# srogatch/ProbQA

Hardware: AMD Instinct MI355X
Metric: next_question_selections_per_sec (higher is better)
Workload: dtype f64; 1 GPU; 1000Qx5Ax1000T fp64 cube resident in HBM, single in-flight quiz; step = priority sweep + argmax + question id on host, synchronous call through the C ABI; questions_per_gpu=1000, parallelism=single GPU, eval_kernel=wg256_np2, selected_question=500

## Files before the change

probqa_amd/csrc/batch_kernels.hip:

```cpp
#include <algorithm>

#include "eval_device.h"
#include "pole_device.h"
#include "pqa_device.h"
#include "pqa_kernels.h"

namespace pqa {

static __device__ double gLog2TableB[kLog2TableDoubles];

hipError_t UploadLog2TableBatch(const double *hostTable) {
  return hipMemcpyToSymbol(HIP_SYMBOL(gLog2TableB), hostTable, kLog2TableDoubles * sizeof(double));
}

namespace {

constexpr int kTileThreads = 256;

template <typename R>
__global__ __launch_bounds__(kTileThreads) void batch_prep_kernel(const QuizSlot *__restrict__ slots, int nSlots, int Bp,
                                                                  const uint32_t *__restrict__ tgap, int64_t ldT, R *__restrict__ PT) {
  __shared__ double tile[64][65];
  const int64_t t0 = (int64_t)blockIdx.x * 64;
  const int b0 = blockIdx.y * 64;
// ... 458 lines not shown
      red[(wave * (K + 2) + K + 1) * QS + slot] = accL;
    }
    __syncthreads();
    if (head) {
      const bool skip = bit_test(a.qgap, q) || ((asked[q >> 5] >> (q & 31)) & 1u);
      double pri = 0.0;
      if (!skip) {
        double mW[K], mWV[K], sums[2];
#pragma unroll
        for (int r = 0; r < K + 2; r++) {
          double s2 = 0.0;
#pragma unroll
          for (int w2 = 0; w2 < NW; w2++) s2 += red[(w2 * (K + 2) + r) * QS + slot];
          if (r < K) { mW[r] = W[r]; mWV[r] = W[r] * sqrt(s2); }
          else sums[r - K] = s2;
        }
        pri = eval_epilogue(mW, -sums[0], mWV, kN, sums[1], a.vCompTail);
        uint32_t listRows = watchW[slot];
        if (watchW[QS + slot] != 0) {
#pragma unroll
          for (int r = 0; r < K; r++)
            if ((EXACT || r < kN) && ((watchW[QS + slot] >> r) & 1u) && mWV[r] * mWV[r] <= kSmallV * (mW[r] * mW[r])) listRows |= 1u << r;
        }
        if (live && listRows != 0) {
          const uint32_t at = pole_list_append(a.poleList, (uint32_t)q, listRows, (uint32_t)b);
          double *dst = a.poleSums + (size_t)at * (2 * kN + 2);
#pragma unroll
          for (int r = 0; r < K; r++)
            if (EXACT || r < kN) { dst[r] = mW[r]; dst[kN + r] = mWV[r]; }
          dst[2 * kN] = sums[0];
          dst[2 * kN + 1] = sums[1];
        }
      }
      watchW[slot] = 0;
      watchW[QS + slot] = 0;
      if (live) {
        if (a.priorityT) a.priorityT[q * Bp + b] = pri;
        if (!skip) {
          if (qs.hostPriority != nullptr) {
            typedef unsigned int u4 __attribute__((ext_vector_type(4)));
            const uint64_t w0 = d2u(pri), w1 = a.tag;
            const u4 x = {(unsigned)w0, (unsigned)(w0 >> 32), (unsigned)w1, (unsigned)(w1 >> 32)};
            asm volatile("global_store_dwordx4 %0, %1, off sc0 sc1" ::"v"(qs.hostPriority + q), "v"(x) : "memory");
          }
          const double cand = pri != pri ? -__builtin_huge_val() : pri;
          if (bestQ < 0 || cand > bestP) { bestP = cand; bestQ = q; }
        }
      }
    }
  }
  if (head && b < Bp) a.recs[(size_t)blockIdx.x * Bp + b] = BatchRecord{bestP, bestQ};
}

__global__ __launch_bounds__(64) void batch_pick_kernel(const BatchRecord *__restrict__ recs, int nRecs, int Bp,
                                                        const QuizSlot *__restrict__ slots, int nSlots, int64_t outBase,
                                                        uint64_t flagValue, uint32_t *dirty, const double *__restrict__ priorityT,
                                                        int64_t Q, const uint32_t *__restrict__ qgap) {
  const int b = blockIdx.x, lane = threadIdx.x;
  if (b >= nSlots) return;
  double bp = 0.0;
  int64_t bq = -1;
  if (dirty != nullptr && dirty[b] != 0) {
    const uint32_t *asked = slots[b].asked;
    for (int64_t q = lane; q < Q; q += 64) {
      if (bit_test(qgap, q) || bit_test(asked, q)) continue;
      double p = priorityT[(size_t)q * Bp + b];
      if (p != p) p = -__builtin_huge_val();
      if (bq < 0 || p > bp) { bp = p; bq = q; }
    }
    if (lane == 0) dirty[b] = 0;
  } else
  for (int g = lane; g < nRecs; g += 64) {
    const BatchRecord r = recs[(size_t)g * Bp + b];
    if (r.index >= 0 && (bq < 0 || r.priority > bp || (r.priority == bp && r.index < bq))) { bp = r.priority; bq = r.index; }
  }
#pragma unroll
  for (int m = 32; m >= 1; m >>= 1) {
    const double op = __shfl_xor(bp, m, 64);
    const int64_t oq = __shfl_xor(bq, m, 64);
    if (oq >= 0 && (bq < 0 || op > bp || (op == bp && oq < bq))) { bp = op; bq = oq; }
  }
  if (lane != 0) return;
  const QuizSlot s = slots[b];
  s.out->priority = bq < 0 ? 0.0 : bp;
  s.out->index = bq < 0 ? -1 : bq + outBase;
  if (s.seq != nullptr) {
    __builtin_amdgcn_fence(__ATOMIC_RELEASE, "");
    __hip_atomic_store(s.seq, flagValue, __ATOMIC_RELAXED, __HIP_MEMORY_SCOPE_SYSTEM);
  }
}

constexpr int kF32LdsTargets = 16384;
__device__ __forceinline__ float wave_sum_f(float v) { return wave_sum_f32(v); }
template <bool LDSROW, int NT>
__global__ __launch_bounds__(NT) void eval_questions_f32_stream(const float *__restrict__ cube, const double *__restrict__ prior,
                                                                 const uint32_t *__restrict__ tgap, const uint32_t *__restrict__ qgap,
                                                                 const uint32_t *__restrict__ asked, double *__restrict__ priority,
                                                                 int64_t K, int64_t Q, int64_t ldT, double vCompTail) {
  constexpr int NW = NT / kWave;
  extern __shared__ double smem[];
  double *wk = smem, *wv = smem + K;
  float *part = reinterpret_cast<float *>(smem + 2 * K);
  float4 *prL = reinterpret_cast<float4 *>(part + 64), *idL = prL + (ldT >> 2);
  const int tid = threadIdx.x, lane = tid % kWave, wave = tid / kWave;
  const int64_t nQuads = ldT >> 2;
  auto prior4 = [&](int64_t i) __attribute__((always_inline)) {
    const uint32_t g = tgap[i >> 3] >> ((4 * i) & 31);
    const double2 a = reinterpret_cast<const double2 *>(prior)[2 * i], b = reinterpret_cast<const double2 *>(prior)[2 * i + 1];
    return make_float4((g & 1) ? 0.f : (float)a.x, (g & 2) ? 0.f : (float)a.y, (g & 4) ? 0.f : (float)b.x, (g & 8) ? 0.f : (float)b.y);
  };
  auto invd4 = [&](const float4 *rowD, int64_t i) __attribute__((always_inline)) {
    const uint32_t g = tgap[i >> 3] >> ((4 * i) & 31);
    const float4 d = rowD[i];
    return make_float4((g & 1) ? 0.f : rcp_nr_f32(d.x), (g & 2) ? 0.f : rcp_nr_f32(d.y), (g & 4) ? 0.f : rcp_nr_f32(d.z),
                       (g & 8) ? 0.f : rcp_nr_f32(d.w));
  };
  if constexpr (LDSROW)
    for (int64_t i = tid; i < nQuads; i += NT) prL[i] = prior4(i);
  for (int64_t q = blockIdx.x; q < Q; q += gridDim.x) {
    if (bit_test(qgap, q) || bit_test(asked, q)) {
      if (tid == 0) priority[q] = 0.0;
      continue;
    }
    const float *qb = cube + q * (K + 1) * ldT;
    const float4 *rowD = reinterpret_cast<const float4 *>(qb + K * ldT);
    __syncthreads();
    if constexpr (LDSROW)
      for (int64_t i = tid; i < nQuads; i += NT) idL[i] = invd4(rowD, i);
    __syncthreads();
    double hWd = 0.0, accLd = 0.0;
    for (int64_t k = 0; k < K; k++) {
      const float4 *rowA = reinterpret_cast<const float4 *>(qb + k * ldT);
      float s = 0.f;
      for (int64_t i = tid; i < nQuads; i += NT) {
        const float4 a = rowA[i];
        float4 id, pr;
        if constexpr (LDSROW) { id = idL[i]; pr = prL[i]; } else { id = invd4(rowD, i); pr = prior4(i); }
        s += (a.x * id.x) * pr.x;
        s += (a.y * id.y) * pr.y;
        s += (a.z * id.z) * pr.z;
        s += (a.w * id.w) * pr.w;
      }
      s = wave_sum_f(s);
      __syncthreads();
      if (lane == 0) part[wave] = s;
      __syncthreads();
      float Wk = 0.f;
#pragma unroll
      for (int w = 0; w < NW; w++) Wk += part[w];
      const float invWk = 1.0f / Wk;
      float v = 0.f, hW = 0.f, accL = 0.f;
      auto element = [&](float a, float id, float pi) __attribute__((always_inline)) {
        const float lh = (a * id) * pi;
        const float p = lh * invWk;
        const float l2 = Num<float>::log2p(p, nullptr);
        hW = fmaf(lh, l2, hW);
        const float d = p - pi;
        v = fmaf(d, d, v);
        return l2;
      };
      for (int64_t i = tid; i < nQuads; i += NT) {
        const float4 a = rowA[i];
        float4 id, pr;
        if constexpr (LDSROW) { id = idL[i]; pr = prL[i]; } else { id = invd4(rowD, i); pr = prior4(i); }
        const float la = element(a.x, id.x, pr.x), lb = element(a.y, id.y, pr.y);
        accL = fmaf(fmaf(id.x * id.x, lb, (id.y * id.y) * la), Num<float>::rcp(la * lb), accL);
        const float lc = element(a.z, id.z, pr.z), ld = element(a.w, id.w, pr.w);
        accL = fmaf(fmaf(id.z * id.z, ld, (id.w * id.w) * lc), Num<float>::rcp(lc * ld), accL);
      }
      v = wave_sum_f(v);
      hW = wave_sum_f(hW);
      accL = wave_sum_f(accL);
// ... 264 lines not shown
```

probqa_amd/csrc/eval_kernels.hip:

```cpp
#include "pqa_device.h"
#include "eval_device.h"
#include "pqa_kernels.h"
#include "prior_device.h"
#include "pole_device.h"

namespace pqa {

static __device__ double gLog2Table[kLog2TableDoubles];
hipError_t UploadLog2Table(const double *hostTable) {
  return hipMemcpyToSymbol(HIP_SYMBOL(gLog2Table), hostTable, kLog2TableDoubles * sizeof(double));
}

struct EvalArgs {
  const double *cube;
  const double *prior;
  const uint32_t *tgap;
  const uint32_t *qgap;
  const uint32_t *asked;
  double *priority;
  double *poleScratch;
  PoleHeader *poleList;
  bool serverWatch;
  bool serverNoWatch;
  int64_t K, T, ldT, qFirst, qLimit;
  double vCompTail;
  FusedSelect fs;
  const QuizSlot *slots;
  int maxGrid;
  int poleNoFollow;
  int poleGate;
  const double *updRowA, *updRowD;
  int64_t updQuestion;
  int64_t updVects, updWorkers;
  int64_t updT;
  TopRequest updTop;
};

__device__ __forceinline__ void select_quiz(EvalArgs &a) {
  if (a.slots == nullptr) return;
  const QuizSlot s = a.slots[blockIdx.y];
  a.prior = s.prior;
  a.asked = s.asked;
  a.priority = s.priority;
  a.fs.out = s.out;
  a.fs.seq = s.seq;
  a.fs.hostPriority = s.hostPriority;
  a.fs.scratch += (size_t)blockIdx.y * (size_t)a.fs.scratchStride;
}

__device__ __forceinline__ void store_priority(double *p, double v) {
  __hip_atomic_store(p, v, __ATOMIC_RELAXED, __HIP_MEMORY_SCOPE_AGENT);
}

struct Best {
  double p;
  int64_t i;
};

__device__ __forceinline__ void best_merge(Best &b, double op, int64_t oi) {
  if (oi >= 0 && (b.i < 0 || op > b.p || (op == b.p && oi < b.i))) { b.p = op; b.i = oi; }
}
__device__ __forceinline__ void best_offer(Best &b, double p, int64_t i) {
  best_merge(b, p != p ? -__builtin_huge_val() : p, i);
}
__device__ __forceinline__ Best wave_best(Best b) {
#pragma unroll
  for (int m = kWave / 2; m >= 1; m >>= 1) {
    const double op = __shfl_xor(b.p, m, kWave);
    const int64_t oi = __shfl_xor(b.i, m, kWave);
    best_merge(b, op, oi);
  }
  return b;
}

template <bool UNI = false>
__device__ __forceinline__ void fused_select(const EvalArgs &a, Best mine, int lane, bool *allReported = nullptr, bool wgSuspect = false) {
  if (a.fs.scratch == nullptr) return;
  const bool sampled = a.fs.sampleSubtasks > 0;
  if (sampled && a.fs.hostPriority == nullptr) asm volatile("s_waitcnt vmcnt(0)" ::: "memory");
  const Best wg = wave_best(mine);
  uint64_t seqValue = a.fs.seqValue, flagValue = a.fs.flagValue;
  if (a.fs.tagCell != nullptr)
    seqValue = flagValue = __hip_atomic_load(a.fs.tagCell, __ATOMIC_RELAXED, __HIP_MEMORY_SCOPE_AGENT);
  const uint64_t tag = (uint64_t)(uint32_t)seqValue << 32;
  SelectResult *rec = a.fs.scratch;
  if (UNI || lane == 0) {
    typedef unsigned int u4 __attribute__((ext_vector_type(4)));
    const uint64_t w0 = d2u(wg.p), w1 = tag | (uint32_t)(wg.i < 0 ? 0x7FFFFFFFu : (uint32_t)wg.i) | (wgSuspect ? 0x80000000u : 0u);
    const u4 v = {(unsigned)w0, (unsigned)(w0 >> 32), (unsigned)w1, (unsigned)(w1 >> 32)};
    asm volatile("global_store_dwordx4 %0, %1, off sc1" ::"v"(rec + blockIdx.x), "v"(v) : "memory");
  }
  if (blockIdx.x != 0) return;
  const unsigned grid = gridDim.x;
  typedef unsigned int u4 __attribute__((ext_vector_type(4)));
  bool complete = true;
  uint32_t anySuspect = 0;
  Best b{0.0, -1};
  for (unsigned chunk = 0; chunk < grid && complete; chunk += 16 * kWave) {
    const SelectResult *p0 = rec + chunk + lane, *p1 = p0 + 4 * kWave, *p2 = p0 + 8 * kWave, *p3 = p0 + 12 * kWave;
    u4 r[16];
    bool all = false;
    for (unsigned spin = 0; spin < (1u << 24) && !all; spin++) {
      asm volatile(
          "global_load_dwordx4 %0, %16, off sc1\n\tglobal_load_dwordx4 %1, %16, off offset:1024 sc1\n\t"
          "global_load_dwordx4 %2, %16, off offset:2048 sc1\n\tglobal_load_dwordx4 %3, %16, off offset:3072 sc1\n\t"
          "global_load_dwordx4 %4, %17, off sc1\n\tglobal_load_dwordx4 %5, %17, off offset:1024 sc1\n\t"
          "global_load_dwordx4 %6, %17, off offset:2048 sc1\n\tglobal_load_dwordx4 %7, %17, off offset:3072 sc1\n\t"
          "global_load_dwordx4 %8, %18, off sc1\n\tglobal_load_dwordx4 %9, %18, off offset:1024 sc1\n\t"
          "global_load_dwordx4 %10, %18, off offset:2048 sc1\n\tglobal_load_dwordx4 %11, %18, off offset:3072 sc1\n\t"
          "global_load_dwordx4 %12, %19, off sc1\n\tglobal_load_dwordx4 %13, %19, off offset:1024 sc1\n\t"
          "global_load_dwordx4 %14, %19, off offset:2048 sc1\n\tglobal_load_dwordx4 %15, %19, off offset:3072 sc1\n\t"
          "s_waitcnt vmcnt(0)"
          : "=&v"(r[0]), "=&v"(r[1]), "=&v"(r[2]), "=&v"(r[3]), "=&v"(r[4]), "=&v"(r[5]), "=&v"(r[6]), "=&v"(r[7]),
            "=&v"(r[8]), "=&v"(r[9]), "=&v"(r[10]), "=&v"(r[11]), "=&v"(r[12]), "=&v"(r[13]), "=&v"(r[14]), "=&v"(r[15])
          : "v"(p0), "v"(p1), "v"(p2), "v"(p3)
          : "memory");
      bool mine = true;
#pragma unroll
      for (int u = 0; u < 16; u++)
        if (chunk + lane + u * kWave < grid) mine = mine && r[u][3] == (unsigned)(tag >> 32);
      all = __all(mine);
      if (!all) __builtin_amdgcn_s_sleep(2);
    }
    complete = all;
#pragma unroll
    for (int u = 0; u < 16; u++)
      if (chunk + lane + u * kWave < grid) {
        const uint64_t pw = (uint64_t)r[u][0] | ((uint64_t)r[u][1] << 32);
        anySuspect |= r[u][2] >> 31;
        best_merge(b, u2d(pw), (r[u][2] & 0x7FFFFFFFu) == 0x7FFFFFFFu ? -1 : (int64_t)(r[u][2] & 0x7FFFFFFFu));
      }
  }
  b = wave_best(b);
  const bool suspects = __any(anySuspect != 0);
  const bool listed = !UNI && suspects && complete && a.poleList != nullptr, lazy = a.fs.lazyFix != 0;
  const bool deferred = listed && !lazy, redo = (UNI && suspects && !a.serverNoWatch) || (listed && lazy);
  if (sampled) {
    if (allReported != nullptr && (UNI || lane == 0)) { allReported[0] = complete; allReported[1] = deferred; allReported[2] = redo; }
    return;
  }
  if (deferred) return;
  if (UNI || lane == 0) {
    a.fs.out->priority = b.i < 0 ? 0.0 : b.p;
    a.fs.out->index = !complete ? -3 : redo ? -4 : b.i < 0 ? -1 : b.i + a.fs.outBase;
    if (a.fs.seq != nullptr) {
      __builtin_amdgcn_fence(__ATOMIC_RELEASE, "");
      __hip_atomic_store(a.fs.seq, flagValue, __ATOMIC_RELAXED, __HIP_MEMORY_SCOPE_SYSTEM);
    }
    if (a.fs.tagCell != nullptr) {
      uint64_t next = seqValue + 1;
      if ((uint32_t)next == 0) next++;
      __hip_atomic_store(a.fs.tagCell, next, __ATOMIC_RELAXED, __HIP_MEMORY_SCOPE_AGENT);
    }
  }
}

__device__ __forceinline__ void pass2_pair(double2 lh, double2 id, double2 pr, double invWk, const double *tbl,
                                           double &hW, double &v, double &accL) {
  const double p0 = lh.x * invWk, p1 = lh.y * invWk;
  const double d0 = p0 - pr.x, d1 = p1 - pr.y;
  const double l20 = log2hot(p0, tbl), l21 = log2hot(p1, tbl);
  hW = fma(lh.x, l20, hW);
  hW = fma(lh.y, l21, hW);
  const double prod = l20 * l21;
  double r = __builtin_amdgcn_rcp(prod);
  r = fma(r, fma(-prod, r, 1.0), r);
  const double num = fma(id.y * l20, id.y, (id.x * l21) * id.x);
  accL = fma(num, r, accL);
  v = fma(d0, d0, v);
  v = fma(d1, d1, v);
}

constexpr double kNearOneShare = 1.0 - 0x1p-9;
constexpr double kQuarterShare = 0.2499;
constexpr int kSusDoubles = 4;

constexpr int kPend = 32;

__host__ __device__ constexpr size_t eval_lds_fixed_doubles(int wpq, int64_t K) {
  return kLog2TableDoubles + 2 * (size_t)wpq + 2 * (size_t)(K + 2) * wpq + (size_t)kPend * (2 * (size_t)K + 3) + 2 * kWave + kSusDoubles;
}
static_assert(kSusDoubles % 2 == 0 && kLog2TableDoubles % 2 == 0 && (kPend * 3) % 2 == 0,
              "the LDS priors behind the fixed part are read as 16-byte pairs: an odd count of doubles in front of them halves their rate (10000 x 5 x 10000: 906 -> 1250 us)");
__host__ __device__ constexpr size_t eval_md_row_offset_bytes(int wpq, int64_t K) {
  return (eval_lds_fixed_doubles(wpq, K) * sizeof(double) + 1023) / 1024 * 1024;
}
__host__ __device__ constexpr size_t eval_lds_doubles(int wpq, int64_t K, bool prLds, int64_t ldT) {
  return kLog2TableDoubles + 2 * (size_t)wpq + 2 * (size_t)(K + 2) * wpq + (size_t)kPend * (2 * (size_t)K + 3) + 2 * kWave + kSusDoubles +
         (prLds ? (size_t)ldT + 2 : 0);
}

__host__ __device__ constexpr bool eval_defers_sums(int wpq, int np, bool prLds) { return wpq <= 8 && !(wpq == 2 && np == 4); }
__host__ __device__ constexpr size_t eval_deferred_bytes(int wpq, int np, int64_t K, bool prLds) {
  return eval_defers_sums(wpq, np, prLds) ? (size_t)(K + 2) * wpq * kWave * sizeof(double) : 0;
}

__device__ __forceinline__ void flush_pending(const EvalArgs &a, const double *pend, int nPend, int lane, Best &best) {
  if (lane < nPend) {
    const int64_t K = a.K;
    const double *rec = pend + (size_t)lane * (2 * K + 3);
    const int64_t q = reinterpret_cast<const int64_t *>(rec)[2 * K + 2];
    const double pri = eval_epilogue(rec, -rec[2 * K], rec + K, K, rec[2 * K + 1], a.vCompTail);
    store_priority(a.priority + (q - a.qFirst), pri);
    if (a.fs.hostPriority != nullptr && a.fs.sampleSubtasks > 0) {
      typedef unsigned int u4 __attribute__((ext_vector_type(4)));
      const uint64_t w0 = d2u(pri), w1 = a.fs.seqValue;
      const u4 x = {(unsigned)w0, (unsigned)(w0 >> 32), (unsigned)w1, (unsigned)(w1 >> 32)};
      asm volatile("global_store_dwordx4 %0, %1, off sc0 sc1" ::"v"(a.fs.hostPriority + (q - a.qFirst)), "v"(x) : "memory");
    }
    best_offer(best, pri, q - a.qFirst);
  }
}

__device__ __forceinline__ double uniform_double(double x) {
  const uint64_t u = d2u(x);
  const uint32_t lo = __builtin_amdgcn_readfirstlane((uint32_t)u), hi = __builtin_amdgcn_readfirstlane((uint32_t)(u >> 32));
  return u2d(((uint64_t)hi << 32) | lo);
}
template <bool COH>
__device__ __forceinline__ uint32_t load_word(const uint32_t *p) {
  if constexpr (COH) return __hip_atomic_load(p, __ATOMIC_RELAXED, __HIP_MEMORY_SCOPE_AGENT);
  else return *p;
}
template <bool COH>
__device__ __forceinline__ double2 load_pair(const double2 *p) {
  if constexpr (COH) {
    const double *d = reinterpret_cast<const double *>(p);
    return make_double2(__hip_atomic_load(d, __ATOMIC_RELAXED, __HIP_MEMORY_SCOPE_AGENT),
                        __hip_atomic_load(d + 1, __ATOMIC_RELAXED, __HIP_MEMORY_SCOPE_AGENT));
  } else {
    return *p;
// ... 317 lines not shown
      }
      wgSuspect = wgSuspect || suspect;
      if (!SERVER && suspect) {
        __syncthreads();
        const int64_t at = a.slots != nullptr ? (int64_t)susWords[4] : q - a.qFirst;
        for (int i = tid; i < 2 * (int)K + 2; i += kThreads) a.poleScratch[at * (2 * K + 2) + i] = rec[i];
      }
      if (nPend + 1 == kPend) {
        __syncthreads();
        if (wave == 0) flush_pending(a, pend, kPend, lane, bestLds[lane]);
      }
    } else {
      hW = wave_sum(hW);
      accL = wave_sum(accL);
      if (lane == 0) {
        part[K * WPQ + wave] = hW;
        part[(K + 1) * WPQ + wave] = accL;
      }
      if constexpr (kListWatch) {
        if (watchRows != 0) atomicOr(&susWords[qpar], watchRows);
      }
      if constexpr (WPQ > 1) __syncthreads();
      uint32_t wideRows = 0;
      if constexpr (kListWatch) {
        const uint32_t w = watchOn ? susWords[qpar] : 0u;
        suspect = (w & 0xFFFFu) != 0;
        wideRows = w >> 16;
      }
      if (wave == 0) {
        for (int r = lane; r < nPart; r += kWave) {
          double acc = part[r * WPQ];
          for (int w2 = 1; w2 < WPQ; w2++) acc += part[r * WPQ + w2];
          if constexpr (kListWatch) {
            if (r < K && acc <= kSmallV && ((wideRows >> (r < 15 ? r : 15)) & 1u)) atomicOr(&susWords[qpar], 1u << (r < 15 ? r : 15));
          }
          if (r < K) acc = rec[r] * sqrt(acc);
          rec[K + r] = acc;
        }
        if constexpr (kListWatch) { if (wideRows != 0) suspect = (susWords[qpar] & 0xFFFFu) != 0; }
        if constexpr (kListWatch && !SERVER) { if (a.poleNoFollow) suspect = false; }
        if (lane == 0) {
          reinterpret_cast<int64_t *>(rec)[2 * K + 2] = q;
          if constexpr (kListWatch) { susWords[qpar ^ 1] = 0; susWords[2 + (qpar ^ 1)] = kGapNoneBits; }
          if constexpr (!SERVER) {
            if (suspect) susWords[4] = pole_list_append(a.poleList, (uint32_t)(q - a.qFirst), K <= 15 ? susWords[qpar] & 0xFFFFu : 0u, a.slots != nullptr ? blockIdx.y : 0u,
                                                        a.poleGate ? susWords[2 + qpar] : 0u);
          }
        }
        wgSuspect = wgSuspect || suspect;
        if (!SERVER && suspect) {
          const int64_t at = a.slots != nullptr ? (int64_t)susWords[4] : q - a.qFirst;
          for (int i = lane; i < 2 * (int)K + 2; i += kWave) a.poleScratch[at * (2 * K + 2) + i] = rec[i];
        }
        if (nPend + 1 == kPend) flush_pending(a, pend, kPend, lane, bestLds[lane]);
      }
    }
    nPend = nPend + 1 == kPend ? 0 : nPend + 1;
    qpar ^= 1;
    q = qn;
  }
  if constexpr (kWatch && SERVER) { if (stepNear >= -0x00001000 || stepSmall >= -0x00201000) susWords[0] = 1u; }
  if constexpr (kDefer || (kWatch && SERVER)) __syncthreads();
  if constexpr (kWatch && SERVER) {
    if (wave == 0) { wgSuspect = watchOn && susWords[0] != 0u; if (lane == 0) susWords[0] = 0u; }
  }
  bool *allReported = reinterpret_cast<bool *>(redW);
  if (wave == 0) flush_pending(a, pend, nPend, lane, bestLds[lane]);
  if (wave == 0) fused_select<SERVER>(a, bestLds[lane], lane, allReported, wgSuspect);
  if constexpr (FUSE) {
    if (blockIdx.x == 0) {
      __syncthreads();
#pragma unroll
      for (int j = 0; j < NP; j++) {
        const int p = tid + j * kThreads;
        if (p < nPairs) reinterpret_cast<double2 *>(const_cast<double *>(a.prior))[p] = pr[j];
      }
    }
  }
  if (a.fs.scratch != nullptr && a.fs.sampleSubtasks > 0 && a.fs.hostPriority != nullptr) {
    if (blockIdx.x == 0) {
      __syncthreads();
      const bool complete = allReported[0], deferred = allReported[1], redo = allReported[2];
      if (!deferred && (SERVER ? wave == 0 : tid == 0)) {
        a.fs.out->priority = 0.0;
        a.fs.out->index = !complete ? -3 : redo ? -4 : 0;
        if (a.fs.seq != nullptr) {
          __builtin_amdgcn_fence(__ATOMIC_RELEASE, "");
          __hip_atomic_store(a.fs.seq, a.fs.flagValue, __ATOMIC_RELAXED, __HIP_MEMORY_SCOPE_SYSTEM);
        }
      }
    }
    return;
  }
  if constexpr (!SERVER) {
    if (a.fs.scratch != nullptr && a.fs.sampleSubtasks > 0 && blockIdx.x == 0) {
      __syncthreads();
      const bool complete = allReported[0];
      if (allReported[1]) return;
      const SampledPick r = select_sampled_wg_lds<true>(a.priority, a.qgap, a.asked, a.qFirst, a.qLimit - a.qFirst,
                                                        a.fs.sampleSubtasks, a.fs.sampleRnd, tbl);
      if (tid == 0) {
        a.fs.out->priority = r.priority;
        a.fs.out->index = complete ? r.index + a.fs.outBase : -3;
        if (a.fs.seq != nullptr) {
          __builtin_amdgcn_fence(__ATOMIC_RELEASE, "");
          __hip_atomic_store(a.fs.seq, a.fs.flagValue, __ATOMIC_RELAXED, __HIP_MEMORY_SCOPE_SYSTEM);
        }
      }
    }
  }
}

template <int WPQ, int NP, bool PRLDS, bool DEFER, bool POLE = false, int KC = 0>
__global__ __launch_bounds__(WPQ * 64) void eval_questions_f64(EvalArgs a) {
  select_quiz(a);
  sweep_body<WPQ, NP, PRLDS, false, DEFER, false, POLE, KC>(a, true);
}
template <int WPQ, int NP, bool PRLDS, bool DEFER, bool POLE = false>
__global__ __launch_bounds__(WPQ * 64) __attribute__((amdgpu_waves_per_eu(3, 3))) void eval_questions_f64_occ3(EvalArgs a) {
  select_quiz(a);
  sweep_body<WPQ, NP, PRLDS, false, DEFER, false, POLE>(a, true);
}

template <int WPQ, int NP, bool DEFER, bool POLE = false, int KC = 0>
__global__ __launch_bounds__(WPQ * 64) void eval_questions_f64_upd(EvalArgs a) {
  sweep_body<WPQ, NP, false, false, DEFER, true, POLE, KC>(a, true);
}

__device__ __forceinline__ uint64_t uniform64(uint64_t x) {
  const uint32_t lo = __builtin_amdgcn_readfirstlane((uint32_t)x), hi = __builtin_amdgcn_readfirstlane((uint32_t)(x >> 32));
  return ((uint64_t)hi << 32) | lo;
}
static_assert(offsetof(ServerMailbox, stop) == 56 && offsetof(ServerMailbox, state) == 64 && sizeof(ServerCtl) == 64, "request line");
__device__ __forceinline__ uint64_t line_u64(uint32_t v, int i) {
  return (uint64_t)(uint32_t)__builtin_amdgcn_readlane((int)v, 2 * i) |
         ((uint64_t)(uint32_t)__builtin_amdgcn_readlane((int)v, 2 * i + 1) << 32);
}

template <int WPQ, int NP, bool DEFER, int KC>
__global__ __launch_bounds__(WPQ * 64) __attribute__((amdgpu_waves_per_eu(3, 3)))
void eval_server_f64(EvalArgs a, ServerMailbox *mb, uint32_t *requestLine, int everyonePolls, ServerCtl *ctl, uint64_t lastSeq,
                     uint64_t idleTicks, unsigned stepOffsetBytes) {
  extern __shared__ double smem[];
  uint32_t *step = reinterpret_cast<uint32_t *>(reinterpret_cast<char *>(smem) + stepOffsetBytes);
  const int wave = (int)__builtin_amdgcn_readfirstlane(threadIdx.x / kWave);
  const unsigned word = threadIdx.x & 15;
  const bool first = blockIdx.x == 0;
  uint32_t *mbWord = requestLine + word, *ctlWord = reinterpret_cast<uint32_t *>(ctl) + word;
  uint64_t last = lastSeq;
  bool copyTable = true;
  for (;;) {
    if (wave == 0) {
      uint32_t v = 0;
      uint64_t go = last;
      const uint64_t t0 = wall_clock64();
      if (first) {
        for (;;) {
          v = __hip_atomic_load(mbWord, __ATOMIC_RELAXED, __HIP_MEMORY_SCOPE_SYSTEM);
          go = line_u64(v, 0);
          if (go != last) break;
          const bool stop = line_u64(v, 7) != 0;
          if (stop || wall_clock64() - t0 > idleTicks) {
            __hip_atomic_store(&mb->state, kServerExiting, __ATOMIC_RELEASE, __HIP_MEMORY_SCOPE_SYSTEM);
            __builtin_amdgcn_fence(__ATOMIC_SEQ_CST, "");
            v = __hip_atomic_load(mbWord, __ATOMIC_RELAXED, __HIP_MEMORY_SCOPE_SYSTEM);
            go = line_u64(v, 0);
            if (go != last && !stop) {
              __hip_atomic_store(&mb->state, kServerRunning, __ATOMIC_RELEASE, __HIP_MEMORY_SCOPE_SYSTEM);
            } else {
              go = ~0ull;
              v = 0xFFFFFFFFu;
            }
            break;
          }
        }
        if (go != ~0ull) __hip_atomic_store(&mb->taken, go, __ATOMIC_RELAXED, __HIP_MEMORY_SCOPE_SYSTEM);
        if (!everyonePolls || go == ~0ull)
          __hip_atomic_store(ctlWord, v, __ATOMIC_RELAXED, __HIP_MEMORY_SCOPE_AGENT);
      } else if (everyonePolls) {
        for (unsigned it = 0;; it++) {
          v = __hip_atomic_load(mbWord, __ATOMIC_RELAXED, __HIP_MEMORY_SCOPE_SYSTEM);
          go = line_u64(v, 0);
          if (go != last && go != 0) break;
          if ((it & 15) == 15) {
            const uint32_t v2 = __hip_atomic_load(ctlWord, __ATOMIC_RELAXED, __HIP_MEMORY_SCOPE_AGENT);
            if (line_u64(v2, 0) == ~0ull) { v = v2; break; }
            if (wall_clock64() - t0 > 8 * idleTicks + 100000000ull) { v = 0xFFFFFFFFu; break; }
          }
          __builtin_amdgcn_s_sleep(1);
        }
      } else {
        for (;;) {
          v = __hip_atomic_load(ctlWord, __ATOMIC_RELAXED, __HIP_MEMORY_SCOPE_AGENT);
          go = line_u64(v, 0);
          if (go != last && go != 0) break;
          if (wall_clock64() - t0 > 8 * idleTicks + 100000000ull) { v = 0xFFFFFFFFu; break; }
          __builtin_amdgcn_s_sleep(1);
        }
      }
      step[word] = v;
    }
    __syncthreads();
    const uint64_t go = uniform64(reinterpret_cast<const uint64_t *>(step)[0]);
    if (go == ~0ull) break;
    EvalArgs b = a;
    b.prior = reinterpret_cast<const double *>(uniform64(reinterpret_cast<const uint64_t *>(step)[1]));
    b.asked = reinterpret_cast<const uint32_t *>(uniform64(reinterpret_cast<const uint64_t *>(step)[2]));
    b.fs.out = reinterpret_cast<SelectResult *>(uniform64(reinterpret_cast<const uint64_t *>(step)[3]));
    b.fs.seq = reinterpret_cast<uint64_t *>(uniform64(reinterpret_cast<const uint64_t *>(step)[4]));
    b.fs.flagValue = uniform64(reinterpret_cast<const uint64_t *>(step)[5]);
    const uint64_t ob = uniform64(reinterpret_cast<const uint64_t *>(step)[6]);
    b.fs.outBase = (int64_t)(ob & ~(kServerHandOver | kServerNoWatch));
    b.serverNoWatch = (ob & kServerNoWatch) != 0;
    b.fs.sampleSubtasks = (ob & kServerHandOver) ? 1 : 0;
    b.fs.seqValue = go;
    asm volatile("" : "+s"(b.cube), "+s"(b.tgap), "+s"(b.qgap), "+s"(b.priority), "+s"(b.fs.scratch), "+s"(b.K), "+s"(b.ldT),
                 "+s"(b.qFirst), "+s"(b.qLimit));
    __syncthreads();
    const uint64_t tA = wall_clock64();
    sweep_body<WPQ, NP, false, true, DEFER, false, true, KC>(b, copyTable);
    copyTable = false;
    last = go;
    if (first && wave == 0) {
      __hip_atomic_store(&mb->pad[0], wall_clock64() - tA, __ATOMIC_RELAXED, __HIP_MEMORY_SCOPE_SYSTEM);
      __hip_atomic_store(&mb->pad[1], go, __ATOMIC_RELEASE, __HIP_MEMORY_SCOPE_SYSTEM);
      __hip_atomic_store(&mb->done, go, __ATOMIC_RELEASE, __HIP_MEMORY_SCOPE_SYSTEM);
    }
    __syncthreads();
  }
  if (first && wave == 0) __hip_atomic_store(&mb->state, kServerExited, __ATOMIC_RELEASE, __HIP_MEMORY_SCOPE_SYSTEM);
}

__global__ __launch_bounds__(256) void eval_questions_f64_stream(EvalArgs a) {
  select_quiz(a);
  constexpr int WPQ = 4, kThreads = 256;
  extern __shared__ double smem[];
  const int64_t ldT = a.ldT, K = a.K;
  double *tbl = smem;
  if (!lds_table_at_zero(tbl)) __builtin_trap();
  double *redW = tbl + kLog2TableDoubles;
  double *wkAll = redW + 2 * WPQ;
  double *partAll = wkAll + 2 * K;
  const int nPart = (int)(K + 2);
  uint32_t *watchWords = reinterpret_cast<uint32_t *>(partAll + 2 * nPart * WPQ);
  const int tid = threadIdx.x, lane = tid % kWave, wave = tid / kWave;
  for (int i = tid; i < kLog2TableDoubles; i += kThreads) tbl[i] = gLog2Table[i];
  if (tid < 4) watchWords[tid] = 0;
  __syncthreads();
  const int64_t qStride = (K + 1) * ldT;
  const int64_t nPairs = ldT >> 1;
  int phase = 0, qpar = 0;
  const bool watch = a.poleList != nullptr;
  bool wgSuspect = false;
  Best best{0.0, -1};
  for (int64_t q = a.qFirst + blockIdx.x; q < a.qLimit; q += gridDim.x) {
    if (bit_test(a.qgap, q) || bit_test(a.asked, q)) {
      if (tid == 0) store_priority(a.priority + (q - a.qFirst), 0.0);
      continue;
    }
    const double *qBase = a.cube + q * qStride;
    const double2 *rowD = reinterpret_cast<const double2 *>(qBase + K * ldT);
    const double2 *prior2 = reinterpret_cast<const double2 *>(a.prior);
    double *wk = wkAll + qpar * K;
    double *part = partAll + qpar * (nPart * WPQ);
    double accL = 0, hW = 0;
    uint32_t poleRows = 0, quarterRows = 0;
    for (int64_t k = 0; k < K; k++) {
      const double2 *rowA = reinterpret_cast<const double2 *>(qBase + k * ldT);
      double s0 = 0, c0 = 0, s1 = 0, c1 = 0;
      for (int64_t p = tid; p < nPairs; p += kThreads) {
        const bool g0 = bit_test(a.tgap, 2 * p), g1 = bit_test(a.tgap, 2 * p + 1);
        const double2 d = rowD[p], av = rowA[p], pv = prior2[p];
        const double x0 = g0 ? 0.0 : (av.x * div_nr(1.0, d.x)) * pv.x;
        const double x1 = g1 ? 0.0 : (av.y * div_nr(1.0, d.y)) * pv.y;
        {
          const double y = x0 - c0;
          const double t = s0 + y;
          c0 = (t - s0) - y;
          s0 = t;
        }
        {
          const double y = x1 - c1;
          const double t = s1 + y;
          c1 = (t - s1) - y;
          s1 = t;
        }
      }
      const double sLane = (s0 - c0) + (s1 - c1);
      double Wk = wave_sum(sLane);
      {
        double *buf = redW + phase * WPQ;
        if (lane == 0) buf[wave] = Wk;
        __syncthreads();
        Wk = row_sum<WPQ>(buf[lane % WPQ]);
        phase ^= 1;
// ... 108 lines not shown
  const int tid = threadIdx.x, lane = tid % kWave, wave = tid / kWave;
  const int b = blockIdx.y;
  const int64_t q = cand[(size_t)b * kRerank + blockIdx.x];
  if (q < 0) {
    if (tid == 0) candPri[(size_t)b * kRerank + blockIdx.x] = 0.0;
    return;
  }
  for (int i = tid; i < kLog2TableDoubles; i += kThreads) tbl[i] = gLog2Table[i];
  __syncthreads();
  const double *prior = slots[b].prior;
  const E *qBase = cube + q * (K + 1) * ldT;
  const E *rowD = qBase + K * ldT;
  const int64_t nPairs = ldT >> 1;
  int phase = 0;
  double accL = 0, hW = 0;
  for (int64_t k = 0; k < K; k++) {
    const E *rowA = qBase + k * ldT;
    double s0 = 0, c0 = 0, s1 = 0, c1 = 0;
    for (int64_t p = tid; p < nPairs; p += kThreads) {
      const bool g0 = bit_test(tgap, 2 * p), g1 = bit_test(tgap, 2 * p + 1);
      const double x0 = g0 ? 0.0 : ((double)rowA[2 * p] * div_nr(1.0, (double)rowD[2 * p])) * prior[2 * p];
      const double x1 = g1 ? 0.0 : ((double)rowA[2 * p + 1] * div_nr(1.0, (double)rowD[2 * p + 1])) * prior[2 * p + 1];
      { const double y = x0 - c0; const double t = s0 + y; c0 = (t - s0) - y; s0 = t; }
      { const double y = x1 - c1; const double t = s1 + y; c1 = (t - s1) - y; s1 = t; }
    }
    double Wk = wave_sum((s0 - c0) + (s1 - c1));
    {
      double *buf = redW + phase * WPQ;
      if (lane == 0) buf[wave] = Wk;
      __syncthreads();
      Wk = row_sum<WPQ>(buf[lane % WPQ]);
      phase ^= 1;
    }
    const double invWk = div_nr(1.0, Wk);
    double v = 0;
    for (int64_t p = tid; p < nPairs; p += kThreads) {
      const bool g0 = bit_test(tgap, 2 * p), g1 = bit_test(tgap, 2 * p + 1);
      double2 pv, id, lh;
      id.x = g0 ? 0.0 : div_nr(1.0, (double)rowD[2 * p]);
      id.y = g1 ? 0.0 : div_nr(1.0, (double)rowD[2 * p + 1]);
      pv.x = g0 ? 0.0 : prior[2 * p];
      pv.y = g1 ? 0.0 : prior[2 * p + 1];
      lh.x = ((double)rowA[2 * p] * id.x) * pv.x;
      lh.y = ((double)rowA[2 * p + 1] * id.y) * pv.y;
      pass2_pair(lh, id, pv, invWk, tbl, hW, v, accL);
    }
    v = wave_sum(v);
    if (lane == 0) {
      if (wave == 0) wk[k] = Wk;
      part[k * WPQ + wave] = v;
    }
  }
  hW = wave_sum(hW);
  accL = wave_sum(accL);
  if (lane == 0) {
    part[K * WPQ + wave] = hW;
    part[(K + 1) * WPQ + wave] = accL;
  }
  __syncthreads();
  if (tid == 0) {
    for (int r = 0; r < nPart; r++) {
      double acc = part[r * WPQ];
      for (int w2 = 1; w2 < WPQ; w2++) acc += part[r * WPQ + w2];
      part[r] = r < K ? wk[r] * sqrt(acc) : acc;
    }
    candPri[(size_t)b * kRerank + blockIdx.x] = eval_epilogue(wk, -part[K], part, K, part[K + 1], vCompTail);
  }
}

__global__ __launch_bounds__(256) void batch_repick_kernel(const int64_t *__restrict__ cand, const double *__restrict__ candPri,
                                                           const QuizSlot *__restrict__ slots, int nSlots, int64_t outBase, uint64_t flagValue) {
  const int b = blockIdx.x * blockDim.x + threadIdx.x;
  if (b >= nSlots) return;
  double bp = 0.0;
  int64_t bq = -1;
  for (int r = 0; r < kRerank; r++) {
    const int64_t q = cand[(size_t)b * kRerank + r];
    if (q < 0) continue;
    double p = candPri[(size_t)b * kRerank + r];
    if (p != p) p = -__builtin_huge_val();
    if (bq < 0 || p > bp || (p == bp && q < bq)) { bp = p; bq = q; }
  }
  const QuizSlot s = slots[b];
  s.out->priority = bq < 0 ? 0.0 : bp;
  s.out->index = bq < 0 ? -1 : bq + outBase;
  if (s.seq != nullptr) {
    __builtin_amdgcn_fence(__ATOMIC_RELEASE, "");
    __hip_atomic_store(s.seq, flagValue, __ATOMIC_RELAXED, __HIP_MEMORY_SCOPE_SYSTEM);
  }
}

size_t BatchRerankScratchBytes() { return (size_t)256 * kRerank * (sizeof(int64_t) + sizeof(double)); }

hipError_t LaunchBatchRerank(const KbView &kb, const QuizSlot *slots, int nSlots, int Bp, const double *priorityT, void *scratch,
                             int64_t outBase, uint64_t flagValue, hipStream_t stream) {
  if (kb.elem != 4 || nSlots <= 0 || nSlots > 256 || scratch == nullptr || priorityT == nullptr) return hipErrorInvalidValue;
  int64_t *cand = static_cast<int64_t *>(scratch);
  double *candPri = reinterpret_cast<double *>(cand + 256 * kRerank);
  const double vCompTail = VCompTail(kb);
  hipLaunchKernelGGL(batch_topk_kernel, dim3((unsigned)nSlots), dim3(256), 0, stream, priorityT, kb.Q, Bp, kb.qgap, slots, cand);
  const size_t shmem = (size_t)(kLog2TableDoubles + 2 * 4 + kb.K + (kb.K + 2) * 4) * sizeof(double);
  hipLaunchKernelGGL(batch_rerank_kernel<float>, dim3(kRerank, (unsigned)nSlots), dim3(256), shmem, stream, static_cast<const float *>(kb.cube),
                     kb.tgap, slots, cand, candPri, kb.K, kb.ldT, vCompTail);
  hipLaunchKernelGGL(batch_repick_kernel, dim3((unsigned)((nSlots + 255) / 256)), dim3(256), 0, stream, cand, candPri, slots, nSlots, outBase, flagValue);
  return hipGetLastError();
}

__global__ __launch_bounds__(256) void log2hot_array_kernel(const double *x, double *out, int64_t n) {
  extern __shared__ double smem[];
  double *tbl = smem;
  if (!lds_table_at_zero(tbl)) __builtin_trap();
  for (int i = threadIdx.x; i < kLog2TableDoubles; i += 256) tbl[i] = gLog2Table[i];
  __syncthreads();
  for (int64_t i = (int64_t)blockIdx.x * 256 + threadIdx.x; i < n; i += (int64_t)gridDim.x * 256) out[i] = log2hot(x[i], tbl);
}

hipError_t LaunchLog2HotArray(const double *x, double *out, int64_t n, hipStream_t stream) {
  if (n <= 0) return hipSuccess;
  const int64_t blocks = (n + 255) / 256;
  hipLaunchKernelGGL(log2hot_array_kernel, dim3((unsigned)(blocks < 2048 ? blocks : 2048)), dim3(256),
                     kLog2TableDoubles * sizeof(double), stream, x, out, n);
  return hipGetLastError();
}

namespace {

struct Variant {
  int id, wpq, np;
  bool prLds;
  const char *name;
};
#define PQA_REG_SHAPES(X)                    \
  X(1, 1, 8, false, "wave_per_question_np8") \
  X(2, 4, 2, false, "wg256_np2")             \
  X(3, 4, 4, false, "wg256_np4")             \
  X(4, 4, 8, false, "wg256_np8")             \
  X(5, 8, 8, true, "wg512_np8_prlds")        \
  X(6, 16, 5, true, "wg1024_np5_prlds")      \
  X(7, 16, 8, true, "wg1024_np8_prlds")      \
  X(8, 2, 4, false, "wg128_np4")             \
  X(9, 8, 5, false, "wg512_np5")             \
  X(10, 8, 10, true, "wg512_np10_prlds")     \
  X(11, 16, 5, false, "wg1024_np5")          \
  X(12, 8, 10, false, "wg512_np10")          \
  X(13, 4, 3, false, "wg256_np3")            \
  X(14, 4, 5, false, "wg256_np5")            \
  X(15, 4, 6, false, "wg256_np6")            \
  X(16, 8, 6, false, "wg512_np6")            \
  X(17, 8, 7, false, "wg512_np7")            \
  X(18, 8, 8, false, "wg512_np8")            \
  X(19, 8, 9, false, "wg512_np9")            \
  X(20, 4, 10, true, "wg256_np10_prlds")     \
  X(21, 4, 10, false, "wg256_np10")          \
  X(22, 4, 6, true, "wg256_np6_prlds")       \
  X(23, 4, 8, true, "wg256_np8_prlds")       \
  X(24, 4, 9, true, "wg256_np9_prlds")
const Variant kVariants[] = {
#define PQA_SHAPE_ROW(id, wpq, np, prLds, name) {id, wpq, np, prLds, name},
    PQA_REG_SHAPES(PQA_SHAPE_ROW)
#undef PQA_SHAPE_ROW
    {99, 4, 0, false, "stream256"},
};

int pick_variant(int64_t ldT, int variant) {
  if (variant != 0) return variant;
  if (ldT <= 1024) return 2;
  if (ldT <= 1536) return 13;
  if (ldT <= 2048) return 3;
  if (ldT <= 2560) return 14;
  if (ldT <= 3072) return 15;
  if (ldT <= 4096) return 4;
  if (ldT <= 4608) return 24;
// ... 292 lines not shown
```

probqa_amd/csrc/hip_engine.h:

```cpp
#pragma once

#include <hip/hip_runtime.h>

#include <atomic>
#include <chrono>
#include <condition_variable>
#include <functional>
#include <cstdint>
#include <memory>
#include <mutex>
#include <cstdio>
#include <ctime>
#include <string>
#include <thread>
#include <unordered_map>
#include <vector>

#include "../../include/PqaHipExt.h"
#include "engine_interface.h"
#include "pqa_kernels.h"
#include "combining.h"
#include "kb_plan.h"
#include "engine_options.h"

// ... 269 lines not shown
  Error RecordAnswerLocked(int64_t iQuiz, int64_t iAnswer, bool remote, bool flushNow);
  struct ResumeEntry { int64_t nAnswered = 0; const AQ *pAQs = nullptr; const void *const *rows = nullptr; Error err; int64_t id = -1; Quiz *quiz = nullptr; };
  Error ResumeEntriesLocked(std::vector<ResumeEntry> &e, bool allOrNone);
  Error ResumeBatchEntriesLocked(int64_t n, const int64_t *pCounts, const AQ *pAQs, const void *const *rows, int64_t *pQuizzes);
  Error PackageRowsLocked(int64_t total, const AQ *pAQs, const void *pRows, std::vector<const void *> &rows);
  Error EnsurePackList(int64_t words);
  int64_t *_hPack = nullptr;
  int64_t _hPackWords = 0;
  hipEvent_t _evPack = nullptr;
  char *_dRowStage = nullptr;
  size_t _rowStageBytes = 0;
  uint64_t _packCalls = 0, _packBytes = 0, _rowsStaged = 0;
  hipError_t TakeQuizBuffers(Quiz *q);
  char *_dResume = nullptr, *_hResume = nullptr;
  size_t _dResumeBytes = 0, _hResumeBytes = 0;
  uint64_t _resumeBatches = 0, _resumesBatched = 0;
  StartBatchInline *_startBatch = nullptr;
  void AppendTrainSteps(int64_t n, const AQ *pAQs, bool fromQuiz, std::vector<TrainStep> &out, std::vector<int64_t> &scratch) const;
  void BuildTrainSteps(int64_t n, const AQ *pAQs, bool fromQuiz, std::vector<TrainStep> &steps, std::vector<int64_t> &chainStart) const;
  struct TrainRecord { const AQ *pAQs; int64_t n, iTarget; double amount; };
  struct TrainBulk;
  TrainBulk *_tb = nullptr;
  void FreeTrainBulk();
  Error ValidateTrainBatchLocked(int64_t n, const int64_t *pCounts, const AQ *pAQs, const int64_t *pTargets, const int64_t *pQuizzes);
  Error TrainRecordsLocked(const std::vector<TrainRecord> &recs, bool fromQuiz);
  uint64_t _trainBulkCalls = 0, _trainBulkRecords = 0, _trainBulkLaunches = 0, _trainBulkHostNs = 0, _trainBulkDeviceNs = 0;
  Error TrainLocked(int64_t nQuestions, const AQ *pAQs, int64_t iTarget, double amount, bool fromQuiz);
  Error ValidateTrainLocked(int64_t nQuestions, const AQ *pAQs, int64_t iTarget) const;
  Error UploadGaps();
  Error RemoveIds(int64_t n, const int64_t *ids, int64_t limit, std::vector<uint32_t> &gapBits, std::vector<int64_t> &gapList, IdLedger &ledger,
                  const char *absentMsg);
  Error ReallocKB(int64_t newQ, int64_t newT, int64_t newQTotal);
  Error CompactLocked(bool fromBlocks, const void *pBlocks, int64_t slotBytes, int64_t emptiedRank, int64_t *pnQuestions,
                      const int64_t **ppOldQuestions, int64_t *pnTargets, const int64_t **ppOldTargets);
  bool IsShard() const { return _qTotal != _Q; }
  int64_t AssignQuiz(Quiz *q);
  void UnassignQuiz(int64_t iQuiz);

  enum class Mode { Regular, Maintenance, Shutdown };

  int64_t _K = 0, _Q = 0, _T = 0, _ldT = 0, _qFirst = 0, _qTotal = 0;
  double _initAmount = 1;
  int _device = 0;
  hipStream_t _stream = nullptr, _ownStream = nullptr;
  char *_dCube = nullptr;
  int _elem = 8;
  uint8_t _precType = 3;
  char *CubeAt(int64_t q, int64_t row = 0) const { return _dCube + ((size_t)(q * (_K + 1) + row) * (size_t)_ldT) * (size_t)_elem; }
  static int64_t RoundLdT(int64_t T, int elem) { const int64_t m = 128 / elem; return ((T + m - 1) / m) * m; }
  double *_dVB = nullptr, *_dPriority = nullptr, *_dRunLength = nullptr, *_dPoleScratch = nullptr;
  size_t PoleScratchBytes(int64_t capQ) const { return (size_t)capQ * (size_t)(2 * _K + 2) * sizeof(double) + PoleListBytes(capQ); }
  uint32_t *_dTGap = nullptr, *_dQGap = nullptr;
  int64_t *_dExps = nullptr, *_dAqs = nullptr, *_dStatus = nullptr, *_dNOut = nullptr;
  int64_t _aqCapacity = 0;
  RatedTargetDev *_dTopScratch[2] = {nullptr, nullptr};
  int64_t _topScratchRecords = 0;
  RatedTargetDev *_hTopBatch = nullptr;
  int64_t _hTopBatchRecords = 0;
  Error EnsureTopScratch(int64_t nQuizzes, int64_t want);
  Error EnsureTopScratchRecords(int64_t need);
  struct TopQFlight { int64_t n = 0, want = 0; uint64_t op = 0; bool onHost = false; std::vector<double> pri; std::vector<std::vector<uint32_t>> asked; };
  TopQFlight _topQ, _topQBatch;
  RatedTargetDev *_hTopQ = nullptr;
  int64_t _hTopQRecords = 0;
  Error EnqueueTopQuestionsLocked(Quiz *q, int64_t maxCount);
  int64_t CollectTopQuestionsLocked(Error &err, CiRatedQuestion *pDest);
  Error EnqueueTopQuestionsBatchLocked(int64_t n, const int64_t *pQuizzes, int64_t maxCount);
  Error CollectTopQuestionsBatchLocked(int64_t n, int64_t stride, CiRatedQuestion *pDest, int64_t *pCounts);
  int64_t TopQuestionsOfVector(const double *pri, const std::vector<uint32_t> &asked, int64_t want, CiRatedQuestion *pDest) const;
  int64_t ListTopTargetsOnHost(Error &err, Quiz *q, int64_t want, CiRatedTarget *pDest, bool referenceOrder = false);
  int64_t ListTopTargetsFast(Error &err, int64_t iQuiz, int64_t maxCount, CiRatedTarget *pDest);
  int64_t ListTopTargetsExact(Error &err, int64_t iQuiz, int64_t maxCount, CiRatedTarget *pDest);
  Error EnsureTopExactScratch(int64_t nQuizzes, int64_t want);
  void *_dTopExact = nullptr;
  size_t _topExactBytes = 0;
  uint64_t _topExactListings = 0;
  struct QuizBuffers { double *dPrior; uint32_t *dAsked; int64_t ldT; size_t askedWords; };
  std::vector<QuizBuffers> _quizBufferPool;
  struct GraphEntry { hipGraphExec_t exec; int64_t variant; hipStream_t stream; uint64_t kbVersion; };
  uint64_t _kbVersion = 0;
  std::unordered_map<Quiz *, GraphEntry> _graphs;
  SelectResult *_dGraphScratch = nullptr;
  uint64_t *_dTagCell = nullptr;
  static constexpr uint64_t kGraphFlagBase = 1ull << 40, kServerFlagBase = 2ull << 40;
  uint64_t _graphTag = kGraphFlagBase + 1;
  void DropQuizBufferPool();
  SelectResult *_dSel = nullptr;
  struct Pinned {
    SelectResult sel; uint64_t seq; int64_t status[2]; int64_t nOut;
    uint64_t opFlag;
    uint64_t topFlag;
    RatedTargetDev top[256];
    int64_t nOutQ;
    uint64_t topQFlag;
    RatedTargetDev topQ[256];
  };
  uint64_t _opSeq = 0;
  std::vector<QuizPinned *> _pinSlabs, _pinFree;
  static constexpr int kPinSlab = 256;
  QuizPinned *TakePin();
  struct BatchCtx;
  struct PendingUpdate { Quiz *q; int64_t qLocal, iAnswer; const void *rowA = nullptr, *rowD = nullptr; bool list = true; };
  std::vector<PendingUpdate> _pendingUpdates;
  Error FlushUpdates();
  void MarkStreamBusy();
  uint64_t _flushes = 0, _flushedUpdates = 0, _maxFlush = 0;
  std::atomic<int> _activeCallers{0};
  const std::atomic<int> *_extCallers = nullptr;
  int Callers() const {
    const int own = _activeCallers.load(std::memory_order_relaxed);
    return _extCallers ? std::max(own, _extCallers->load(std::memory_order_relaxed)) : own;
  }
  bool Concurrent() const { return _opt.combine && Callers() > 1; }
  static int AllowedCpus();
  bool ClientsFitCpus() const { return _opt.combineSpin && Callers() + 2 <= AllowedCpus(); }
  struct SelRequest {
    int64_t iQuiz = -1;
    int kind = 0;
    uint64_t rnd = 0;
    int64_t result = -1;
    Error err;
    std::atomic<int> state{0};
    const double *pri = nullptr;
    int64_t priStride = 0;
    uint64_t priTag = 0;
    BatchCtx *ctx = nullptr;
    uint64_t serial = 0;
    Quiz *quiz = nullptr;
    std::vector<uint32_t> unavailable;
    int64_t nQ = 0, nSub = 0;
  };
  int64_t SelectFromPriorities(SelRequest *r);
  std::atomic<size_t> _pendingCount{0};
  std::atomic<int64_t> _flushedSinceSweep{0};
  std::atomic<int64_t> _sweepNsEwma{0};
  std::atomic<int64_t> _lastCombined{0};
  int64_t Combine(Error &err, int64_t iQuiz, int kind, uint64_t rnd);
  struct Flight;
  struct PostedOp {
    int kind = 0;
    const AQ *aqs = nullptr;
    double amount = 0;
    int64_t iQuiz = -1, arg = 0;
    bool remote = false;
    Error err;
    int64_t result = 0;
    QuizPinned *pin = nullptr;
    uint64_t flagOp = 0;
    Quiz *quiz = nullptr;
    uint64_t serial = 0;
    BatchCtx *ctx = nullptr;
    std::vector<SelRequest *> *batch = nullptr;
    Flight *flight = nullptr;
    std::atomic<int> state{0};
    PostedOp *next = nullptr;
  };
  uint64_t _postedOps = 0, _postedDrains = 0;
  void DrainPosted(PostedOp *ordered);
  void TrainPosted(PostedOp *ordered);
  uint64_t _trainBatches = 0, _trainBatchCalls = 0;
  Error ReleaseQuizLocked(int64_t iQuiz, bool mayWait);
  Error RecordQuizTargetLocked(int64_t iQuiz, int64_t iTarget, double amount);
  int64_t PreferredCombinedBatch(int64_t m) const;
  struct Flight {
    std::vector<SelRequest *> live;
    uint64_t tag = 0;
    bool anySampled = false, quizMinor = false, tagged = false;
    int64_t Bp = 0, nQ = 0;
    hipError_t he = hipSuccess;
    std::chrono::steady_clock::time_point tA, tB, tC;
  };
  void LaunchBatch(BatchCtx &c, std::vector<SelRequest *> &batch, Flight &f);
  void LaunchBatchLocked(BatchCtx &c, std::vector<SelRequest *> &batch, Flight &f);
  bool CollectBatch(BatchCtx &c, std::vector<SelRequest *> &batch, Flight &f, SelRequest *own);
  int64_t NextQuestionArgmaxLocked(Error &err, int64_t iQuiz);
  int64_t NextQuestionSampledLocked(Error &err, int64_t iQuiz, uint64_t rnd);
  std::mutex _rngMu;
  uint64_t _quizSerial = 0;
  uint64_t _combBatches = 0, _combRequests = 0, _combMaxBatch = 0;
  std::atomic<uint64_t> _combNs[7] = {{0}, {0}, {0}, {0}, {0}, {0}, {0}};
  volatile uint64_t *_pendingRecordFlag = nullptr;
  Error WaitFlag(volatile uint64_t *flag, uint64_t value, const char *what);
  Error WaitFlagNapping(volatile uint64_t *flag, uint64_t value, const char *what);
  SelectResult *_dSelScratch = nullptr;
  double *_dPriorScratch = nullptr;
  hipEvent_t _evSweep[2] = {nullptr, nullptr};
  mutable bool _sweepTimed = false;
  static constexpr int64_t kMaxBatch = 256, kBatchGrid = 1024;
  struct BatchPinned {
    QuizSlot slots[kMaxBatch]; SelectResult out[kMaxBatch]; uint64_t seq[kMaxBatch];
    SelectResult sweepOut[kMaxBatch]; uint64_t sweepSeq[kMaxBatch]; uint64_t rnd[kMaxBatch];
  };
  struct BatchCtx : CombineCtx {
    BatchPinned *h = nullptr;
    QuizSlot *dSlots = nullptr;
    SelectResult *dScratch = nullptr;
    double *dPriority = nullptr;
    int64_t priorityQ = -1;
    void *dPT = nullptr; double *dAcc = nullptr; BatchRecord *dRecs = nullptr; double *dPriT = nullptr;
    size_t ptBytes = 0, accBytes = 0, recBytes = 0, priTBytes = 0, rerankBytes = 0;
    void *dRerank = nullptr;
    void *dPole = nullptr;
    size_t poleBytes = 0;
    double *dSelGrand = nullptr, *dSelRun = nullptr;
    size_t selGrandBytes = 0, selRunBytes = 0;
    hipEvent_t evSel[2] = {nullptr, nullptr};
    int lastBp = 0;
    double *hPri = nullptr;
    size_t hPriDoubles = 0;
    bool hPriCoherent = false;
    hipEvent_t event = nullptr;
  };
  BatchCtx _ctx[2];
  Combiner<SelRequest, BatchCtx> _comb{_ctx};
  Error BatchSweep(BatchCtx &c, int64_t n, const int64_t *pQuizzes, std::vector<Quiz *> &quizzes, bool wantPriorities, uint64_t tag,
                   bool hostPriorities = false, bool *pQuizMinor = nullptr, bool *pTagged = nullptr, bool devicePriorities = false);
  Error ValidateBatchLocked(int64_t n, const int64_t *pQuizzes);
  Error NextQuestionSampledBatchLocked(int64_t n, const int64_t *pQuizzes, const uint64_t *pRnd, int64_t *pOut);
  Error LaunchSampledBatch(BatchCtx &c, int64_t n, const uint64_t *pRnd, uint64_t tag);
  struct PartsPack {
    uint64_t seq = 0;
    std::vector<int64_t> quizzes;
    std::vector<uint64_t> serials, versions;
    int64_t nSub = 0, qFirst = 0, nLocal = 0, qTotal = 0, runQuiz = 0, runStride = 0;
    uint64_t kbVersion = 0;
  } _parts;
  int64_t SampledSubtasks() const { return _opt.evalSubtasks ? _opt.evalSubtasks : 8 * _opt.workers; }
  uint64_t *_dPartsWords = nullptr;
  double *_dPartsRun = nullptr, *_dPartsGrand = nullptr, *_dPartsPickRun = nullptr;
  size_t _partsRunBytes = 0, _partsGrandBytes = 0, _partsPickRunBytes = 0;
  uint64_t _sampledBatches = 0, _sampledBatchDeviceNs = 0;
  uint64_t _priorityHostBytes = 0;
  Error WaitBatchFlags(BatchCtx &c, int64_t n, uint64_t tag);
  Error EnqueueBatchLocked(int64_t n, const int64_t *pQuizzes, bool wantPriorities, uint64_t *pTag);
  Error CollectBatchSelectionsLocked(int64_t n, uint64_t tag, CiHipSelection *pOut);
  Error CollectBatchPrioritiesLocked(int64_t n, double *pOut);
  std::vector<Quiz *> _batchQuizzes;
  void *_dClusterScratch = nullptr;
  size_t _clusterScratchBytes = 0;
  bool UseClusterSweep() const;
  Error LaunchSingleSweep(Quiz *q, const FusedSelect *fused);
  bool LazyFix() const;
  Error RunLazyFix(Quiz *q, const FusedSelect &swept, const char *what);
  uint64_t _selSeq = 0;
  uint64_t NextLaunchTag() {
    if ((uint32_t)++_selSeq == 0) ++_selSeq;
    return _selSeq;
  }
  Pinned *_hPinned = nullptr;
  std::vector<uint32_t> _hTGap, _hQGap;
  int64_t _nTargetGaps = 0;
  int64_t _capQ = 0;
  std::vector<int64_t> _questionGapList, _targetGapList;
  IdLedger _questionIds, _targetIds, _quizIds;
  std::vector<int64_t> _globalQuestionGaps;
  IdLedger _globalQuestionIds;
  uint32_t _precMantissa = 0;
  uint16_t _precExponent = 0;
  std::vector<Quiz *> _quizzes;
  std::vector<int64_t> _quizGaps;
  friend struct KbIo;
  struct EngineMutex : PostingLock<PostedOp, HipEngine> {
    using PostingLock::PostingLock;
    bool busy = false, wasBusy = false;
    std::atomic<bool> spinFirst{false};
    bool try_lock() {
      if (!PostingLock::try_lock()) return false;
      wasBusy = busy; busy = true;
      return true;
    }
    void lock() {
      if (spinFirst.load(std::memory_order_relaxed))
        for (int i = 0; i < 400; i++) {
          if (PostingLock::try_lock()) { wasBusy = busy; busy = true; return; }
          for (int j = 0; j < 4; j++) __builtin_ia32_pause();
        }
      PostingLock::lock(); wasBusy = busy; busy = true;
    }
    void lock_urgent() { lock(); }
  };
  struct UrgentLock {
    EngineMutex &mu;
    bool held = false;
    explicit UrgentLock(EngineMutex &m) : mu(m) { lock(); }
    ~UrgentLock() { if (held) unlock(); }
    void lock() { mu.lock_urgent(); held = true; }
    void unlock() { mu.unlock(); held = false; }
  };
  mutable EngineMutex _mu{this, &HipEngine::DrainPosted};
  std::atomic<uint64_t> _nQuestionsAsked{0};
  Mode _mode = Mode::Regular;
  EngineOptions _opt;
  void ApplyEnvironment();
  TaggedPriority *_hHostPriority = nullptr;
  std::vector<double> _hostRun;
  Error CollectHostPriority(uint64_t tag, const Quiz *q);
  int64_t _hostPriorityCap = 0;
  hipError_t EnsureHostPriority();
  int64_t ClusterFrom() const { return _elem == 8 ? _opt.clusterFrom : 16384; }
  struct Speculation {
    Quiz *quiz = nullptr;
    uint64_t priorVersion = 0, tag = 0;
    int kind = 0;
    int64_t variant = 0;
    hipStream_t stream = nullptr;
    FusedSelect fs{};
  } _spec;
  bool _poleListPending = false;
  Error SettlePoleList();
  int _specScore = 0;
  uint64_t _specProbe = 0, _specHits = 0, _specDropped = 0;
  bool Speculate(Quiz *q, int64_t updQuestion = -1, int64_t updAnswer = -1);
  uint64_t _fusedUpdates = 0;
  int64_t SpeculateFor(int64_t iQuiz);
  int TakeSpeculation(Quiz *q, int kindMask, uint64_t *pTag);
  void DropSpeculation() {
    if (_spec.quiz != nullptr) { _spec.quiz = nullptr; _specDropped++; if (_specScore > -8) _specScore--; }
  }
  int64_t _topWantRecent = 10;
  hipStream_t _serverStream = nullptr;
  ServerMailbox *_hMailbox = nullptr;
  ServerCtl *_dServerCtl = nullptr;
  volatile uint64_t *_serverRequest = nullptr;
  bool _serverRequestInVram = false;
  uint64_t _serverReqSeq = 0;
  bool _serverLaunched = false;
  uint64_t _serverKb = 0, _serverPosted = 0;
  int64_t _serverVariant = 0;
  uint64_t _pendingRecordOp = 0;
  bool ServerUsable() const;
  Error ServerPost(Quiz *q, SelectResult *out, uint64_t *flag, uint64_t flagValue, int64_t outBase);
  Error ServerWait(volatile uint64_t *flag, uint64_t value, const char *what);
  void StopServer();
  void ServerQuiesce();
  SelectorRng _rng;
};

void LogAnomaly(DefaultLogger::Severity sev, const char *what, double value);
void CheckPriority(double priority, int64_t index);
int64_t SelectSampledHost(double *run, int64_t n, int64_t nWorkers, uint64_t rnd, const std::function<bool(int64_t)> &skipped);
int64_t SelectSampledHostBits(double *run, int64_t n, int64_t nWorkers, uint64_t rnd, const uint32_t *a, const uint32_t *b);
int64_t FindNearestInPacks(int64_t iMiddle, int64_t nQuestions, const std::function<uint64_t(int64_t)> &avail);
IEngine *CreateShardedEngine(Error &err, const CiEngineDefinition &def, const std::vector<int> &devices);
IEngine *LoadShardedEngine(Error &err, const char *filePath, const std::vector<int> &devices, uint8_t precType = 0);

}
```

probqa_amd/csrc/hip_engine_select.cpp:

```cpp
#include "hip_engine_internal.h"

namespace pqa {
bool HipEngine::QuestionUnavailable(const Quiz *q, int64_t qLocal) const {
  return BitTest(_hQGap, qLocal) || BitTest(q->hAsked, qLocal);
}

int64_t FindNearestInPacks(int64_t iMiddle, int64_t nQuestions, const std::function<uint64_t(int64_t)> &avail) {
  const uint32_t dInf = 200;
  const int64_t iPack64 = iMiddle >> 6;
  const uint32_t iWithin = (uint32_t)(iMiddle & 63);
  const uint64_t available = avail(iPack64);
  if (available != 0) {
    const uint64_t baseMask = (1ULL << iWithin) - 1;
    const uint64_t higher = available & ~baseMask, lower = baseMask & available;
    const uint32_t dHigher = higher ? ((uint32_t)__builtin_ctzll(higher) - iWithin) : dInf;
    const uint32_t dLower = lower ? (iWithin - (uint32_t)(63 - __builtin_clzll(lower))) : dInf;
    return (dHigher < dLower) ? iMiddle + dHigher : iMiddle - dLower;
  }
  const int64_t limPack64 = (nQuestions + 63) >> 6;
  int64_t i = 1;
  while ((iPack64 >= i) && (iPack64 + i < limPack64)) {
    const uint64_t availLeft = avail(iPack64 - i), availRight = avail(iPack64 + i);
    if ((availLeft | availRight) == 0) { i++; continue; }
    const uint32_t dHigher = availRight ? ((uint32_t)__builtin_ctzll(availRight) + 64 - iWithin) : dInf;
// ... 37 lines not shown
    double get() const { return sum - corr; }
  };
  const int64_t quot = n / nWorkers, rem = n % nWorkers, nSubtasks = quot == 0 ? rem : nWorkers;
  auto bound = [&](int64_t i) { return (i + 1) * quot + std::min<int64_t>(i + 1, rem); };
  std::vector<double> grand((size_t)nSubtasks);
  for (int64_t s = 0; s < nSubtasks; s++) {
    Kahan acc;
    for (int64_t i = s == 0 ? 0 : bound(s - 1); i < bound(s); i++) {
      if (!skipped(i)) acc.add(run[i]);
      run[i] = acc.get();
    }
    grand[(size_t)s] = acc.get();
  }
  Kahan tot;
  for (int64_t s = 0; s < nSubtasks; s++) {
    tot.add(grand[(size_t)s]);
    grand[(size_t)s] = tot.get();
    if (!std::isfinite(grand[(size_t)s]))
      LogAnomaly(DefaultLogger::Severity::Error, "Overflow or underflow has happened in the question evaluation subtasks: ", grand[(size_t)s]);
  }
  const double totG = grand[(size_t)nSubtasks - 1];
  if (totG <= 0) LogAnomaly(DefaultLogger::Severity::Warning, "Grand-grand total is ", totG);
  const double selRunLen = totG * (double)rnd / 18446744073709551615.0;
  const int64_t iWorker = std::upper_bound(grand.begin(), grand.end(), selRunLen) - grand.begin();
  if (iWorker >= nSubtasks) return n - 1;
  const double inWorker = selRunLen - (iWorker == 0 ? 0.0 : grand[(size_t)iWorker - 1]);
  const int64_t first = iWorker == 0 ? 0 : bound(iWorker - 1), limit = bound(iWorker);
  int64_t sel = std::upper_bound(run + first, run + limit, inWorker) - run;
  if (sel >= limit) sel = limit - 1;
  return sel;
}
}
int64_t SelectSampledHost(double *run, int64_t n, int64_t nWorkers, uint64_t rnd, const std::function<bool(int64_t)> &skipped) {
  return SelectSampledHostT(run, n, nWorkers, rnd, skipped);
}
int64_t SelectSampledHostBits(double *run, int64_t n, int64_t nWorkers, uint64_t rnd, const uint32_t *a, const uint32_t *b) {
  if (b == nullptr) return SelectSampledHostT(run, n, nWorkers, rnd, [a](int64_t i) { return ((a[i >> 5] >> (i & 31)) & 1u) != 0; });
  return SelectSampledHostT(run, n, nWorkers, rnd, [a, b](int64_t i) { return (((a[i >> 5] | b[i >> 5]) >> (i & 31)) & 1u) != 0; });
}

int64_t HipEngine::FindNearestQuestion(int64_t iMiddle, const Quiz *q) const {
  return FindNearestInPacks(iMiddle, _Q, [&](int64_t p) { return ~(Pack64(_hQGap, p) | Pack64(q->hAsked, p)); });
}

int64_t HipEngine::FinishSelection(Error &err, Quiz *q, int64_t selLocal) {
  if (selLocal >= 0 && QuestionUnavailable(q, selLocal)) selLocal = FindNearestQuestion(selLocal, q);
  if (selLocal < 0) {
    err = Error::Make(ErrCode::QuestionsExhausted, "Found no unasked question that is not in a gap.");
    return -1;
  }
  q->activeQuestion = _qFirst + selLocal;
  _nQuestionsAsked.fetch_add(1, std::memory_order_relaxed);
  return q->activeQuestion;
}

Error HipEngine::EnqueueEval(int64_t iQuiz) {
  std::lock_guard<EngineMutex> lk(_mu);
  Error err = CheckRegular("compute next question");
  if (!err.ok()) return err;
  Quiz *q = UseQuiz(err, iQuiz);
  if (!q) return err;
  hipSetDevice(_device);
  StopServer();
  return LaunchSingleSweep(q, nullptr);
}

bool HipEngine::UseClusterSweep() const { return _opt.evalVariant == 0 && _ldT > ClusterFrom() && EvalClusterSupported(View()); }

Error HipEngine::LaunchSingleSweep(Quiz *q, const FusedSelect *fused) {
  { Error se = SettlePoleList(); if (!se.ok()) return se; }
  if (UseClusterSweep()) {
    const size_t need = EvalClusterScratchBytes(View());
    if (need > _clusterScratchBytes) {
      HIP_TRY(hipStreamSynchronize(_stream));
      hipFree(_dClusterScratch);
      _dClusterScratch = nullptr;
      _clusterScratchBytes = 0;
      HIP_TRY(hipMalloc(&_dClusterScratch, need));
      HIP_TRY(hipMemsetAsync(_dClusterScratch, 0, need, _stream));
      _clusterScratchBytes = need;
    }
    HIP_TRY(LaunchEvalCluster(View(), q->dPrior, q->dAsked, _dPriority, _dClusterScratch, _stream));
    if (fused != nullptr)
      HIP_TRY(LaunchSelectArgmax(_dPriority, _dQGap, q->dAsked, 0, _Q, fused->outBase, fused->out, fused->seq, fused->flagValue, _stream));
    return Error();
  }
  if (_elem == 8) {
    if (_opt.timeSweeps) {
      if (!_evSweep[0]) { HIP_TRY(hipEventCreate(&_evSweep[0])); HIP_TRY(hipEventCreate(&_evSweep[1])); }
      HIP_TRY(hipEventRecord(_evSweep[0], _stream));
    }
    HIP_TRY(LaunchEvalQuestions(View(), q->dPrior, q->dAsked, 0, _Q, _dPriority, (int)_opt.evalVariant, fused, _stream));
    if (_opt.timeSweeps) { HIP_TRY(hipEventRecord(_evSweep[1], _stream)); _sweepTimed = true; }
    return Error();
  }
  if (_opt.evalVariant != 99 && EvalF32RegisterShape(View(), (int)_opt.evalVariant))
    HIP_TRY(LaunchEvalQuestionsF32Reg(View(), q->dPrior, q->dAsked, _dPriority, (int)_opt.evalVariant, _stream));
  else
    HIP_TRY(LaunchEvalQuestionsF32(View(), q->dPrior, q->dAsked, _dPriority, _stream));
  if (fused != nullptr)
    HIP_TRY(LaunchSelectArgmax(_dPriority, _dQGap, q->dAsked, 0, _Q, fused->outBase, fused->out, fused->seq, fused->flagValue, _stream));
  return Error();
}

Error HipEngine::EnqueueSelectArgmax(int64_t iQuiz, void *pOut) {
  std::lock_guard<EngineMutex> lk(_mu);
  Error err = CheckRegular("compute next question");
  if (!err.ok()) return err;
  Quiz *q = UseQuiz(err, iQuiz);
  if (!q) return err;
  const FusedSelect fs{_dSelScratch, pOut ? (SelectResult *)pOut : _dSel, nullptr, NextLaunchTag(), _qFirst, 0, 0, nullptr, 0, 0, nullptr, nullptr};
  hipSetDevice(_device);
  StopServer();
  return LaunchSingleSweep(q, &fs);
}

Error HipEngine::EnqueueSelectArgmaxFlag(int64_t iQuiz, void *pOut, void *pFlag, uint64_t flagValue) {
  std::lock_guard<EngineMutex> lk(_mu);
  Error err = CheckRegular("compute next question");
  if (!err.ok()) return err;
  Quiz *q = UseQuiz(err, iQuiz);
  if (!q) return err;
  if (!pOut || !pFlag) return Error::Make(ErrCode::NullArgument, "Nullptr is passed in place of the record or the flag.");
  hipSetDevice(_device);
  if (_opt.server && !_opt.poleFix && ServerUsable()) return ServerPost(q, (SelectResult *)pOut, (uint64_t *)pFlag, flagValue, _qFirst | (int64_t)kServerNoWatch);
  const FusedSelect fs{_dSelScratch, (SelectResult *)pOut, (uint64_t *)pFlag, NextLaunchTag(), _qFirst, 0, flagValue, nullptr, 0, 0, nullptr, nullptr};
  StopServer();
  return LaunchSingleSweep(q, &fs);
}

hipError_t HipEngine::EnsureHostPriority() {
  if (_hostPriorityCap >= _capQ && _hHostPriority != nullptr) return hipSuccess;
  StopServer();
  if (_hHostPriority) hipHostFree(_hHostPriority);
  _hHostPriority = nullptr;
  _hostPriorityCap = 0;
  const hipError_t e = hipHostMalloc((void **)&_hHostPriority, (size_t)_capQ * sizeof(TaggedPriority), hipHostMallocMapped | hipHostMallocCoherent);
  if (e == hipSuccess) {
    std::memset(_hHostPriority, 0, (size_t)_capQ * sizeof(TaggedPriority));
    _hostPriorityCap = _capQ;
  }
  return e;
}

Error HipEngine::CollectHostPriority(uint64_t tag, const Quiz *q) {
  _hostRun.resize((size_t)_Q);
  const volatile TaggedPriority *rec = _hHostPriority;
  SpinWait w;
  for (int64_t i = 0; i < _Q; i++) {
    if (BitTest(_hQGap, i) || BitTest(q->hAsked, i)) { _hostRun[(size_t)i] = 0.0; continue; }
    while (rec[i].tag != tag)
      if (!w.Tick(std::chrono::seconds(30))) return HipErr(hipErrorNotReady, "priority vector hand-over");
    std::atomic_thread_fence(std::memory_order_acquire);
    _hostRun[(size_t)i] = rec[i].priority;
  }
  return Error();
}

Error HipEngine::WaitFlagNapping(volatile uint64_t *flag, uint64_t value, const char *what) {
  for (int spins = 0; spins < 2000; spins++) {
    if (*flag == value) { std::atomic_thread_fence(std::memory_order_acquire); return Error(); }
    _mm_pause();
  }
  static thread_local bool slackSet = false;
  if (!slackSet) { prctl(PR_SET_TIMERSLACK, 2000UL, 0, 0, 0); slackSet = true; }
  const auto t0 = std::chrono::steady_clock::now();
  uint64_t naps = 0;
  while (*flag != value) {
    struct timespec ts{0, 20000};
    nanosleep(&ts, nullptr);
    if ((++naps & 0x3FF) == 0) {
      if (hipStreamQuery(_stream) == hipSuccess && *flag != value) {
        const hipError_t he = hipStreamSynchronize(_stream);
        if (he != hipSuccess || *flag != value) return HipErr(he == hipSuccess ? hipErrorUnknown : he, what);
      }
      if (std::chrono::steady_clock::now() - t0 > std::chrono::seconds(30)) return HipErr(hipErrorNotReady, what);
    }
  }
  std::atomic_thread_fence(std::memory_order_acquire);
  return Error();
}

Error HipEngine::WaitFlag(volatile uint64_t *flag, uint64_t value, const char *what) {
  SpinWait w;
  while (*flag != value) {
    if (!w.Tick(std::chrono::seconds(30))) return HipErr(hipErrorNotReady, what);
    if (w.Due() && hipStreamQuery(_stream) == hipSuccess && *flag != value) {
      const hipError_t he = hipStreamSynchronize(_stream);
      if (he != hipSuccess || *flag != value) return HipErr(he == hipSuccess ? hipErrorUnknown : he, what);
    }
  }
  std::atomic_thread_fence(std::memory_order_acquire);
  return Error();
}

int64_t HipEngine::NextQuestionArgmax(Error &err, int64_t iQuiz) { return Combine(err, iQuiz, 0, 0); }

bool HipEngine::LazyFix() const {
  return _opt.poleFix && _opt.poleLazy && _opt.poleFollow && _elem == 8 && !UseClusterSweep() && EvalVariantHasFinisherWorkgroup(View(), (int)_opt.evalVariant);
}
Error HipEngine::SettlePoleList() {
  if (!_poleListPending) return Error();
  _poleListPending = false;
  DropSpeculation();
  const KbView kb = View();
  if (kb.poleList != nullptr) HIP_TRY(hipMemsetAsync(kb.poleList, 0, sizeof(PoleHeader), _stream));
  return Error();
}
Error HipEngine::RunLazyFix(Quiz *q, const FusedSelect &swept, const char *what) {
  FusedSelect fs = swept;
  fs.lazyFix = 0;
  fs.flagValue = NextLaunchTag();
  HIP_TRY(LaunchEvalPoleFixup(View(), q->dPrior, q->dAsked, _dPriority, fs, _stream));
  Error err = WaitFlag(fs.seq, fs.flagValue, what);
  std::atomic_thread_fence(std::memory_order_acquire);
  if (err.ok()) _poleListPending = false;
  return err;
}

int64_t HipEngine::NextQuestionArgmaxLocked(Error &err, int64_t iQuiz) {
  err = CheckRegular("compute next question");
  if (!err.ok()) return -1;
  Quiz *q = UseQuiz(err, iQuiz);
  if (!q) return -1;
  hipSetDevice(_device);
  err = FlushUpdates();
  if (!err.ok()) return -1;
  if (_opt.useGraph && _elem == 8) return NextQuestionArgmaxGraph(err, q);
  if (_opt.server && !q->noServer && ServerUsable()) {
    const uint64_t value = kServerFlagBase | ++_opSeq;
    err = ServerPost(q, &_hPinned->sel, &_hPinned->seq, value, 0);
    if (err.ok()) err = ServerWait(&_hPinned->seq, value, "NextQuestionArgmax");
    if (!err.ok()) return -1;
    if (_hPinned->sel.index == -3) {
      err = HipErr(hipErrorLaunchFailure, "NextQuestionArgmax (incomplete sweep)");
      return -1;
    }
    if (_hPinned->sel.index != -4) {
      CheckPriority(_hPinned->sel.priority, _hPinned->sel.index);
      return FinishSelection(err, q, _hPinned->sel.index);
    }
    q->noServer = true;
  }
  uint64_t seq;
  FusedSelect fs{};
  if (TakeSpeculation(q, 1 << 1, &seq) != 0) fs = _spec.fs;
  else {
    seq = NextLaunchTag();
    fs = FusedSelect{_dSelScratch, &_hPinned->sel, &_hPinned->seq, seq, 0, 0, seq, nullptr, 0, 0, nullptr, nullptr, LazyFix() && q->lateStreak < _opt.lateEager ? 1 : 0};
    StopServer();
    err = LaunchSingleSweep(q, &fs);
    if (!err.ok()) return -1;
    if (fs.lazyFix) _poleListPending = true;
  }
  err = WaitFlag(&_hPinned->seq, seq, "NextQuestionArgmax");
  if (!err.ok()) return -1;
  std::atomic_thread_fence(std::memory_order_acquire);
  if (fs.lazyFix) {
    if (_hPinned->sel.index == -4) {
      err = RunLazyFix(q, fs, "NextQuestionArgmax");
      if (!err.ok()) return -1;
      q->lateStreak++;
    } else {
      q->lateStreak = 0;
      if (_hPinned->sel.index != -3) _poleListPending = false;
    }
  }
  if (_hPinned->sel.index == -3) {
    err = HipErr(hipErrorLaunchFailure, "NextQuestionArgmax (incomplete sweep)");
    return -1;
  }
  CheckPriority(_hPinned->sel.priority, _hPinned->sel.index);
  return FinishSelection(err, q, _hPinned->sel.index);
}


Error HipEngine::BatchSweep(BatchCtx &c, int64_t n, const int64_t *pQuizzes, std::vector<Quiz *> &quizzes, bool wantPriorities, uint64_t tag,
                            bool hostPriorities, bool *pQuizMinor, bool *pTagged, bool devicePriorities) {
  if (!c.h) {
    HIP_TRY(hipHostMalloc(&c.h, sizeof(BatchPinned), hipHostMallocMapped | hipHostMallocCoherent));
    std::memset(c.h, 0, sizeof(BatchPinned));
    HIP_TRY(hipMalloc(&c.dSlots, kMaxBatch * sizeof(QuizSlot)));
    HIP_TRY(hipMalloc(&c.dScratch, (size_t)kMaxBatch * kBatchGrid * sizeof(SelectResult)));
    HIP_TRY(hipMemset(c.dScratch, 0, (size_t)kMaxBatch * kBatchGrid * sizeof(SelectResult)));
  }
  const int64_t qb = _opt.batchQb > 0 ? _opt.batchQb : (_elem == 4 ? 4 : 2), wavesRowSharing = ((n + 63) / 64) * ((_Q + qb - 1) / qb);
  bool rowSharing = _elem == 4 || wantPriorities ||
                    (_opt.batchMin > 0 ? n >= _opt.batchMin : (n >= 32 && (wavesRowSharing >= 1536 || (n > 32 && _ldT > 1024 && wavesRowSharing >= 1000))));
  bool mid = EvalMidBatchSupported(View()) && ((_opt.batchForm == 0 && !rowSharing && n >= 7) || _opt.batchForm == 3);
  if (_opt.batchForm == 1 && _elem == 8) { rowSharing = false; mid = false; }
  if (_opt.batchForm == 2) { rowSharing = true; mid = false; }
  if (mid) rowSharing = false;
  if (hostPriorities) {
    wantPriorities = rowSharing;
    if (pQuizMinor) *pQuizMinor = rowSharing;
    if (!c.event) HIP_TRY(hipEventCreateWithFlags(&c.event, hipEventDisableTiming));
  }
  auto copyToHost = [&](const double *src, size_t doubles) -> Error {
    if (c.readers.load(std::memory_order_acquire) != 0)
      return Error::Make(ErrCode::Internal, "A priority buffer is still being read.");
    if (doubles > c.hPriDoubles) {
      HIP_TRY(hipStreamSynchronize(_stream));
      if (c.hPri) hipHostFree(c.hPri);
      c.hPri = nullptr;
      c.hPriDoubles = 0;
      HIP_TRY(hipHostMalloc((void **)&c.hPri, doubles * sizeof(double), hipHostMallocDefault));
      c.hPriDoubles = doubles;
      c.hPriCoherent = false;
    }
    HIP_TRY(hipMemcpyAsync(c.hPri, src, doubles * sizeof(double), hipMemcpyDeviceToHost, _stream));
    _priorityHostBytes += doubles * sizeof(double);
    return Error();
  };
  if (!rowSharing && c.priorityQ != _Q) {
    if (c.dPriority) hipFree(c.dPriority);
    c.dPriority = nullptr;
    c.priorityQ = -1;
    HIP_TRY(hipMalloc(&c.dPriority, (size_t)kMaxBatch * (size_t)_Q * sizeof(double)));
    c.priorityQ = _Q;
  }
  Error err;
  quizzes.assign((size_t)n, nullptr);
  for (int64_t i = 0; i < n; i++) {
    quizzes[i] = UseQuiz(err, pQuizzes[i]);
    if (!quizzes[i]) return err;
    for (int64_t j = 0; j < i; j++)
      if (pQuizzes[j] == pQuizzes[i])
        return Error::MakeP(ErrCode::IndexOutOfRange, "quizId=" + std::to_string(pQuizzes[i]), "A quiz appears twice in one batch.");
    c.h->slots[i] = QuizSlot{quizzes[i]->dPrior, quizzes[i]->dAsked, rowSharing ? nullptr : c.dPriority + (size_t)i * (size_t)_Q,
                                 devicePriorities ? &c.h->sweepOut[i] : &c.h->out[i], devicePriorities ? &c.h->sweepSeq[i] : &c.h->seq[i], nullptr};
  }
  const bool tagged = hostPriorities && !rowSharing && (mid || EvalVariantHasFinisherWorkgroup(View(), (int)_opt.evalVariant));
  if (pTagged) *pTagged = tagged;
  if (tagged) {
    const size_t doubles = 2 * (size_t)n * (size_t)_Q;
    if (c.readers.load(std::memory_order_acquire) != 0) return Error::Make(ErrCode::Internal, "A priority buffer is still being read.");
    if (doubles > c.hPriDoubles || !c.hPriCoherent) {
      HIP_TRY(hipStreamSynchronize(_stream));
      if (c.hPri) hipHostFree(c.hPri);
      c.hPri = nullptr;
// ... 271 lines not shown
    _hostRun.resize((size_t)_Q);
    for (int64_t i = 0; i < n; i++) {
      if (c.h->out[i].index == -3) return HipErr(hipErrorLaunchFailure, "sampled batch (incomplete sweep)");
      const Quiz *q = _batchQuizzes[(size_t)i];
      if (tagged) {
        const volatile TaggedPriority *rec = reinterpret_cast<const TaggedPriority *>(c.hPri) + (size_t)i * (size_t)_Q;
        SpinWait w;
        for (int64_t k = 0; k < _Q; k++) {
          if (BitTest(_hQGap, k) || BitTest(q->hAsked, k)) { _hostRun[(size_t)k] = 0.0; continue; }
          while (rec[k].tag != tag)
            if (!w.Tick(std::chrono::seconds(30))) return HipErr(hipErrorNotReady, "priority vector hand-over (sampled batch)");
          std::atomic_thread_fence(std::memory_order_acquire);
          _hostRun[(size_t)k] = rec[k].priority;
        }
      } else {
        const double *pri = quizMinor ? c.hPri + i : c.hPri + (size_t)i * (size_t)_Q;
        const size_t stride = quizMinor ? (size_t)c.lastBp : 1;
        for (int64_t k = 0; k < _Q; k++) _hostRun[(size_t)k] = BitTest(_hQGap, k) || BitTest(q->hAsked, k) ? 0.0 : pri[(size_t)k * stride];
      }
      picks[(size_t)i] = SelectSampledHostBits(_hostRun.data(), _Q, nSub, pRnd[i], _hQGap.data(), q->hAsked.data());
    }
  } else {
    err = BatchSweep(c, n, pQuizzes, _batchQuizzes, false, tag, false, nullptr, nullptr, true);
    if (!err.ok()) return err;
    err = LaunchSampledBatch(c, n, pRnd, tag);
    if (!err.ok()) return err;
    err = WaitBatchFlags(c, n, tag);
    if (!err.ok()) return err;
    for (int64_t i = 0; i < n; i++) {
      if (c.h->sweepSeq[i] == tag && c.h->sweepOut[i].index == -3) return HipErr(hipErrorLaunchFailure, "sampled batch (incomplete sweep)");
      CheckPriority(c.h->out[i].priority, c.h->out[i].index);
      picks[(size_t)i] = c.h->out[i].index;
    }
    if (_opt.timeSweeps && c.evSel[1]) {
      float ms = 0;
      if (hipEventSynchronize(c.evSel[1]) == hipSuccess && hipEventElapsedTime(&ms, c.evSel[0], c.evSel[1]) == hipSuccess) _sampledBatchDeviceNs += (uint64_t)(ms * 1e6);
      else (void)hipGetLastError();
    }
  }
  _sampledBatches++;
  for (int64_t i = 0; i < n; i++) {
    Error e;
    pOut[i] = FinishSelection(e, _batchQuizzes[(size_t)i], picks[(size_t)i]);
  }
  return Error();
}

Error HipEngine::NextQuestionSampledBatch(int64_t n, const int64_t *pQuizzes, const uint64_t *pRnd, int64_t *pOut) {
  std::lock_guard<std::mutex> selLk(_ctx[0].mu);
  std::lock_guard<EngineMutex> lk(_mu);
  return NextQuestionSampledBatchLocked(n, pQuizzes, pRnd, pOut);
}

Error HipEngine::NextQuestionBatch(int64_t n, const int64_t *pQuizzes, int64_t *pOut) {
  if (_opt.select == 1) return NextQuestionArgmaxBatch(n, pQuizzes, pOut);
  std::lock_guard<std::mutex> selLk(_ctx[0].mu);
  std::lock_guard<EngineMutex> lk(_mu);
  Error err = ValidateBatchLocked(n, pQuizzes);
  if (!err.ok() || n == 0) return err;
  if (!pOut) return Error::Make(ErrCode::NullArgument, "Nullptr is passed in place of a batch buffer.");
  std::vector<uint64_t> rnd((size_t)n);
  {
    std::lock_guard<std::mutex> rk(_rngMu);
    for (int64_t i = 0; i < n; i++) rnd[(size_t)i] = _rng.Next();
  }
  return NextQuestionSampledBatchLocked(n, pQuizzes, rnd.data(), pOut);
}

int64_t HipEngine::NextQuestionArgmaxGraph(Error &err, Quiz *q) {
  if (!_dGraphScratch) {
    hipError_t he = hipMalloc(&_dGraphScratch, kFusedMaxGrid * sizeof(SelectResult));
    if (he == hipSuccess) he = hipMemsetAsync(_dGraphScratch, 0, kFusedMaxGrid * sizeof(SelectResult), _stream);
    if (he == hipSuccess) he = hipMalloc(&_dTagCell, sizeof(uint64_t));
    const uint64_t one = kGraphFlagBase + 1;
    if (he == hipSuccess) he = hipMemcpyAsync(_dTagCell, &one, sizeof(one), hipMemcpyHostToDevice, _stream);
    if (he == hipSuccess) he = hipStreamSynchronize(_stream);
    if (he != hipSuccess) { err = HipErr(he, "graph selection buffers"); return -1; }
    _graphTag = one;
  }
  auto it = _graphs.find(q);
  if (it == _graphs.end() || it->second.variant != _opt.evalVariant || it->second.stream != _stream ||
      it->second.kbVersion != _kbVersion) {
    if (it != _graphs.end()) { hipGraphExecDestroy(it->second.exec); _graphs.erase(it); }
    const FusedSelect fs{_dGraphScratch, &_hPinned->sel, &_hPinned->seq, 0, 0, 0, 0, _dTagCell, 0, 0, nullptr, nullptr};
    hipGraph_t graph = nullptr;
    hipGraphExec_t exec = nullptr;
    hipError_t he = hipStreamBeginCapture(_stream, hipStreamCaptureModeThreadLocal);
    if (he == hipSuccess) {
      const hipError_t le = LaunchEvalQuestions(View(), q->dPrior, q->dAsked, 0, _Q, _dPriority, (int)_opt.evalVariant, &fs, _stream);
      he = hipStreamEndCapture(_stream, &graph);
      if (he == hipSuccess) he = le;
    }
    if (he == hipSuccess) he = hipGraphInstantiate(&exec, graph, nullptr, nullptr, 0);
    if (graph) hipGraphDestroy(graph);
    if (he != hipSuccess) { err = HipErr(he, "graph capture of the selection"); return -1; }
    it = _graphs.emplace(q, GraphEntry{exec, _opt.evalVariant, _stream, _kbVersion}).first;
  }
  const uint64_t expect = _graphTag;
  StopServer();
  err = SettlePoleList();
  if (!err.ok()) return -1;
  const hipError_t he = hipGraphLaunch(it->second.exec, _stream);
  if (he != hipSuccess) { err = HipErr(he, "hipGraphLaunch"); return -1; }
  uint64_t next = _graphTag + 1;
  if ((uint32_t)next == 0) next++;
  _graphTag = next;
  err = WaitFlag(&_hPinned->seq, expect, "NextQuestionArgmax (graph)");
  if (!err.ok()) return -1;
  if (_hPinned->sel.index == -3) { err = HipErr(hipErrorLaunchFailure, "NextQuestionArgmax (incomplete sweep)"); return -1; }
  CheckPriority(_hPinned->sel.priority, _hPinned->sel.index);
  return FinishSelection(err, q, _hPinned->sel.index);
}

int64_t HipEngine::NextQuestionSampled(Error &err, int64_t iQuiz, uint64_t rnd) { return Combine(err, iQuiz, 1, rnd); }

int64_t HipEngine::NextQuestionSampledLocked(Error &err, int64_t iQuiz, uint64_t rnd) {
  err = CheckRegular("compute next question");
  if (!err.ok()) return -1;
  Quiz *q = UseQuiz(err, iQuiz);
  if (!q) return -1;
  hipSetDevice(_device);
  err = FlushUpdates();
  if (!err.ok()) return -1;
  const KbView kb = View();
  const int64_t nSub = _opt.evalSubtasks ? _opt.evalSubtasks : 8 * _opt.workers;
  if (_opt.server && !q->noServer && _opt.hostSampled && !_opt.fusedSampled && ServerUsable()) {
    const uint64_t value = kServerFlagBase | ++_opSeq;
    err = ServerPost(q, &_hPinned->sel, &_hPinned->seq, value, (int64_t)kServerHandOver);
    if (err.ok()) err = ServerWait(&_hPinned->seq, value, "NextQuestionSampled");
    if (!err.ok()) return -1;
    if (_hPinned->sel.index == -3) { err = HipErr(hipErrorLaunchFailure, "NextQuestionSampled (incomplete sweep)"); return -1; }
    if (_hPinned->sel.index != -4) {
      err = CollectHostPriority(_serverPosted, q);
      if (!err.ok()) return -1;
      const int64_t sel = SelectSampledHostBits(_hostRun.data(), _Q, nSub, rnd, _hQGap.data(), q->hAsked.data());
      return FinishSelection(err, q, sel);
    }
    q->noServer = true;
  }
  uint64_t specTag = 0;
  const int took = TakeSpeculation(q, (1 << 2) | (1 << 3), &specTag);
  const bool speculated = took == 2;
  if (took == 0) StopServer();
  if (took != 3 && _opt.hostSampled && !_opt.fusedSampled && _elem == 8 && EvalVariantHasFinisherWorkgroup(kb, (int)_opt.evalVariant)) {
    const hipError_t ae = EnsureHostPriority();
    if (ae != hipSuccess) { err = HipErr(ae, "host priority buffer"); return -1; }
    uint64_t seq = specTag;
    FusedSelect fs{};
    if (speculated) fs = _spec.fs;
    else {
      { Error se = SettlePoleList(); if (!se.ok()) { err = se; return -1; } }
      seq = NextLaunchTag();
      fs = FusedSelect{_dSelScratch, &_hPinned->sel, &_hPinned->seq, seq, 0, 0, seq, nullptr, 1, 0, nullptr, _hHostPriority, LazyFix() && q->lateStreak < _opt.lateEager ? 1 : 0};
      const hipError_t he = LaunchEvalQuestions(kb, q->dPrior, q->dAsked, 0, _Q, _dPriority, (int)_opt.evalVariant, &fs, _stream);
      if (he != hipSuccess) { err = HipErr(he, "NextQuestionSampled"); return -1; }
      if (fs.lazyFix) _poleListPending = true;
    }
    err = WaitFlag(&_hPinned->seq, seq, "NextQuestionSampled");
    if (!err.ok()) return -1;
    if (fs.lazyFix) {
      if (_hPinned->sel.index == -4) {
        err = RunLazyFix(q, fs, "NextQuestionSampled");
        if (!err.ok()) return -1;
        q->lateStreak++;
      } else {
        q->lateStreak = 0;
        if (_hPinned->sel.index != -3) _poleListPending = false;
      }
    }
    if (_hPinned->sel.index == -3) { err = HipErr(hipErrorLaunchFailure, "NextQuestionSampled (incomplete sweep)"); return -1; }
    err = CollectHostPriority(seq, q);
    if (!err.ok()) return -1;
    const int64_t sel = SelectSampledHostBits(_hostRun.data(), _Q, nSub, rnd, _hQGap.data(), q->hAsked.data());
    return FinishSelection(err, q, sel);
  }
  if (took != 3 && _opt.fusedSampled && _elem == 8 && EvalVariantFusesSampled(kb, (int)_opt.evalVariant, nSub)) {
    { Error se = SettlePoleList(); if (!se.ok()) { err = se; return -1; } }
    const uint64_t seq = NextLaunchTag();
    const FusedSelect fs{_dSelScratch, &_hPinned->sel, &_hPinned->seq, seq, 0, 0, seq, nullptr, nSub, rnd, _dRunLength, nullptr};
    const hipError_t he = LaunchEvalQuestions(kb, q->dPrior, q->dAsked, 0, _Q, _dPriority, (int)_opt.evalVariant, &fs, _stream);
    if (he != hipSuccess) { err = HipErr(he, "NextQuestionSampled"); return -1; }
    err = WaitFlag(&_hPinned->seq, seq, "NextQuestionSampled");
    if (!err.ok()) return -1;
    if (_hPinned->sel.index == -3) { err = HipErr(hipErrorLaunchFailure, "NextQuestionSampled (incomplete sweep)"); return -1; }
    CheckPriority(_hPinned->sel.priority, _hPinned->sel.index);
  return FinishSelection(err, q, _hPinned->sel.index);
  }
  if (took != 3) {
    err = LaunchSingleSweep(q, nullptr);
    if (!err.ok()) return -1;
  }
  hipError_t he = hipSuccess;
  const uint64_t op = ++_opSeq;
  if (he == hipSuccess)
    he = LaunchSelectSampled(_dPriority, _dQGap, q->dAsked, 0, _Q, nSub, rnd, _dRunLength, &_hPinned->sel, &_hPinned->opFlag,
                             op, _stream);
  if (he != hipSuccess) { err = HipErr(he, "NextQuestionSampled"); return -1; }
  err = WaitFlag(&_hPinned->opFlag, op, "NextQuestionSampled");
  if (!err.ok()) return -1;
  CheckPriority(_hPinned->sel.priority, _hPinned->sel.index);
  return FinishSelection(err, q, _hPinned->sel.index);
}

int64_t HipEngine::NextQuestion(Error &err, int64_t iQuiz) {
  if (_opt.select == 1) return Combine(err, iQuiz, 0, 0);
  uint64_t rnd;
  { std::lock_guard<std::mutex> lk(_rngMu); rnd = _rng.Next(); }
  return Combine(err, iQuiz, 1, rnd);
}

}
```

probqa_amd/csrc/hip_engine_server.cpp:

```cpp
#include "hip_engine_internal.h"

namespace pqa {
bool HipEngine::ServerUsable() const { return _elem == 8 && EvalServerSupported(View(), (int)_opt.evalVariant) && _Q > 0; }

void HipEngine::StopServer() {
  (void)FlushUpdates();
  DropSpeculation();
  if (!_serverLaunched) return;
  hipSetDevice(_device);
  _serverRequest[7] = 1;
  std::atomic_thread_fence(std::memory_order_seq_cst);
  hipStreamSynchronize(_serverStream);
  _serverRequest[7] = 0;
  std::atomic_thread_fence(std::memory_order_seq_cst);
  _serverLaunched = false;
}

void HipEngine::ServerQuiesce() {
  if (!_serverLaunched || _serverPosted == 0) return;
  volatile ServerMailbox *mb = _hMailbox;
  SpinWait w;
  while (mb->done != _serverPosted && mb->state != kServerExited)
    if (!w.Tick(std::chrono::seconds(30))) return;
}

Error HipEngine::ServerWait(volatile uint64_t *flag, uint64_t value, const char *what) {
  SpinWait w;
  volatile ServerMailbox *mb = _hMailbox;
  while (*flag != value) {
    if (!w.Tick(std::chrono::seconds(30))) return HipErr(hipErrorNotReady, what);
    if (w.Due() && mb->state == kServerExited && mb->taken != _serverPosted && *flag != value) return HipErr(hipErrorUnknown, what);
  }
  std::atomic_thread_fence(std::memory_order_acquire);
  return Error();
}

Error HipEngine::ServerPost(Quiz *q, SelectResult *out, uint64_t *flag, uint64_t flagValue, int64_t outBase) {
  { Error fe = FlushUpdates(); if (!fe.ok()) return fe; }
  if (_pendingRecordOp != 0 && _pendingRecordFlag != nullptr && !_mu.wasBusy) {
    Error e = WaitFlag(_pendingRecordFlag, _pendingRecordOp, "ServerPost");
    if (!e.ok()) return e;
  } else if (_mu.wasBusy) {
    HIP_TRY(hipStreamSynchronize(_stream));
  }
  _pendingRecordOp = 0;
  _mu.busy = false;
  if (!_serverStream) {
    int prLeast = 0, prGreatest = 0;
    HIP_TRY(hipDeviceGetStreamPriorityRange(&prLeast, &prGreatest));
    HIP_TRY(hipStreamCreateWithPriority(&_serverStream, hipStreamNonBlocking, prLeast));
    HIP_TRY(hipHostMalloc((void **)&_hMailbox, sizeof(ServerMailbox), hipHostMallocDefault));
    std::memset(_hMailbox, 0, sizeof(ServerMailbox));
    HIP_TRY(hipMalloc((void **)&_dServerCtl, sizeof(ServerCtl)));
    void *vram = nullptr;
    int largeBar = 0;
    if (_opt.serverVramMailbox && hipDeviceGetAttribute(&largeBar, hipDeviceAttributeIsLargeBar, _device) == hipSuccess && largeBar &&
        hipExtMallocWithFlags(&vram, 64, hipDeviceMallocFinegrained) == hipSuccess && vram != nullptr) {
      _serverRequest = (volatile uint64_t *)vram;
      _serverRequestInVram = true;
      for (int i = 0; i < 8; i++) _serverRequest[i] = 0;
      std::atomic_thread_fence(std::memory_order_seq_cst);
    } else {
      (void)hipGetLastError();
    }
    if (!_serverRequestInVram) _serverRequest = &_hMailbox->req;
  }
  if (_serverLaunched && (_serverKb != _kbVersion || _serverVariant != _opt.evalVariant)) StopServer();
  volatile ServerMailbox *mb = _hMailbox;
  if (_serverLaunched && _serverPosted != 0) {
    SpinWait w;
    while ((_serverRequestInVram ? mb->done : mb->taken) != _serverPosted && mb->state != kServerExited)
      if (!w.Tick(std::chrono::seconds(30))) return HipErr(hipErrorNotReady, "ServerPost (previous request never taken)");
  }
  const uint64_t prev = _serverReqSeq;
  const uint64_t seq = NextLaunchTag();
  volatile uint64_t *rq = _serverRequest;
  rq[1] = (uint64_t)(uintptr_t)q->dPrior;
  rq[2] = (uint64_t)(uintptr_t)q->dAsked;
  rq[3] = (uint64_t)(uintptr_t)out;
  rq[4] = (uint64_t)(uintptr_t)flag;
  rq[5] = flagValue;
  rq[6] = (uint64_t)outBase;
  std::atomic_thread_fence(std::memory_order_seq_cst);
  rq[0] = seq;
  std::atomic_thread_fence(std::memory_order_seq_cst);
  _serverReqSeq = seq;
  _serverPosted = seq;
  if (_serverLaunched) {
    SpinWait w;
    for (;;) {
      if (mb->taken == seq) return Error();
      if (mb->state == kServerExited) {
        std::atomic_thread_fence(std::memory_order_acquire);
        if (mb->taken == seq) return Error();
        break;
      }
      if (!w.Tick(std::chrono::seconds(30))) return HipErr(hipErrorNotReady, "ServerPost (request neither taken nor refused)");
    }
    _serverLaunched = false;
  }
  HIP_TRY(hipStreamSynchronize(_serverStream));
  HIP_TRY(hipMemsetAsync(_dServerCtl, 0, sizeof(ServerCtl), _serverStream));
  mb->state = kServerRunning;
  std::atomic_thread_fence(std::memory_order_seq_cst);
  HIP_TRY(EnsureHostPriority());
  HIP_TRY(LaunchEvalServer(View(), 0, _Q, _dPriority, (int)_opt.evalVariant, _dSelScratch, _hMailbox, (void *)_serverRequest, _serverRequestInVram, _dServerCtl, prev,
                           (uint64_t)_opt.serverIdleUs * 100, _hHostPriority, _serverStream,
                           _opt.poleFix != 0));
  _serverLaunched = true;
  _serverKb = _kbVersion;
  _serverVariant = _opt.evalVariant;
  return Error();
}

}
```

probqa_amd/csrc/hip_engine_update.cpp:

```cpp
#include "hip_engine_internal.h"

namespace pqa {
Error HipEngine::RecordAnswerImpl(int64_t iQuiz, int64_t iAnswer, bool remote) {
  CallScope scope(_activeCallers);
  if (_opt.combine && (_opt.postAlways || !_mu.try_lock())) {
    PostedOp op;
    op.kind = 1; op.iQuiz = iQuiz; op.arg = iAnswer; op.remote = remote;
    PostAndWait(_mu, op);
    return op.err;
  }
  std::unique_lock<EngineMutex> lk(_mu, std::defer_lock);
  if (_opt.combine) lk = std::unique_lock<EngineMutex>(_mu, std::adopt_lock);
  else lk.lock();
  return RecordAnswerLocked(iQuiz, iAnswer, remote, !Concurrent());
}

Error HipEngine::RecordAnswerBatch(int64_t n, const int64_t *pQuizzes, const int64_t *pAnswers) {
  if (n < 0) return Error::MakeP(ErrCode::NegativeCount, "count=" + std::to_string(n), "|nQuizzes| must be non-negative.");
  if (n > 0 && (!pQuizzes || !pAnswers)) return Error::Make(ErrCode::NullArgument, "Nullptr is passed in place of a batch buffer.");
  CallScope scope(_activeCallers);
  std::lock_guard<EngineMutex> lk(_mu);
  Error first;
  for (int64_t i = 0; i < n && first.ok(); i++) first = RecordAnswerLocked(pQuizzes[i], pAnswers[i], false, false);
  Error fe = FlushUpdates();
// ... 89 lines not shown
  if (_pendingUpdates.empty()) return Error();
  std::vector<PendingUpdate> ups;
  ups.swap(_pendingUpdates);
  _pendingCount.store(0, std::memory_order_relaxed);
  for (PendingUpdate &u : ups) u.q->updatePending = false;
  auto requeue = [&](size_t from, hipError_t he, const char *what) {
    (void)hipGetLastError();
    for (size_t i = from; i < ups.size(); i++) ups[i].q->updatePending = true;
    _pendingUpdates.insert(_pendingUpdates.begin(), ups.begin() + (std::ptrdiff_t)from, ups.end());
    _pendingCount.store(_pendingUpdates.size(), std::memory_order_relaxed);
    MarkStreamBusy();
    return HipErr(he, what);
  };
  hipSetDevice(_device);
  ServerQuiesce();
  const int64_t nLoose = std::max<int64_t>(1, _opt.workers - 1);
  const int64_t topCount = _T <= 16384 ? std::min<int64_t>(std::min<int64_t>(std::min<int64_t>(_opt.topCache, _topWantRecent), kQuizTop), _T) : 0;
  auto listed = [&](Quiz *q, uint64_t op) { q->topOp = op; q->topVersion = q->priorVersion; q->topCount = topCount; };
  auto counted = [&](size_t n) {
    _flushes++;
    _flushedUpdates += n;
    _flushedSinceSweep.fetch_add((int64_t)n, std::memory_order_relaxed);
    if (n > _maxFlush) _maxFlush = n;
  };
  if (ups.size() == 1) {
    const PendingUpdate &u = ups[0];
    const uint64_t op = _opSeq + 1;
    const hipError_t he = LaunchRecordAnswer(View(), u.q->dPrior, u.q->dAsked, u.qLocal, u.iAnswer, nLoose, u.list ? u.q->pin->top : nullptr, &u.q->pin->nOut,
                                             &u.q->pin->topFlag, op, topCount, _stream, u.rowA, u.rowD);
    if (he != hipSuccess) return requeue(0, he, "LaunchRecordAnswer");
    _opSeq = op;
    counted(1);
    if (u.list) listed(u.q, op);
    if (topCount > 0 && u.list) {
      _pendingRecordOp = op;
      _pendingRecordFlag = &u.q->pin->topFlag;
      _mu.busy = _mu.wasBusy;
    } else {
      MarkStreamBusy();
    }
    return Error();
  }
  static_assert(kQuizTopDev == kQuizTop && offsetof(QuizPinned, nOut) == kQuizTop * sizeof(RatedTargetDev) &&
                offsetof(QuizPinned, topFlag) == offsetof(QuizPinned, nOut) + 8, "the batched kernel addresses the quiz's lines by layout");
  const KbView kb = View();
  static thread_local RecordBatchInline b;
  for (size_t first = 0; first < ups.size(); first += kRecordInline) {
    b.n = (int32_t)std::min<size_t>(kRecordInline, ups.size() - first);
    b.topCount = (int32_t)topCount;
    for (int32_t i = 0; i < b.n; i++) {
      const PendingUpdate &u = ups[first + (size_t)i];
      b.s[i] = RecordSlot{u.q->dPrior, u.q->dAsked, u.list ? (void *)u.q->pin : nullptr, (int32_t)u.qLocal, (int32_t)u.iAnswer, _opSeq + 1 + (uint64_t)i, u.rowA, u.rowD};
    }
    const hipError_t he = LaunchRecordAnswerBatch(kb, b, nLoose, _stream);
    if (he != hipSuccess) return requeue(first, he, "LaunchRecordAnswerBatch");
    for (int32_t i = 0; i < b.n; i++) if (ups[first + (size_t)i].list) listed(ups[first + (size_t)i].q, _opSeq + 1 + (uint64_t)i);
    _opSeq += (uint64_t)b.n;
    counted((size_t)b.n);
  }
  MarkStreamBusy();
  return Error();
}

bool HipEngine::Speculate(Quiz *q, int64_t updQuestion, int64_t updAnswer) {
  const bool withUpdate = updQuestion >= 0;
  if (!withUpdate) DropSpeculation();
  if (!_opt.speculate || (_opt.server && !q->noServer) || _opt.useGraph || _qTotal != _Q || _Q <= 0) return false;
  if (_opt.server && _serverLaunched) return false;
  if (Concurrent()) return false;
  if (withUpdate && (!_opt.fuseUpdate || _specScore < -4)) return false;
  if (_specScore < -4 && (++_specProbe & 31) != 0) return false;
  const KbView kb = View();
  int kind = 0;
  if (_opt.select == 1) kind = 1;
  else if (_opt.hostSampled && !_opt.fusedSampled && _elem == 8 && EvalVariantHasFinisherWorkgroup(kb, (int)_opt.evalVariant)) kind = 2;
  else if (!(_opt.fusedSampled && _elem == 8)) kind = 3;
  if (kind == 0) return false;
  const int64_t nLoose = std::max<int64_t>(1, _opt.workers - 1);
  if (withUpdate && (kind == 3 || UseClusterSweep() || !EvalFusesUpdate(kb, (int)_opt.evalVariant, nLoose))) return false;
  if (kind == 2 && EnsureHostPriority() != hipSuccess) return false;
  if (withUpdate) DropSpeculation();
  const uint64_t seq = NextLaunchTag();
  if (!SettlePoleList().ok()) return false;
  const FusedSelect fs{_dSelScratch, &_hPinned->sel, &_hPinned->seq, seq, 0, 0, seq, nullptr, kind == 2 ? 1 : 0, 0, nullptr,
                       kind == 2 ? _hHostPriority : nullptr, (kind == 1 || kind == 2) && LazyFix() && q->lateStreak < _opt.lateEager ? 1 : 0};
  if (withUpdate) {
    const int64_t topCount = std::min<int64_t>(std::min<int64_t>(std::min<int64_t>(_opt.topCache, _topWantRecent), kQuizTop), _T);
    const uint64_t op = _opSeq + 1;
    if (LaunchEvalQuestionsWithUpdate(kb, q->dPrior, q->dAsked, _dPriority, (int)_opt.evalVariant, fs, updQuestion, updAnswer, nLoose, q->pin->top,
                                      &q->pin->nOut, &q->pin->topFlag, op, topCount, _stream) != hipSuccess) {
      (void)hipGetLastError();
      return false;
    }
    _opSeq = op;
    q->topOp = op; q->topVersion = q->priorVersion; q->topCount = topCount;
    _flushes++; _flushedUpdates++; _fusedUpdates++;
    if (_maxFlush < 1) _maxFlush = 1;
  } else if (kind == 1   ? !LaunchSingleSweep(q, &fs).ok()
             : kind == 3 ? !LaunchSingleSweep(q, nullptr).ok()
                         : LaunchEvalQuestions(kb, q->dPrior, q->dAsked, 0, _Q, _dPriority, (int)_opt.evalVariant, &fs, _stream) != hipSuccess) {
    (void)hipGetLastError();
    return false;
  }
  _spec.quiz = q; _spec.priorVersion = q->priorVersion; _spec.tag = seq; _spec.kind = kind; _spec.fs = fs;
  if (fs.lazyFix) _poleListPending = true;
  _spec.variant = _opt.evalVariant; _spec.stream = _stream;
  _pendingRecordOp = 0;
  _pendingRecordFlag = nullptr;
  _mu.busy = true;
  return withUpdate;
}

int HipEngine::TakeSpeculation(Quiz *q, int kindMask, uint64_t *pTag) {
  if (_spec.quiz == nullptr) return 0;
  const bool match = _spec.quiz == q && ((kindMask >> _spec.kind) & 1) && _spec.priorVersion == q->priorVersion && _spec.tag == _selSeq &&
                     _spec.variant == _opt.evalVariant && _spec.stream == _stream && (!_opt.server || q->noServer) && !_opt.useGraph;
  if (!match) { DropSpeculation(); return 0; }
  _spec.quiz = nullptr;
  _specHits++;
  if (_specScore < 8) _specScore++;
  *pTag = _spec.tag;
  return _spec.kind;
}

Error HipEngine::RecordAnswer(int64_t iQuiz, int64_t iAnswer) { return RecordAnswerImpl(iQuiz, iAnswer, false); }
Error HipEngine::RecordAnswerRemote(int64_t iQuiz, int64_t iAnswer) { return RecordAnswerImpl(iQuiz, iAnswer, true); }

int64_t HipEngine::GetActiveQuestionId(Error &err, int64_t iQuiz) {
  std::lock_guard<EngineMutex> lk(_mu);
  err = CheckRegular("get active question ID for a quiz");
  if (!err.ok()) return -1;
  Quiz *q = UseQuiz(err, iQuiz);
  if (!q) return -1;
  return q->activeQuestion;
}

Error HipEngine::SetActiveQuestion(int64_t iQuiz, int64_t iQuestion) {
  std::lock_guard<EngineMutex> lk(_mu);
  Error err = CheckRegular("set active question ID for a quiz");
  if (!err.ok()) return err;
  Quiz *q = UseQuiz(err, iQuiz);
  if (!q) return err;
  q->activeQuestion = iQuestion;
  return Error();
}

Error HipEngine::GetPriors(int64_t iQuiz, double *pOut, int64_t n) {
  std::lock_guard<EngineMutex> lk(_mu);
  Error err;
  Quiz *q = UseQuiz(err, iQuiz);
  if (!q) return err;
  if (!pOut) return Error::Make(ErrCode::NullArgument, "Nullptr is passed in place of the prior buffer.");
  if (n != _T) return Error::MakeP(ErrCode::IndexOutOfRange, RangeParams(n, _T, _T), "Prior buffer length must equal nTargets.");
  hipSetDevice(_device);
  { Error fe = FlushUpdates(); if (!fe.ok()) return fe; }
  HIP_TRY(hipMemcpyAsync(pOut, q->dPrior, (size_t)_T * sizeof(double), hipMemcpyDeviceToHost, _stream));
  HIP_TRY(hipStreamSynchronize(_stream));
  return Error();
}

Error HipEngine::Log2HotArray(const double *pIn, double *pOut, int64_t n) {
  std::lock_guard<EngineMutex> lk(_mu);
  if (n < 0 || (n > 0 && (!pIn || !pOut))) return Error::Make(ErrCode::NullArgument, "Nullptr is passed in place of a Log2Hot buffer.");
  if (n == 0) return Error();
  hipSetDevice(_device);
  double *dIn = nullptr, *dOut = nullptr;
  HIP_TRY(hipMalloc(&dIn, (size_t)n * sizeof(double)));
  hipError_t he = hipMalloc(&dOut, (size_t)n * sizeof(double));
// ... 491 lines not shown
```

probqa_amd/csrc/pole_kernels.hip:

```cpp
#include <cmath>

#include "eval_device.h"
#include "pole_device.h"
#include "pqa_device.h"
#include "pqa_kernels.h"

namespace pqa {

static __device__ double gLog2TableP[kLog2TableDoubles];
static __device__ double gLog2Entry0RefP;

hipError_t UploadLog2TablePole(const double *hostTable) {
  const double entry0 = std::log2(1.0 + 0x1p-11) * 9.9999999999999927e-01;
  const hipError_t e = hipMemcpyToSymbol(HIP_SYMBOL(gLog2Entry0RefP), &entry0, sizeof(double));
  if (e != hipSuccess) return e;
  return hipMemcpyToSymbol(HIP_SYMBOL(gLog2TableP), hostTable, kLog2TableDoubles * sizeof(double));
}

namespace {

#ifndef PQA_FIX_WAVES
#define PQA_FIX_WAVES 4
#endif
#ifndef PQA_FIX_DEPTH
// ... 239 lines not shown
            double vNew = (vOld - dF * dF) + dR * dR;
            if (!(vNew > 0.0)) vNew = dR * dR;
            recV[kk] = a.secondIsWV ? Wx * sqrt(vNew) : vNew;
            recW[kk] = Wx;
          }
          rr[10] = dH;
          rr[11] = dL;
        }
        __builtin_amdgcn_wave_barrier();
        if (lane == 0)
          for (int r = 0; r < nb; r++) { dHsum += red[(size_t)r * kFixRed + 10]; dLsum += red[(size_t)r * kFixRed + 11]; }
        __builtin_amdgcn_wave_barrier();
      }
    }
    if (lane == 0) {
      if (a.priority != nullptr || a.priorityT != nullptr || a.slots != nullptr) {
        const double pri = eval_epilogue(recW, -(rec[2 * K] + dHsum), recV, K, rec[2 * K + 1] + dLsum, a.vCompTail);
        double *dst = a.priorityT != nullptr ? a.priorityT + (size_t)qLocal * a.Bp + en.b
                      : a.slots != nullptr ? a.slots[en.b].priority + qLocal : a.priority + qLocal;
        __hip_atomic_store(dst, pri, __ATOMIC_RELAXED, __HIP_MEMORY_SCOPE_AGENT);
        TaggedPriority *hp = a.slots != nullptr ? a.slots[en.b].hostPriority : a.hostPriority;
        if (hp != nullptr) {
          typedef unsigned int u4 __attribute__((ext_vector_type(4)));
          const uint64_t w0 = d2u(pri), w1 = a.hostTag;
          const u4 x = {(unsigned)w0, (unsigned)(w0 >> 32), (unsigned)w1, (unsigned)(w1 >> 32)};
          asm volatile("global_store_dwordx4 %0, %1, off sc0 sc1" ::"v"(hp + qLocal), "v"(x) : "memory");
        }
      } else {
        for (int k = 0; k < K; k++) { recG[a.wOff + k] = recW[k]; recG[a.vOff + k] = recV[k]; }
        recG[a.hOff] = rec[2 * K] + dHsum;
        recG[a.lOff] = rec[2 * K + 1] + dLsum;
      }
      if (a.maskDense != nullptr) a.maskDense[qLocal] = 0;
      if (a.dirty != nullptr) a.dirty[en.b] = 1u;
    }
    __builtin_amdgcn_wave_barrier();
  }
  double *misc = smem, *pub = smem + 8;
  if (a.hostPriority != nullptr || a.slots != nullptr) __threadfence_system();
  else __threadfence();
  __syncthreads();
  if (tid == 0) {
    const uint32_t arrived = atomicAdd(&a.list->arrived, 1u);
    misc[2] = arrived == gridDim.x - 1 ? 1.0 : 0.0;
  }
  __syncthreads();
  if (misc[2] == 0.0) return;
  __threadfence();
  if (a.fs.scratch != nullptr && a.slots == nullptr) {
    const int64_t nQ = a.nQ;
    const bool sampled = a.fs.sampleSubtasks > 0;
    uint64_t seqValue = a.fs.seqValue, flagValue = a.fs.flagValue;
    if (a.fs.tagCell != nullptr) seqValue = flagValue = __hip_atomic_load(a.fs.tagCell, __ATOMIC_RELAXED, __HIP_MEMORY_SCOPE_AGENT);
    double outP = 0.0;
    int64_t outI = 0;
    if (!sampled) {
      Best b{0.0, -1};
      for (int64_t j = tid; j < nQ; j += blockDim.x) {
        const int64_t q = a.qFirst + j;
        if (bit_test(a.qgap, q) || bit_test(a.asked, q)) continue;
        double p = __hip_atomic_load(a.priority + j, __ATOMIC_RELAXED, __HIP_MEMORY_SCOPE_AGENT);
        if (p != p) p = -__builtin_huge_val();
        best_merge(b, p, j);
      }
      for (int m = kWave / 2; m >= 1; m >>= 1) {
        const double op = __shfl_xor(b.p, m, kWave);
        const int64_t oi = __shfl_xor(b.i, m, kWave);
        best_merge(b, op, oi);
      }
      Best *wb = reinterpret_cast<Best *>(pub);
      if (lane == 0) wb[wave] = b;
      __syncthreads();
      if (tid == 0) {
        for (int w = 1; w < wgWaves; w++) best_merge(b, wb[w].p, wb[w].i);
        outP = b.i < 0 ? 0.0 : b.p;
        outI = b.i < 0 ? -1 : b.i + a.fs.outBase;
      }
    } else if (a.fs.hostPriority == nullptr) {
      const SampledPick r = select_sampled_wg_lds<true>(a.priority, a.qgap, a.asked, a.qFirst, nQ, a.fs.sampleSubtasks, a.fs.sampleRnd, pub);
      outP = r.priority;
      outI = r.index + a.fs.outBase;
    }
    if (tid == 0) {
      a.fs.out->priority = outP;
      a.fs.out->index = outI;
      if (a.fs.seq != nullptr) {
        __builtin_amdgcn_fence(__ATOMIC_RELEASE, "");
        __hip_atomic_store(a.fs.seq, flagValue, __ATOMIC_RELAXED, __HIP_MEMORY_SCOPE_SYSTEM);
      }
      if (a.fs.tagCell != nullptr) {
        uint64_t next = seqValue + 1;
        if ((uint32_t)next == 0) next++;
        __hip_atomic_store(a.fs.tagCell, next, __ATOMIC_RELAXED, __HIP_MEMORY_SCOPE_AGENT);
      }
    }
  }
  if (a.fs.scratch != nullptr && a.slots != nullptr && a.nSlots > 0) {
    const bool handOver = a.fs.sampleSubtasks > 0;
    for (int b = wave; b < a.nSlots; b += wgWaves) {
      const QuizSlot qs = a.slots[b];
      Best best{0.0, -1};
      if (!handOver) {
        for (int64_t j = lane; j < a.nQ; j += kWave) {
          const int64_t q = a.qFirst + j;
          if (bit_test(a.qgap, q) || bit_test(qs.asked, q)) continue;
          double p = __hip_atomic_load(qs.priority + j, __ATOMIC_RELAXED, __HIP_MEMORY_SCOPE_AGENT);
          if (p != p) p = -__builtin_huge_val();
          best_merge(best, p, j);
        }
        for (int m = kWave / 2; m >= 1; m >>= 1) {
          const double op = __shfl_xor(best.p, m, kWave);
          const int64_t oi = __shfl_xor(best.i, m, kWave);
          best_merge(best, op, oi);
        }
      }
      if (lane == 0) {
        qs.out->priority = handOver || best.i < 0 ? 0.0 : best.p;
        qs.out->index = handOver ? 0 : best.i < 0 ? -1 : best.i + a.fs.outBase;
        if (qs.seq != nullptr) {
          __builtin_amdgcn_fence(__ATOMIC_RELEASE, "");
          __hip_atomic_store(qs.seq, a.fs.flagValue, __ATOMIC_RELAXED, __HIP_MEMORY_SCOPE_SYSTEM);
        }
      }
    }
  }
  if (tid == 0) {
    a.list->arrived = 0;
    a.list->floorBits = 0ull;
    __hip_atomic_store(&a.list->count, 0u, __ATOMIC_RELAXED, __HIP_MEMORY_SCOPE_AGENT);
  }
}

}

size_t PoleListBytes(int64_t capacity) { return sizeof(PoleHeader) + (size_t)capacity * sizeof(PoleEntry); }

hipError_t LaunchPoleFixup(const PoleFix &fix, hipStream_t stream) {
  if (fix.list == nullptr || fix.sums == nullptr) return hipErrorInvalidValue;
  PoleFix a = fix;
  a.rows = a.K <= 2 ? 2 : a.K <= 5 ? 5 : a.K <= 8 ? 8 : 16;
  void (*kern)(PoleFix) = a.rows == 2 ? pole_fixup_kernel<2> : a.rows == 5 ? pole_fixup_kernel<5> : a.rows == 8 ? pole_fixup_kernel<8> : pole_fixup_kernel<16>;
  a.waveLds = (int)(((size_t)kFixDepth * (((size_t)a.rows + 2) * 1024 + 16) / 8 + (size_t)a.rows * kFixRowStride + (size_t)a.rows * kFixRed + 2 * (size_t)a.K + 2 + 1) / 2 * 2);
  int wgWaves = kFixThreads / kWave;
  while (wgWaves > 1 && (size_t)wgWaves * a.waveLds * sizeof(double) > 150 * 1024) wgWaves--;
  size_t shmem = (size_t)wgWaves * a.waveLds * sizeof(double);
  if (shmem < 512) shmem = 512;
  if (a.fs.scratch != nullptr && a.fs.sampleSubtasks > 0 && a.fs.hostPriority == nullptr) {
    const size_t need = ((size_t)select_sampled_lds_doubles(a.nQ, a.fs.sampleSubtasks) + 8) * sizeof(double);
    if (need > shmem) shmem = need;
  }
  if (shmem > kLdsPerCU) return hipErrorInvalidValue;
  static LaunchCache caches[4];
  const int dev = DeviceSlot();
  int perCU = 0;
  const hipError_t e = caches[a.rows == 2 ? 0 : a.rows == 5 ? 1 : a.rows == 8 ? 2 : 3].Residency(dev, kern, wgWaves * kWave, shmem, &perCU);
  if (e != hipSuccess) return e;
  int64_t grid = (int64_t)DeviceCUs(dev) * perCU;
  const int64_t wgs = (fix.capacity + wgWaves - 1) / wgWaves;
  if (fix.capacity > 0 && grid > wgs) grid = wgs;
  if (grid < 1) grid = 1;
  if (a.gate) {
    if (a.priority == nullptr || a.slots != nullptr || a.bySlot || !a.secondIsWV) a.gate = 0;
    else hipLaunchKernelGGL(pole_bounds_kernel, dim3((unsigned)((fix.capacity + 255) / 256 < 1 ? 1 : (fix.capacity + 255) / 256 > 64 ? 64 : (fix.capacity + 255) / 256)),
                            dim3(256), 0, stream, a);
  }
  hipLaunchKernelGGL(kern, dim3((unsigned)grid), dim3((unsigned)(wgWaves * kWave)), shmem, stream, a);
  return hipGetLastError();
}

}
```

probqa_amd/csrc/pqa_device.h:

```cpp
#pragma once

#include <hip/hip_runtime.h>
#include <stdint.h>

#include <type_traits>
#include <utility>

namespace pqa {

constexpr int kWave = 64;

template <typename F, int... I>
__device__ __forceinline__ void static_for_impl(F &&f, std::integer_sequence<int, I...>) {
  (f(std::integral_constant<int, I>{}), ...);
}
template <int N, typename F>
__device__ __forceinline__ void static_for(F &&f) {
  static_for_impl(static_cast<F &&>(f), std::make_integer_sequence<int, N>{});
}
constexpr uint64_t kExpMaskUp = 0x7FF0000000000000ULL;
constexpr uint64_t kExp0Up = 0x3FF0000000000000ULL;

__device__ __forceinline__ uint64_t d2u(double d) { return (uint64_t)__double_as_longlong(d); }
__device__ __forceinline__ double u2d(uint64_t u) { return __longlong_as_double((long long)u); }

__device__ __forceinline__ bool bit_test(const uint32_t *__restrict__ bits, int64_t i) {
  return (bits[i >> 5] >> (i & 31)) & 1u;
}

__device__ __forceinline__ double cube_ld(const void *cube, int elem, int64_t i) {
  return elem == 8 ? static_cast<const double *>(cube)[i] : (double)static_cast<const float *>(cube)[i];
}
__device__ __forceinline__ void cube_st(void *cube, int elem, int64_t i, double v) {
  if (elem == 8) static_cast<double *>(cube)[i] = v; else static_cast<float *>(cube)[i] = (float)v;
}

__device__ __forceinline__ double div_nr(double n, double d) {
  double r = __builtin_amdgcn_rcp(d);
  const double e = fma(-d, r, 1.0);
  r = fma(r, e, r);
  const double q0 = n * r;
  const double rem = fma(-d, q0, n);
  return fma(rem, r, q0);
}

typedef unsigned int u32x4_t __attribute__((ext_vector_type(4)));
using RowRsrc = __amdgpu_buffer_rsrc_t;

__device__ __forceinline__ RowRsrc row_rsrc(const void *row, int64_t bytes) {
  const uint64_t p = (uint64_t)(uintptr_t)row;
  const uint64_t pu = ((uint64_t)(uint32_t)__builtin_amdgcn_readfirstlane((int)(uint32_t)(p >> 32)) << 32) |
                      (uint32_t)__builtin_amdgcn_readfirstlane((int)(uint32_t)p);
  return __builtin_amdgcn_make_buffer_rsrc(reinterpret_cast<void *>((uintptr_t)pu), (short)0,
                                           __builtin_amdgcn_readfirstlane((int)bytes), 0x00020000);
}
template <bool NT = false>
__device__ __forceinline__ double2 row_load(RowRsrc rs, uint32_t byteOffset) {
  return __builtin_bit_cast(double2, __builtin_amdgcn_raw_buffer_load_b128(rs, byteOffset, 0, NT ? 2 : 0));
}

typedef unsigned int dma_rsrc_t __attribute__((ext_vector_type(4)));
template <bool PLAIN_BYTES = false>
__device__ __forceinline__ dma_rsrc_t dma_rsrc(const void *row, int64_t bytes) {
  const uint64_t base = (uint64_t)(uintptr_t)row;
  return dma_rsrc_t{(unsigned)__builtin_amdgcn_readfirstlane((unsigned)base),
                    (unsigned)__builtin_amdgcn_readfirstlane((unsigned)(base >> 32)) & 0xFFFFu,
                    PLAIN_BYTES ? (unsigned)bytes : (unsigned)__builtin_amdgcn_readfirstlane((unsigned)bytes), 0x00020000u};
}
__device__ __forceinline__ void dma16(dma_rsrc_t rsrc, unsigned byteOffset, unsigned ldsDst) {
  unsigned keep;
  asm volatile("s_mov_b32 %0, m0\n\ts_mov_b32 m0, %3\n\ts_nop 0\n\tbuffer_load_dwordx4 %1, %2, 0 offen lds\n\ts_mov_b32 m0, %0"
               : "=&s"(keep) : "v"(byteOffset), "s"(rsrc), "s"(__builtin_amdgcn_readfirstlane(ldsDst)) : "memory");
}
__device__ __forceinline__ void dma4(dma_rsrc_t rsrc, unsigned byteOffset, unsigned ldsDst) {
  unsigned keep;
  asm volatile("s_mov_b32 %0, m0\n\ts_mov_b32 m0, %3\n\ts_nop 0\n\tbuffer_load_dword %1, %2, 0 offen lds\n\ts_mov_b32 m0, %0"
               : "=&s"(keep) : "v"(byteOffset), "s"(rsrc), "s"(__builtin_amdgcn_readfirstlane(ldsDst)) : "memory");
}
__device__ __forceinline__ void wait_vmcnt(int n) {
#define PQA_VM(k) case k: asm volatile("s_waitcnt vmcnt(" #k ")" ::: "memory"); break;
  switch (n) {
    PQA_VM(0) PQA_VM(1) PQA_VM(2) PQA_VM(3) PQA_VM(4) PQA_VM(5) PQA_VM(6) PQA_VM(7) PQA_VM(8) PQA_VM(9) PQA_VM(10) PQA_VM(11) PQA_VM(12)
    PQA_VM(13) PQA_VM(14) PQA_VM(15) PQA_VM(16) PQA_VM(17) PQA_VM(18) PQA_VM(19) PQA_VM(20) PQA_VM(21) PQA_VM(22) PQA_VM(23) PQA_VM(24)
    PQA_VM(25) PQA_VM(26) PQA_VM(27) PQA_VM(28) PQA_VM(29) PQA_VM(30) PQA_VM(31) PQA_VM(32) PQA_VM(33) PQA_VM(34) PQA_VM(35) PQA_VM(36)
    PQA_VM(37) PQA_VM(38) PQA_VM(39) PQA_VM(40) PQA_VM(41) PQA_VM(42) PQA_VM(43) PQA_VM(44) PQA_VM(45) PQA_VM(46) PQA_VM(47) PQA_VM(48)
    default: asm volatile("s_waitcnt vmcnt(48)" ::: "memory"); break;
  }
#undef PQA_VM
}
// ... 21 lines not shown
  return k;
}

__device__ __forceinline__ double log2hot(double x, const double *__restrict__ tbl) {
  const Log2Bits k = log2_bits();
  const uint32_t lo = (uint32_t)d2u(x);
  const uint32_t hi = (uint32_t)(d2u(x) >> 32);
  const double de = u2d(0x4330000000000000ULL | (uint64_t)(hi >> 20)) - 4503599627371519.0;
#ifdef PQA_ABLATE_TABLE_CONFLICTS
  const uint32_t tblByte = (((hi >> 6) & 0x0u) | ((uint32_t)__lane_id() << 4)) & 0x3FF0u;
#else
  const uint32_t tblByte = (hi >> 6) & 0x3FF0u;
#endif
  (void)tbl;
  typedef double f64x2_t __attribute__((ext_vector_type(2)));
  const f64x2_t yc = *reinterpret_cast<const __attribute__((address_space(3))) f64x2_t *>((uintptr_t)tblByte);
  const uint32_t mhi = (hi & k.keepM) | (k.fill & ~k.keepM);
  const uint32_t zhi = (hi & k.keepZ) | (k.fill & ~k.keepZ);
  const double m = u2d((uint64_t)mhi << 32);
  const double z = u2d(((uint64_t)zhi << 32) | lo);
  const double w = (z - m) * yc.y;
  double c = fma(w, -0x1.55046a143789p-4, 0x1.47fd3ffac83b4p-3);
  c = fma(w, c, -0x1.62e42fefa39efp-2);
  c = fma(w, c, 1.0);
  const double log2z = fma(w, c, yc.x);
  return log2z + de;
}

__device__ __forceinline__ void two_sum(double a, double b, double &s, double &e) {
  s = a + b;
  const double bb = s - a;
  e = (a - (s - bb)) + (b - bb);
}

struct Comp {
  double s, c;
};

__device__ __forceinline__ Comp comp_merge(Comp a, Comp b) {
  Comp r;
  double e;
  two_sum(a.s, b.s, r.s, e);
  r.c = (a.c + b.c) + e;
  return r;
}

constexpr int kDppXor1 = 0xB1, kDppXor2 = 0x4E, kDppHalfMirror = 0x141, kDppMirror = 0x140;

template <int CTRL>
__device__ __forceinline__ double mov_dpp(double v) {
  const uint64_t b = d2u(v);
  int lo = (int)(uint32_t)b, hi = (int)(uint32_t)(b >> 32);
  lo = __builtin_amdgcn_update_dpp(0, lo, CTRL, 0xF, 0xF, true);
  hi = __builtin_amdgcn_update_dpp(0, hi, CTRL, 0xF, 0xF, true);
  return u2d(((uint64_t)(uint32_t)hi << 32) | (uint32_t)lo);
}

struct Pair { double a, b; };
__device__ __forceinline__ Pair swap16(double v) {
  const uint64_t b = d2u(v);
  const auto r0 = __builtin_amdgcn_permlane16_swap((uint32_t)b, (uint32_t)b, false, false);
  const auto r1 = __builtin_amdgcn_permlane16_swap((uint32_t)(b >> 32), (uint32_t)(b >> 32), false, false);
  return Pair{u2d(((uint64_t)r1[0] << 32) | r0[0]), u2d(((uint64_t)r1[1] << 32) | r0[1])};
}
__device__ __forceinline__ Pair swap32(double v) {
  const uint64_t b = d2u(v);
  const auto r0 = __builtin_amdgcn_permlane32_swap((uint32_t)b, (uint32_t)b, false, false);
  const auto r1 = __builtin_amdgcn_permlane32_swap((uint32_t)(b >> 32), (uint32_t)(b >> 32), false, false);
  return Pair{u2d(((uint64_t)r1[0] << 32) | r0[0]), u2d(((uint64_t)r1[1] << 32) | r0[1])};
}

__device__ __forceinline__ double wave_sum(double v) {
  v += mov_dpp<kDppXor1>(v);
  v += mov_dpp<kDppXor2>(v);
  v += mov_dpp<kDppHalfMirror>(v);
  v += mov_dpp<kDppMirror>(v);
  Pair p = swap16(v);
  v = p.a + p.b;
  p = swap32(v);
  return p.a + p.b;
}

template <int CTRL>
__device__ __forceinline__ float mov_dpp_f32(float v) {
  return __builtin_bit_cast(float, __builtin_amdgcn_update_dpp(0, __builtin_bit_cast(int, v), CTRL, 0xF, 0xF, true));
}
__device__ __forceinline__ float wave_sum_f32(float v) {
  v += mov_dpp_f32<kDppXor1>(v);
  v += mov_dpp_f32<kDppXor2>(v);
  v += mov_dpp_f32<kDppHalfMirror>(v);
  v += mov_dpp_f32<kDppMirror>(v);
  const uint32_t b = __builtin_bit_cast(uint32_t, v);
  const auto r = __builtin_amdgcn_permlane16_swap(b, b, false, false);
  v = __builtin_bit_cast(float, (uint32_t)r[0]) + __builtin_bit_cast(float, (uint32_t)r[1]);
  const uint32_t c = __builtin_bit_cast(uint32_t, v);
  const auto r2 = __builtin_amdgcn_permlane32_swap(c, c, false, false);
  return __builtin_bit_cast(float, (uint32_t)r2[0]) + __builtin_bit_cast(float, (uint32_t)r2[1]);
}

__device__ __forceinline__ Comp wave_sum_comp(Comp v) {
  v = comp_merge(v, Comp{mov_dpp<kDppXor1>(v.s), mov_dpp<kDppXor1>(v.c)});
  v = comp_merge(v, Comp{mov_dpp<kDppXor2>(v.s), mov_dpp<kDppXor2>(v.c)});
  v = comp_merge(v, Comp{mov_dpp<kDppHalfMirror>(v.s), mov_dpp<kDppHalfMirror>(v.c)});
  v = comp_merge(v, Comp{mov_dpp<kDppMirror>(v.s), mov_dpp<kDppMirror>(v.c)});
  Pair ps = swap16(v.s), pc = swap16(v.c);
  v = comp_merge(Comp{ps.a, pc.a}, Comp{ps.b, pc.b});
  ps = swap32(v.s);
  pc = swap32(v.c);
  return comp_merge(Comp{ps.a, pc.a}, Comp{ps.b, pc.b});
}

template <int W>
__device__ __forceinline__ Comp row_sum_comp(Comp v) {
  if constexpr (W >= 2) v = comp_merge(v, Comp{mov_dpp<kDppXor1>(v.s), mov_dpp<kDppXor1>(v.c)});
  if constexpr (W >= 4) v = comp_merge(v, Comp{mov_dpp<kDppXor2>(v.s), mov_dpp<kDppXor2>(v.c)});
  if constexpr (W >= 8) v = comp_merge(v, Comp{mov_dpp<kDppHalfMirror>(v.s), mov_dpp<kDppHalfMirror>(v.c)});
  if constexpr (W >= 16) v = comp_merge(v, Comp{mov_dpp<kDppMirror>(v.s), mov_dpp<kDppMirror>(v.c)});
  return v;
}

template <int W>
__device__ __forceinline__ double row_sum(double v) {
  if constexpr (W >= 2) v += mov_dpp<kDppXor1>(v);
  if constexpr (W >= 4) v += mov_dpp<kDppXor2>(v);
  if constexpr (W >= 8) v += mov_dpp<kDppHalfMirror>(v);
  if constexpr (W >= 16) v += mov_dpp<kDppMirror>(v);
  return v;
}

__device__ __forceinline__ double shfl_xor_d(double v, int mask) { return __shfl_xor(v, mask, kWave); }

struct Kahan1 {
  double sum, corr;
  __device__ __forceinline__ void init(double v) { sum = v; corr = 0; }
  __device__ __forceinline__ void add(double v) {
    const double y = v - corr;
    const double t = sum + y;
    corr = (t - sum) - y;
    sum = t;
  }
  __device__ __forceinline__ double get() const { return sum - corr; }
};

__device__ __forceinline__ double precise_sum4(const double *sum, const double *corr) {
  Kahan1 a;
  a.init(corr[3]);
  for (int i = 2; i >= 0; i--) a.add(corr[i]);
  a.sum = -a.sum;
  a.corr = -a.corr;
  for (int i = 3; i >= 0; i--) a.add(sum[i]);
  return a.get();
}

__device__ __forceinline__ int64_t upper_bound_d(const double *a, int64_t n, double v) {
  int64_t lo = 0, hi = n;
  while (lo < hi) {
    const int64_t mid = lo + ((hi - lo) >> 1);
    if (!(v < a[mid])) lo = mid + 1; else hi = mid;
  }
  return lo;
}
__device__ __forceinline__ int64_t upper_bound_strided(const double *a, int64_t n, int64_t stride, double v) {
  int64_t lo = 0, hi = n;
  while (lo < hi) {
    const int64_t mid = lo + ((hi - lo) >> 1);
    if (!(v < a[mid * stride])) lo = mid + 1; else hi = mid;
// ... 309 lines not shown
```

probqa_amd/csrc/pqa_kernels.h:

```cpp
#pragma once

#include <hip/hip_runtime.h>
#include <stdint.h>

#include <atomic>

namespace pqa {

constexpr size_t kLdsPerCU = 160 * 1024;
constexpr size_t kLdsNoOptIn = 64 * 1024;
constexpr double kLnSqrt2 = 0.34657359027997265470861606072909;

constexpr int kMaxDevices = 64;
inline int DeviceSlot() { int d = 0; return hipGetDevice(&d) == hipSuccess ? (d & (kMaxDevices - 1)) : 0; }
inline int DeviceCUs(int dev) {
  static std::atomic<int> numCUs[kMaxDevices];
  int n = numCUs[dev].load(std::memory_order_relaxed);
  if (n == 0) {
    int d = 0;
    n = (hipGetDevice(&d) == hipSuccess && hipDeviceGetAttribute(&n, hipDeviceAttributeMultiprocessorCount, d) == hipSuccess && n > 0) ? n : 256;
    numCUs[dev].store(n, std::memory_order_relaxed);
  }
  return n;
}
inline int DeviceCUs() { return DeviceCUs(DeviceSlot()); }

struct LaunchCache {
  std::atomic<uint64_t> slot[kMaxDevices];
  bool Get(int dev, size_t key, int *perCU) const {
    const uint64_t v = slot[dev].load(std::memory_order_acquire);
    if (v == 0 || (v >> 16) != (uint64_t)key) return false;
    *perCU = (int)(v & 0xFFFF) - 1;
    return true;
  }
  void Put(int dev, size_t key, int perCU) { slot[dev].store(((uint64_t)key << 16) | (uint64_t)(perCU + 1), std::memory_order_release); }
  static hipError_t Ask(const void *kern, int threads, size_t shmem, int *perCU) {
    *perCU = 0;
    if (shmem > kLdsNoOptIn) {
      const hipError_t e = hipFuncSetAttribute(kern, hipFuncAttributeMaxDynamicSharedMemorySize, (int)shmem);
      if (e != hipSuccess) return e;
    }
    if (hipOccupancyMaxActiveBlocksPerMultiprocessor(perCU, kern, threads, shmem) != hipSuccess) *perCU = 0;
    return hipSuccess;
  }
  template <typename Kern>
  hipError_t Residency(int dev, Kern *kern, int threads, size_t shmem, size_t key, int *perCU) {
    if (Get(dev, key, perCU)) return hipSuccess;
    const hipError_t e = Ask(reinterpret_cast<const void *>(kern), threads, shmem, perCU);
    if (e != hipSuccess) return e;
    if (*perCU < 1) *perCU = 1;
    Put(dev, key, *perCU);
    return hipSuccess;
  }
  template <typename Kern>
  hipError_t Residency(int dev, Kern *kern, int threads, size_t shmem, int *perCU) { return Residency(dev, kern, threads, shmem, shmem, perCU); }
  template <typename Kern>
  hipError_t OptIn(int dev, Kern *kern, size_t maxShmem, size_t key = 1) {
    int done = 0;
    if (Get(dev, key, &done)) return hipSuccess;
    const hipError_t e = hipFuncSetAttribute(reinterpret_cast<const void *>(kern), hipFuncAttributeMaxDynamicSharedMemorySize, (int)maxShmem);
    if (e == hipSuccess) Put(dev, key, 1);
    return e;
  }
};

struct KbView {
  const void *cube;
  int elem;
  const double *vB;
  const uint32_t *tgap;
  const uint32_t *qgap;
  int64_t K, Q, T, ldT;
  int64_t nValidTargets;
  int smallLaunches;
  double *priorScratch;
  int maxGrid;
  int clusterForm;
  int clusterShape;
  int64_t clusterFrom;
  double *poleScratch;
  struct PoleHeader *poleList;
  int poleNoFollow;
  int poleGate;
};

inline double VCompTail(const KbView &kb) {
  const double nT = (double)(kb.nValidTargets + 1);
  return kLnSqrt2 / (nT * nT);
}

struct PoleHeader { uint32_t count, arrived; unsigned long long floorBits; };
struct PoleEntry {
  uint32_t q;
  uint32_t rowMask;
  uint32_t b;
  uint32_t gap;
};
static_assert(sizeof(PoleHeader) == 16, "header and entries are 16 bytes each");
size_t PoleListBytes(int64_t capacity);
hipError_t UploadLog2TablePole(const double *hostTable);

struct SelectResult {
  double priority;
  int64_t index;
};

hipError_t UploadLog2Table(const double *hostTable);
hipError_t LaunchLog2HotArray(const double *x, double *out, int64_t n, hipStream_t stream);

constexpr int kFusedMaxGrid = 4096;
struct alignas(16) TaggedPriority { double priority; uint64_t tag; };

struct FusedSelect {
  SelectResult *scratch;
  SelectResult *out;
  uint64_t *seq;
  uint64_t seqValue;
  int64_t outBase;
  int64_t scratchStride;
  uint64_t flagValue;
  uint64_t *tagCell;
  int64_t sampleSubtasks;
  uint64_t sampleRnd;
  double *runLength;
  TaggedPriority *hostPriority;
  int64_t lazyFix;
};
struct QuizSlot {
  const double *prior;
  const uint32_t *asked;
  double *priority;
  SelectResult *out;
  uint64_t *seq;
  TaggedPriority *hostPriority;
};
hipError_t LaunchEvalQuestions(const KbView &kb, const double *prior, const uint32_t *asked, int64_t qFirst,
                               int64_t qLimit, double *priority, int variant, const FusedSelect *fused,
                               hipStream_t stream);
hipError_t LaunchEvalPoleFixup(const KbView &kb, const double *prior, const uint32_t *asked, double *priority, const FusedSelect &fused,
                               hipStream_t stream);
struct PoleFix {
  const double *cube;
  const uint32_t *tgap, *qgap, *asked;
  const double *prior;
  const QuizSlot *slots;
  int nSlots;
  PoleHeader *list;
  uint32_t *maskDense;
  uint32_t *dirty;
  double *sums;
  int64_t sumsStride;
  int bySlot, wOff, vOff, hOff, lOff, secondIsWV;
  double *priority, *priorityT;
  int Bp;
  TaggedPriority *hostPriority;
  uint64_t hostTag;
  int64_t K, T, ldT, qFirst, nQ, capacity;
  double vCompTail;
  FusedSelect fs;
  int rows, waveLds;
  int gate;
};
hipError_t LaunchPoleFixup(const PoleFix &fix, hipStream_t stream);
inline PoleFix PoleFixWV(const double *cube, const uint32_t *tgap, const uint32_t *qgap, int64_t K, int64_t T, int64_t ldT) {
  PoleFix f{};
  f.cube = cube; f.tgap = tgap; f.qgap = qgap;
  f.K = K; f.T = T; f.ldT = ldT;
  f.sumsStride = 2 * K + 2;
  f.wOff = 0; f.vOff = (int)K; f.hOff = (int)(2 * K); f.lOff = (int)(2 * K + 1); f.secondIsWV = 1;
  return f;
}
size_t EvalBatchPoleBytes(const KbView &kb, int nSlots);
hipError_t LaunchEvalQuestionsBatch(const KbView &kb, const QuizSlot *slots, int nSlots, int64_t qFirst, int64_t qLimit,
                                    int variant, const FusedSelect &fused, hipStream_t stream, void *pole = nullptr);
constexpr int kBatchMaxGrid = 2048;
struct BatchRecord { double priority; int64_t index; };
struct BatchPlan {
  int tileTargets;
  int questionsPerBlock;
  int splitTail;
  int questionGroups;
  int grid, Bp;
  size_t ptBytes, accBytes, recBytes;
  size_t poleBytes;
  void *pole;
};
constexpr size_t kBatchPoleClear = 1024 + 16;
static_assert(kBatchPoleClear == 256 * sizeof(uint32_t) + sizeof(PoleHeader), "marks and list header");
inline size_t batch_pole_bytes(const KbView &kb, int quizzes) {
  const size_t cap = (size_t)kb.Q * (size_t)quizzes;
  return kBatchPoleClear + cap * sizeof(PoleEntry) + cap * (size_t)(2 * kb.K + 2) * sizeof(double);
}
struct BatchPole { PoleHeader *list; uint32_t *dirty; double *sums; };
inline BatchPole batch_pole(const KbView &kb, int quizzes, void *pole) {
  char *p = static_cast<char *>(pole);
  const size_t cap = (size_t)kb.Q * (size_t)quizzes;
  return BatchPole{reinterpret_cast<PoleHeader *>(p + 256 * sizeof(uint32_t)), reinterpret_cast<uint32_t *>(p),
                   reinterpret_cast<double *>(p + kBatchPoleClear + cap * sizeof(PoleEntry))};
}
hipError_t LaunchEvalBatch(const KbView &kb, const QuizSlot *slots, int nSlots, BatchPlan *plan, void *PT, double *acc,
                           BatchRecord *recs, double *priorityT, int64_t outBase, uint64_t flagValue, bool queryOnly, hipStream_t stream,
                           bool skipPick = false);
bool EvalMidBatchSupported(const KbView &kb);
hipError_t LaunchEvalMidBatch(const KbView &kb, const QuizSlot *slots, int nSlots, BatchPlan *plan, void *PT, BatchRecord *recs,
                              double *priorityT, int64_t outBase, uint64_t flagValue, bool queryOnly, hipStream_t stream);
size_t BatchRerankScratchBytes();
hipError_t LaunchBatchRerank(const KbView &kb, const QuizSlot *slots, int nSlots, int Bp, const double *priorityT, void *scratch,
                             int64_t outBase, uint64_t flagValue, hipStream_t stream);
hipError_t LaunchEvalQuestionsF32(const KbView &kb, const double *prior, const uint32_t *asked, double *priority, hipStream_t stream);
bool EvalF32RegisterShape(const KbView &kb, int variant);
const char *EvalF32KernelName(const KbView &kb, int variant);
hipError_t LaunchEvalQuestionsF32Reg(const KbView &kb, const double *prior, const uint32_t *asked, double *priority, int variant,
                                     hipStream_t stream);
hipError_t UploadLog2TableBatch(const double *hostTable);
hipError_t UploadLog2TableCluster(const double *hostTable);
bool EvalClusterSupported(const KbView &kb);
const char *EvalClusterKernelName(const KbView &kb);
size_t EvalClusterScratchBytes(const KbView &kb);
hipError_t LaunchEvalCluster(const KbView &kb, const double *prior, const uint32_t *asked, double *priority, void *scratch, hipStream_t stream);
const char *EvalVariantName(const KbView &kb, int variant);
bool EvalVariantFusesSampled(const KbView &kb, int variant, int64_t nSubtasks);
bool EvalVariantHasFinisherWorkgroup(const KbView &kb, int variant);

struct ServerMailbox {
  uint64_t req;
  const double *prior;
  const uint32_t *asked;
  SelectResult *out;
  uint64_t *flag;
  uint64_t flagValue;
  int64_t outBase;
  uint64_t stop;
  uint64_t state;
  uint64_t taken;
  uint64_t done;
  uint64_t pad[5];
};
constexpr uint64_t kServerRunning = 1, kServerExiting = 2, kServerExited = 3;
struct ServerCtl {
  uint64_t go;
  const double *prior;
  const uint32_t *asked;
  SelectResult *out;
  uint64_t *flag;
  uint64_t flagValue;
  int64_t outBase;
  uint64_t pad;
};
constexpr uint64_t kServerHandOver = 1ull << 62;
constexpr uint64_t kServerNoWatch = 1ull << 61;
hipError_t LaunchEvalServer(const KbView &kb, int64_t qFirst, int64_t qLimit, double *priority, int variant,
                            SelectResult *scratch, ServerMailbox *mailbox, void *requestLine, bool everyonePolls,
                            ServerCtl *ctl, uint64_t lastSeq, uint64_t idleTicks, TaggedPriority *hostPriority, hipStream_t stream,
                            bool watch = false);
bool EvalServerSupported(const KbView &kb, int variant);


struct RatedTargetDev { int64_t iTarget; double prob; };
bool EvalFusesUpdate(const KbView &kb, int variant, int64_t nWorkers);
hipError_t LaunchEvalQuestionsWithUpdate(const KbView &kb, double *prior, uint32_t *asked, double *priority, int variant, const FusedSelect &fused,
                                         int64_t iQuestion, int64_t iAnswer, int64_t nWorkers, RatedTargetDev *topOut, int64_t *topN,
                                         uint64_t *topFlag, uint64_t topFlagValue, int64_t topCount, hipStream_t stream);

hipError_t LaunchSelectArgmax(const double *priority, const uint32_t *qgap, const uint32_t *asked, int64_t qFirst,
                              int64_t n, int64_t outBase, SelectResult *out, uint64_t *flag, uint64_t flagValue,
                              hipStream_t stream);
hipError_t LaunchSelectSampled(const double *priority, const uint32_t *qgap, const uint32_t *asked, int64_t qFirst,
                               int64_t n, int64_t nSubtasks, uint64_t rnd, double *runLength, SelectResult *out,
                               uint64_t *flag, uint64_t flagValue, hipStream_t stream);
constexpr size_t kSampledBatchLdsBytes = kLdsPerCU;
struct SampledBatch {
  const QuizSlot *slots;
  int nSlots, Bp;
  const double *priorityT;
  const uint32_t *qgap;
  int64_t n, nWorkers;
  const uint64_t *rnd;
  double *grand, *run;
  SelectResult *out;
  uint64_t *seq;
  uint64_t flagValue;
  int64_t outBase;
};
void SelectSampledBatchScratch(int64_t n, int64_t nSubtasks, int nSlots, int Bp, size_t *grandDoubles, size_t *runDoubles);
hipError_t LaunchSelectSampledBatch(const SampledBatch &a, hipStream_t stream);
struct SampledPartsPack {
  const QuizSlot *slots;
  int nSlots, Bq;
  const double *priorityT;
  const uint32_t *qgap;
  int64_t qFirst, nLocal, qTotal, nWorkers;
  char *dst;
  int64_t partBytes;
  double *run;
  uint64_t *stamp;
  uint64_t seq;
  unsigned *counter;
  uint64_t *flag;
  uint64_t flagValue;
};
hipError_t LaunchSampledPackParts(const SampledPartsPack &a, hipStream_t stream);
constexpr int kSampledMaxWorld = 64;
struct SampledPartsPick {
  int nSlots, world, rank;
  const char *parts;
  int64_t partBytes, qTotal, nWorkers;
  const uint64_t *rnd;
  const double *packRun;
  int64_t packRunQuiz, packRunStride;
  const uint64_t *stamp;
  uint64_t seq;
  double *grand, *run;
  SelectResult *out;
  uint64_t *flags;
  uint64_t flagValue;
};
hipError_t LaunchSampledPickParts(const SampledPartsPick &a, hipStream_t stream);

constexpr int64_t kMaxWorkers = 1000;
hipError_t LaunchStartQuiz(const KbView &kb, double *prior, uint32_t *asked, int64_t askedWords, int64_t nWorkers, hipStream_t stream);
hipError_t LaunchRecordAnswer(const KbView &kb, double *prior, uint32_t *asked, int64_t iQuestion, int64_t iAnswer,
                              int64_t nWorkers, RatedTargetDev *topOut, int64_t *topN, uint64_t *topFlag,
                              uint64_t topFlagValue, int64_t topCount, hipStream_t stream, const void *rowA = nullptr,
                              const void *rowD = nullptr);
constexpr int kRecordInline = 256;
struct RecordSlot {
  double *prior;
  uint32_t *asked;
  void *pin;
  int32_t iQuestion, iAnswer;
  uint64_t topFlagValue;
  const void *rowA, *rowD;
};
constexpr int kQuizTopDev = 32;
struct RecordBatchInline {
  int32_t n, topCount;
  RecordSlot s[kRecordInline];
};
hipError_t LaunchRecordAnswerBatch(const KbView &kb, const RecordBatchInline &batch, int64_t nWorkers, hipStream_t stream);
constexpr int kStartInline = 256;
struct StartBatchInline {
  int32_t n;
  int64_t askedWords;
  double *prior[kStartInline];
  uint32_t *asked[kStartInline];
};
hipError_t LaunchStartQuizBatch(const KbView &kb, const StartBatchInline &batch, int64_t nWorkers, hipStream_t stream);
hipError_t LaunchResumeQuiz(const KbView &kb, double *prior, int64_t *exps, const void *const *rows, int64_t nAnswered,
                            int64_t nWorkers, int bugCompat, int64_t *status, hipStream_t stream);
// ... 99 lines not shown
```

probqa_amd/csrc/select_kernels.hip:

```cpp
#include "pqa_device.h"
#include "pqa_kernels.h"
#include "sampled_part.h"

namespace pqa {

namespace {

struct Best {
  double p;
  int64_t i;
};

__device__ __forceinline__ bool better(const Best &a, const Best &b) {
  if (b.i < 0) return a.i >= 0;
  if (a.i < 0) return false;
  return (a.p > b.p) || (a.p == b.p && a.i < b.i);
}

__global__ __launch_bounds__(1024) void select_argmax_kernel(const double *__restrict__ priority,
                                                             const uint32_t *__restrict__ qgap,
                                                             const uint32_t *__restrict__ asked, int64_t qFirst,
                                                             int64_t n, int64_t outBase, SelectResult *out, uint64_t *flag,
                                                             uint64_t flagValue) {
  __shared__ double sp[16];
  __shared__ int64_t si[16];
  Best b = {0.0, -1};
  for (int64_t j = threadIdx.x; j < n; j += blockDim.x) {
    const int64_t q = qFirst + j;
    if (bit_test(qgap, q) || bit_test(asked, q)) continue;
    double p = priority[j];
    if (p != p) p = -__builtin_huge_val();
    const Best c = {p, q};
    if (better(c, b)) b = c;
  }
#pragma unroll
  for (int m = kWave / 2; m >= 1; m >>= 1) {
    Best o;
    o.p = __shfl_xor(b.p, m, kWave);
    o.i = __shfl_xor(b.i, m, kWave);
    if (better(o, b)) b = o;
  }
  const int wave = threadIdx.x / kWave, lane = threadIdx.x % kWave;
  if (lane == 0) {
    sp[wave] = b.p;
    si[wave] = b.i;
  }
  __syncthreads();
  if (threadIdx.x == 0) {
    Best r = {sp[0], si[0]};
    const int nw = (blockDim.x + kWave - 1) / kWave;
    for (int w = 1; w < nw; w++) {
      const Best c = {sp[w], si[w]};
      if (better(c, r)) r = c;
    }
    out->priority = r.p;
    out->index = r.i < 0 ? -1 : r.i - qFirst + outBase;
    if (flag != nullptr) {
      __builtin_amdgcn_fence(__ATOMIC_RELEASE, "");
      __hip_atomic_store(flag, flagValue, __ATOMIC_RELAXED, __HIP_MEMORY_SCOPE_SYSTEM);
    }
  }
}

__global__ __launch_bounds__(1024) void select_sampled_kernel(const double *__restrict__ priority,
                                                              const uint32_t *__restrict__ qgap,
                                                              const uint32_t *__restrict__ asked, int64_t qFirst,
                                                              int64_t n, int64_t nWorkers, uint64_t rnd,
                                                              double *__restrict__ runLength, SelectResult *out, uint64_t *flag, uint64_t flagValue) {
  extern __shared__ double grand[];
  const SampledPick r = select_sampled_wg_impl<false>(priority, qgap, asked, qFirst, n, nWorkers, rnd, runLength, grand);
  if (threadIdx.x == 0) {
    out->priority = r.priority;
    out->index = r.index;
    if (flag != nullptr) {
      __builtin_amdgcn_fence(__ATOMIC_RELEASE, "");
      __hip_atomic_store(flag, flagValue, __ATOMIC_RELAXED, __HIP_MEMORY_SCOPE_SYSTEM);
    }
  }
}

__global__ __launch_bounds__(256) void select_sampled_lds_kernel(const double *__restrict__ priority,
                                                                 const uint32_t *__restrict__ qgap,
                                                                 const uint32_t *__restrict__ asked, int64_t qFirst, int64_t n,
                                                                 int64_t nWorkers, uint64_t rnd, SelectResult *out, uint64_t *flag,
                                                                 uint64_t flagValue) {
  extern __shared__ double lds[];
  const SampledPick r = select_sampled_wg_lds<false>(priority, qgap, asked, qFirst, n, nWorkers, rnd, lds);
  if (threadIdx.x == 0) {
    out->priority = r.priority;
    out->index = r.index;
    if (flag != nullptr) {
      __builtin_amdgcn_fence(__ATOMIC_RELEASE, "");
      __hip_atomic_store(flag, flagValue, __ATOMIC_RELAXED, __HIP_MEMORY_SCOPE_SYSTEM);
    }
  }
}

template <bool LDS>
__global__ __launch_bounds__(256) void select_sampled_batch_vec_kernel(SampledBatch a) {
  extern __shared__ double lds[];
  const int b = blockIdx.x;
  const QuizSlot s = a.slots[b];
  const uint64_t rnd = a.rnd[b];
  SampledPick r;
  if constexpr (LDS) r = select_sampled_wg_lds<false>(s.priority, a.qgap, s.asked, 0, a.n, a.nWorkers, rnd, lds);
  else r = select_sampled_wg_impl<false>(s.priority, a.qgap, s.asked, 0, a.n, a.nWorkers, rnd, a.run + (size_t)b * (size_t)a.n, lds);
  if (threadIdx.x == 0) {
    a.out[b].priority = r.priority;
    a.out[b].index = r.index + a.outBase;
    __builtin_amdgcn_fence(__ATOMIC_RELEASE, "");
    __hip_atomic_store(a.seq + b, a.flagValue, __ATOMIC_RELAXED, __HIP_MEMORY_SCOPE_SYSTEM);
  }
}

template <bool STORE>
__device__ __forceinline__ double sampled_lane_chain(const double *__restrict__ col, int64_t stride, const uint32_t *__restrict__ qgap,
                                                     const uint32_t *__restrict__ asked, int64_t first, int64_t limit, double *run) {
  Kahan1 acc;
  acc.init(0.0);
  int64_t word = -1;
  uint32_t bits = 0;
  for (int64_t i0 = first; i0 < limit; i0 += 8) {
    double v[8];
#pragma unroll
    for (int u = 0; u < 8; u++) v[u] = i0 + u < limit ? col[(i0 + u) * stride] : 0.0;
#pragma unroll
    for (int u = 0; u < 8; u++) {
      const int64_t i = i0 + u;
      if (i < limit) {
        if ((i >> 5) != word) { word = i >> 5; bits = qgap[word] | asked[word]; }
        if (!((bits >> (i & 31)) & 1u)) acc.add(v[u]);
        if constexpr (STORE) run[(i - first) * stride] = acc.get();
      }
    }
  }
  return acc.get();
}

__global__ __launch_bounds__(256) void select_sampled_lanes_kernel(SampledBatch a) {
  const int64_t g = (int64_t)blockIdx.x * blockDim.x + threadIdx.x;
  const int b = (int)(g % a.Bp);
  const int64_t s = g / a.Bp;
  const int64_t quot = a.n / a.nWorkers, rem = a.n % a.nWorkers;
  const int64_t nSubtasks = (quot == 0) ? rem : a.nWorkers;
  if (s >= nSubtasks || b >= a.nSlots) return;
  const int64_t first = (s == 0) ? 0 : calc_split_bound(s - 1, quot, rem), limit = calc_split_bound(s, quot, rem);
  a.grand[s * a.Bp + b] = sampled_lane_chain<false>(a.priorityT + b, a.Bp, a.qgap, a.slots[b].asked, first, limit, nullptr);
}

__global__ __launch_bounds__(64) void select_sampled_lanes_finish_kernel(SampledBatch a) {
  const int b = (int)(blockIdx.x * blockDim.x + threadIdx.x);
  if (b >= a.nSlots) return;
  const int64_t Bp = a.Bp, n = a.n;
  const int64_t quot = n / a.nWorkers, rem = n % a.nWorkers;
  const int64_t nSubtasks = (quot == 0) ? rem : a.nWorkers;
  double *grand = a.grand + b;
  Kahan1 accTotG;
  accTotG.init(0.0);
  for (int64_t s0 = 0; s0 < nSubtasks; s0 += 16) {
    double g[16];
#pragma unroll
    for (int u = 0; u < 16; u++) g[u] = s0 + u < nSubtasks ? grand[(s0 + u) * Bp] : 0.0;
#pragma unroll
    for (int u = 0; u < 16; u++) {
      if (s0 + u < nSubtasks) {
        accTotG.add(g[u]);
        g[u] = accTotG.get();
      }
    }
#pragma unroll
    for (int u = 0; u < 16; u++)
      if (s0 + u < nSubtasks) grand[(s0 + u) * Bp] = g[u];
  }
  const double totG = grand[(nSubtasks - 1) * Bp];
  const double selRunLen = totG * (double)a.rnd[b] / 18446744073709551615.0;
  int64_t sel;
  const int64_t iWorker = upper_bound_strided(grand, nSubtasks, Bp, selRunLen);
  if (iWorker >= nSubtasks) {
    sel = n - 1;
  } else {
    const double inWorkerRunLen = selRunLen - ((iWorker == 0) ? 0.0 : grand[(iWorker - 1) * Bp]);
    const int64_t first = (iWorker == 0) ? 0 : calc_split_bound(iWorker - 1, quot, rem);
    const int64_t limit = calc_split_bound(iWorker, quot, rem);
    double *run = a.run + b;
    sampled_lane_chain<true>(a.priorityT + b, Bp, a.qgap, a.slots[b].asked, first, limit, run);
    sel = first + upper_bound_strided(run, limit - first, Bp, inWorkerRunLen);
    if (sel >= limit) sel = limit - 1;
  }
  a.out[b].priority = totG;
  a.out[b].index = sel + a.outBase;
  __builtin_amdgcn_fence(__ATOMIC_RELEASE, "");
  __hip_atomic_store(a.seq + b, a.flagValue, __ATOMIC_RELAXED, __HIP_MEMORY_SCOPE_SYSTEM);
}

__global__ __launch_bounds__(256) void sampled_pack_parts_kernel(SampledPartsPack a) {
  const SampledSplit sp = sampled_split(a.qTotal, a.nWorkers);
  const int64_t g = (int64_t)blockIdx.x * blockDim.x + threadIdx.x;
  const int b = (int)(g % a.Bq);
  const int64_t s = g / a.Bq;
  if (s < sp.nS && b < a.nSlots) {
    char *part = a.dst + (int64_t)b * a.partBytes;
    const SampledPartShape sh = sampled_part_shape(sp, a.qFirst, a.nLocal);
    if (s == 0) {
      SampledPartHeader *h = reinterpret_cast<SampledPartHeader *>(part);
      h->qFirst = a.qFirst;
      h->nLocal = a.nLocal;
      h->nS = sp.nS;
      h->seq = a.seq;
      a.stamp[b] = a.seq;
    }
    const bool matrix = a.priorityT != nullptr;
    const double *col = matrix ? a.priorityT + b : a.slots[b].priority;
    const int64_t stride = matrix ? a.Bq : 1;
    const uint32_t *asked = a.slots[b].asked;
    double total = 0.0;
    if (s >= sh.firstWhole && s < sh.firstWhole + sh.nWhole) {
      const int64_t first = sampled_first(sp, s) - a.qFirst, limit = sampled_limit(sp, s) - a.qFirst;
      double *run = matrix ? a.run + first * a.Bq + b : a.run + (int64_t)b * a.nLocal + first;
      total = sampled_lane_chain<true>(col, stride, a.qgap, asked, first, limit, run);
    } else if (s == sh.p0Sub || s == sh.p1Sub) {
      const int piece = s == sh.p0Sub ? 0 : 1;
      const int64_t first = (piece == 0 ? sh.p0First : sh.p1First) - a.qFirst, len = piece == 0 ? sh.p0Len : sh.p1Len;
      double *pri = reinterpret_cast<double *>(part + sampled_piece_offset(sp, piece));
      uint64_t *skip = reinterpret_cast<uint64_t *>(pri + sp.L);
      uint64_t word = 0;
#pragma unroll 4
      for (int64_t j = 0; j < len; j++) {
        const int64_t i = first + j;
        pri[j] = col[i * stride];
        word |= (uint64_t)(((a.qgap[i >> 5] | asked[i >> 5]) >> (i & 31)) & 1u) << (j & 63);
        if ((j & 63) == 63 || j == len - 1) { skip[j >> 6] = word; word = 0; }
      }
    }
    reinterpret_cast<double *>(part + sampled_totals_offset())[s] = total;
  }
  if (a.flag == nullptr) return;
  __builtin_amdgcn_fence(__ATOMIC_RELEASE, "");
  __syncthreads();
  if (threadIdx.x != 0) return;
  if (__hip_atomic_fetch_add(a.counter, 1u, __ATOMIC_ACQ_REL, __HIP_MEMORY_SCOPE_AGENT) != gridDim.x - 1) return;
  __builtin_amdgcn_fence(__ATOMIC_RELEASE, "");
  __hip_atomic_store(a.flag, a.flagValue, __ATOMIC_RELAXED, __HIP_MEMORY_SCOPE_SYSTEM);
}

template <bool STORE>
__device__ __forceinline__ void sampled_piece_chain(Kahan1 &acc, const double *__restrict__ pri, const uint64_t *__restrict__ skip, int64_t n,
                                                    double *run) {
  for (int64_t i0 = 0; i0 < n; i0 += 8) {
    double v[8];
#pragma unroll
    for (int u = 0; u < 8; u++) v[u] = i0 + u < n ? pri[i0 + u] : 0.0;
    const uint64_t bits = skip[i0 >> 6];
#pragma unroll
    for (int u = 0; u < 8; u++) {
      const int64_t i = i0 + u;
      if (i < n) {
        if (!((bits >> (i & 63)) & 1u)) acc.add(v[u]);
        if constexpr (STORE) run[i] = acc.get();
      }
    }
  }
}

__device__ __forceinline__ int sampled_rank_of(const int64_t *firsts, int world, int64_t q) {
  int r = 0;
  while (r + 1 < world && firsts[r + 1] <= q) r++;
  return r;
}

template <bool STORE>
__device__ __forceinline__ double sampled_cut_chain(const SampledPartsPick &a, const SampledSplit &sp, const int64_t *firsts, int b, int64_t s,
                                                    double *run) {
  Kahan1 acc;
  acc.init(0.0);
  const int64_t limit = sampled_limit(sp, s);
  int64_t done = 0;
  for (int r = sampled_rank_of(firsts, a.world, sampled_first(sp, s)); r < a.world && firsts[r] < limit; r++) {
    const SampledPartShape sh = sampled_part_shape(sp, firsts[r], firsts[r + 1] - firsts[r]);
    if (sh.p0Sub != s && sh.p1Sub != s) break;
    const int piece = sh.p0Sub == s ? 0 : 1;
    const int64_t len = piece == 0 ? sh.p0Len : sh.p1Len;
    const char *part = a.parts + ((int64_t)r * a.nSlots + b) * a.partBytes;
    const double *pri = reinterpret_cast<const double *>(part + sampled_piece_offset(sp, piece));
    sampled_piece_chain<STORE>(acc, pri, reinterpret_cast<const uint64_t *>(pri + sp.L), len, STORE ? run + done : nullptr);
    done += len;
  }
  return acc.get();
}

__global__ __launch_bounds__(64) void sampled_pick_parts_kernel(SampledPartsPick a) {
  __shared__ int64_t firsts[kSampledMaxWorld + 1];
  __shared__ int64_t counts[kSampledMaxWorld];
  __shared__ int bad;
  const int b = blockIdx.x, t = threadIdx.x;
  const SampledSplit sp = sampled_split(a.qTotal, a.nWorkers);
  if (t == 0) bad = 0;
  __syncthreads();
  for (int r = t; r < a.world; r += blockDim.x) {
    const SampledPartHeader *h = reinterpret_cast<const SampledPartHeader *>(a.parts + ((int64_t)r * a.nSlots + b) * a.partBytes);
    firsts[r] = h->qFirst;
    counts[r] = h->nLocal;
    if (h->nS != sp.nS) atomicOr(&bad, 2);
    if (r == a.rank && (h->seq != a.seq || a.stamp[b] != a.seq)) atomicOr(&bad, 1);
  }
  __syncthreads();
  if (t == 0) {
    int64_t at = 0;
    bool tiles = true;
    for (int r = 0; r < a.world; r++) {
      tiles = tiles && firsts[r] == at && counts[r] >= 1 && counts[r] <= a.qTotal - at;
      if (!tiles) break;
      at += counts[r];
    }
    firsts[a.world] = at;
    if (!tiles || at != a.qTotal) bad |= 2;
  }
  __syncthreads();
  if (bad != 0) {
    if (t == 0) {
      a.out[b].priority = 0.0;
      a.out[b].index = (bad & 1) ? -2 : -3;
      __builtin_amdgcn_fence(__ATOMIC_RELEASE, "");
      __hip_atomic_store(a.flags + b, a.flagValue, __ATOMIC_RELAXED, __HIP_MEMORY_SCOPE_SYSTEM);
    }
    return;
  }
  double *grand = a.grand + (int64_t)b * sp.nS;
  for (int64_t s = t; s < sp.nS; s += blockDim.x) {
    const int r = sampled_rank_of(firsts, a.world, sampled_first(sp, s));
    if (sampled_limit(sp, s) <= firsts[r + 1])
      grand[s] = reinterpret_cast<const double *>(a.parts + ((int64_t)r * a.nSlots + b) * a.partBytes + sampled_totals_offset())[s];
  }
  for (int r = t + 1; r < a.world; r += blockDim.x) {
    const int64_t s = sampled_subtask_of(sp, firsts[r]), first = sampled_first(sp, s);
    if (first == firsts[r] || (r > 1 && first < firsts[r - 1])) continue;
    grand[s] = sampled_cut_chain<false>(a, sp, firsts, b, s, nullptr);
  }
  __syncthreads();
  if (t != 0) return;
  const int64_t nSubtasks = sp.nS;
  Kahan1 accTotG;
  accTotG.init(0.0);
  for (int64_t s0 = 0; s0 < nSubtasks; s0 += 16) {
    double g[16];
#pragma unroll
    for (int u = 0; u < 16; u++) g[u] = s0 + u < nSubtasks ? grand[s0 + u] : 0.0;
#pragma unroll
    for (int u = 0; u < 16; u++) {
      if (s0 + u < nSubtasks) {
        accTotG.add(g[u]);
        g[u] = accTotG.get();
      }
    }
#pragma unroll
    for (int u = 0; u < 16; u++)
      if (s0 + u < nSubtasks) grand[s0 + u] = g[u];
  }
  const double totG = grand[nSubtasks - 1];
  const double selRunLen = totG * (double)a.rnd[b] / 18446744073709551615.0;
  int64_t sel;
  const int64_t iWorker = upper_bound_strided(grand, nSubtasks, 1, selRunLen);
  if (iWorker >= nSubtasks) {
    sel = a.qTotal - 1;
  } else {
    const double inWorkerRunLen = selRunLen - ((iWorker == 0) ? 0.0 : grand[iWorker - 1]);
    const int64_t first = sampled_first(sp, iWorker), limit = sampled_limit(sp, iWorker);
    const int r = sampled_rank_of(firsts, a.world, first);
    if (limit > firsts[r + 1]) {
      double *run = a.run + (int64_t)b * sp.L;
      sampled_cut_chain<true>(a, sp, firsts, b, iWorker, run);
      sel = first + upper_bound_strided(run, limit - first, 1, inWorkerRunLen);
      if (sel >= limit) sel = limit - 1;
    } else if (r == a.rank) {
      const double *run = a.packRun + (int64_t)b * a.packRunQuiz + (first - firsts[r]) * a.packRunStride;
      sel = first + upper_bound_strided(run, limit - first, a.packRunStride, inWorkerRunLen);
      if (sel >= limit) sel = limit - 1;
    } else {
      sel = -1;
    }
  }
  a.out[b].priority = totG;
  a.out[b].index = sel;
  __builtin_amdgcn_fence(__ATOMIC_RELEASE, "");
  __hip_atomic_store(a.flags + b, a.flagValue, __ATOMIC_RELAXED, __HIP_MEMORY_SCOPE_SYSTEM);
}

}

hipError_t LaunchSelectArgmax(const double *priority, const uint32_t *qgap, const uint32_t *asked, int64_t qFirst,
                              int64_t n, int64_t outBase, SelectResult *out, uint64_t *flag, uint64_t flagValue,
                              hipStream_t stream) {
  const unsigned threads = n >= 1024 ? 1024 : (unsigned)(((n + 63) / 64) * 64 ? ((n + 63) / 64) * 64 : 64);
  hipLaunchKernelGGL(select_argmax_kernel, dim3(1), dim3(threads), 0, stream, priority, qgap, asked, qFirst, n,
                     outBase, out, flag, flagValue);
  return hipGetLastError();
}

hipError_t LaunchSelectSampled(const double *priority, const uint32_t *qgap, const uint32_t *asked, int64_t qFirst,
                               int64_t n, int64_t nSubtasks, uint64_t rnd, double *runLength, SelectResult *out,
                               uint64_t *flag, uint64_t flagValue, hipStream_t stream) {
  if (n <= 0 || nSubtasks <= 0) return hipErrorInvalidValue;
  const size_t staged = (size_t)select_sampled_lds_doubles(n, nSubtasks) * sizeof(double);
  if (staged <= kLdsNoOptIn) {
    hipLaunchKernelGGL(select_sampled_lds_kernel, dim3(1), dim3(256), staged, stream, priority, qgap, asked, qFirst, n, nSubtasks,
                       rnd, out, flag, flagValue);
    return hipGetLastError();
  }
  const size_t shmem = (size_t)nSubtasks * sizeof(double);
  if (shmem > kLdsNoOptIn) return hipErrorInvalidValue;
  hipLaunchKernelGGL(select_sampled_kernel, dim3(1), dim3(1024), shmem, stream, priority, qgap, asked, qFirst, n, nSubtasks,
                     rnd, runLength, out, flag, flagValue);
  return hipGetLastError();
}

void SelectSampledBatchScratch(int64_t n, int64_t nSubtasks, int nSlots, int Bp, size_t *grandDoubles, size_t *runDoubles) {
  const int64_t quot = n / nSubtasks, rem = n % nSubtasks, subtasks = quot == 0 ? rem : nSubtasks;
  if (Bp > 0) {
    *grandDoubles = (size_t)subtasks * (size_t)Bp;
    *runDoubles = (size_t)(quot + 1) * (size_t)Bp;
    return;
  }
  *grandDoubles = 0;
  *runDoubles = (size_t)select_sampled_lds_doubles(n, nSubtasks) * sizeof(double) <= kSampledBatchLdsBytes ? 0 : (size_t)nSlots * (size_t)n;
}

hipError_t LaunchSelectSampledBatch(const SampledBatch &a, hipStream_t stream) {
  if (a.n <= 0 || a.nWorkers <= 0 || a.nSlots <= 0 || a.nSlots > 256 || !a.slots || !a.rnd || !a.out || !a.seq) return hipErrorInvalidValue;
  if (a.priorityT != nullptr) {
    if (a.Bp < a.nSlots || a.Bp % kWave != 0 || !a.grand || !a.run) return hipErrorInvalidValue;
    const int64_t quot = a.n / a.nWorkers, rem = a.n % a.nWorkers, nSubtasks = quot == 0 ? rem : a.nWorkers;
    const int64_t threads = nSubtasks * a.Bp;
    hipLaunchKernelGGL(select_sampled_lanes_kernel, dim3((unsigned)((threads + 255) / 256)), dim3(256), 0, stream, a);
    hipError_t e = hipGetLastError();
    if (e != hipSuccess) return e;
    hipLaunchKernelGGL(select_sampled_lanes_finish_kernel, dim3((unsigned)((a.nSlots + kWave - 1) / kWave)), dim3(kWave), 0, stream, a);
    return hipGetLastError();
  }
  const size_t staged = (size_t)select_sampled_lds_doubles(a.n, a.nWorkers) * sizeof(double);
  if (staged <= kSampledBatchLdsBytes) {
    if (staged > kLdsNoOptIn) {
      static LaunchCache cache;
      const hipError_t e = cache.OptIn(DeviceSlot(), select_sampled_batch_vec_kernel<true>, kSampledBatchLdsBytes);
      if (e != hipSuccess) return e;
    }
    hipLaunchKernelGGL(select_sampled_batch_vec_kernel<true>, dim3((unsigned)a.nSlots), dim3(256), staged, stream, a);
    return hipGetLastError();
  }
  const size_t shmem = (size_t)a.nWorkers * sizeof(double);
  if (shmem > kLdsNoOptIn || !a.run) return hipErrorInvalidValue;
  hipLaunchKernelGGL(select_sampled_batch_vec_kernel<false>, dim3((unsigned)a.nSlots), dim3(256), shmem, stream, a);
  return hipGetLastError();
}

hipError_t LaunchSampledPackParts(const SampledPartsPack &a, hipStream_t stream) {
  if (a.nSlots < 0 || a.nSlots > 256 || a.qTotal <= 0 || a.nWorkers <= 0 || a.nLocal <= 0 || a.qFirst < 0 || a.qFirst + a.nLocal > a.qTotal)
    return hipErrorInvalidValue;
  if (a.nSlots > 0 && (!a.slots || !a.qgap || !a.dst || !a.run || !a.stamp || a.Bq < a.nSlots || a.Bq % kWave != 0)) return hipErrorInvalidValue;
  if (a.flag != nullptr && a.counter == nullptr) return hipErrorInvalidValue;
  const SampledSplit sp = sampled_split(a.qTotal, a.nWorkers);
  if (a.nSlots > 0 && a.partBytes != sampled_part_bytes(sp)) return hipErrorInvalidValue;
  const int64_t threads = a.nSlots > 0 ? sp.nS * a.Bq : 1;
  hipLaunchKernelGGL(sampled_pack_parts_kernel, dim3((unsigned)((threads + 255) / 256)), dim3(256), 0, stream, a);
  return hipGetLastError();
}

hipError_t LaunchSampledPickParts(const SampledPartsPick &a, hipStream_t stream) {
  if (a.nSlots <= 0 || a.nSlots > 256 || a.world <= 0 || a.world > kSampledMaxWorld || a.rank < 0 || a.rank >= a.world || a.qTotal <= 0 ||
      a.nWorkers <= 0 || !a.parts || !a.rnd || !a.packRun || !a.stamp || !a.grand || !a.run || !a.out || !a.flags)
    return hipErrorInvalidValue;
  if (a.partBytes != sampled_part_bytes(sampled_split(a.qTotal, a.nWorkers))) return hipErrorInvalidValue;
  hipLaunchKernelGGL(sampled_pick_parts_kernel, dim3((unsigned)a.nSlots), dim3(kWave), 0, stream, a);
  return hipGetLastError();
}

}
```

Measured before the change: 42080 selections/s.

## Publish selection as one packed 16-byte tagged store and use DPP wave reduction

Replaces the device-to-host result handoff, which wrote priority and index, fenced, then stored a separate flag, with a single 16-byte system-coherent store that carries the priority bits plus a tag and answer word. The host spins on that record directly. This removes a fence and a second PCIe write from the critical path of each synchronous selection. The wave-level argmax also switches from xor shuffles to DPP moves and swap helpers. The cost is a 31-bit index limit, reserved answer codes, and more complex tag handling across the launched, graph and resident paths.

```diff
diff --git a/probqa_amd/csrc/batch_kernels.hip b/probqa_amd/csrc/batch_kernels.hip
--- a/probqa_amd/csrc/batch_kernels.hip
+++ b/probqa_amd/csrc/batch_kernels.hip
@@ -564,12 +564,7 @@
   }
   if (lane != 0) return;
   const QuizSlot s = slots[b];
-  s.out->priority = bq < 0 ? 0.0 : bp;
-  s.out->index = bq < 0 ? -1 : bq + outBase;
-  if (s.seq != nullptr) {
-    __builtin_amdgcn_fence(__ATOMIC_RELEASE, "");
-    __hip_atomic_store(s.seq, flagValue, __ATOMIC_RELAXED, __HIP_MEMORY_SCOPE_SYSTEM);
-  }
+  host_publish(s.out, bq < 0 ? 0.0 : bp, bq < 0 ? -1 : bq + outBase, s.seq, flagValue);
 }
 
 constexpr int kF32LdsTargets = 16384;
diff --git a/probqa_amd/csrc/eval_kernels.hip b/probqa_amd/csrc/eval_kernels.hip
--- a/probqa_amd/csrc/eval_kernels.hip
+++ b/probqa_amd/csrc/eval_kernels.hip
@@ -63,13 +63,25 @@
 __device__ __forceinline__ void best_offer(Best &b, double p, int64_t i) {
   best_merge(b, p != p ? -__builtin_huge_val() : p, i);
 }
+template <int CTRL>
+__device__ __forceinline__ void best_step(Best &b) {
+  const double op = mov_dpp<CTRL>(b.p);
+  const int64_t oi = mov_dpp_i64<CTRL>(b.i);
+  best_merge(b, op, oi);
+}
 __device__ __forceinline__ Best wave_best(Best b) {
-#pragma unroll
-  for (int m = kWave / 2; m >= 1; m >>= 1) {
-    const double op = __shfl_xor(b.p, m, kWave);
-    const int64_t oi = __shfl_xor(b.i, m, kWave);
-    best_merge(b, op, oi);
-  }
+  best_step<kDppXor1>(b);
+  best_step<kDppXor2>(b);
+  best_step<kDppHalfMirror>(b);
+  best_step<kDppMirror>(b);
+  Pair p = swap16(b.p);
+  PairI64 i = swap16_i64(b.i);
+  b = Best{p.a, i.a};
+  best_merge(b, p.b, i.b);
+  p = swap32(b.p);
+  i = swap32_i64(b.i);
+  b = Best{p.a, i.a};
+  best_merge(b, p.b, i.b);
   return b;
 }
 
@@ -141,12 +153,8 @@
   }
   if (deferred) return;
   if (UNI || lane == 0) {
-    a.fs.out->priority = b.i < 0 ? 0.0 : b.p;
-    a.fs.out->index = !complete ? -3 : redo ? -4 : b.i < 0 ? -1 : b.i + a.fs.outBase;
-    if (a.fs.seq != nullptr) {
-      __builtin_amdgcn_fence(__ATOMIC_RELEASE, "");
-      __hip_atomic_store(a.fs.seq, flagValue, __ATOMIC_RELAXED, __HIP_MEMORY_SCOPE_SYSTEM);
-    }
+    if (a.fs.packed) host_publish_packed(a.fs.out, b.i < 0 ? 0.0 : b.p, flagValue, !complete ? -3 : redo ? -4 : b.i < 0 ? -1 : b.i);
+    else host_publish(a.fs.out, b.i < 0 ? 0.0 : b.p, !complete ? -3 : redo ? -4 : b.i < 0 ? -1 : b.i + a.fs.outBase, a.fs.seq, flagValue);
     if (a.fs.tagCell != nullptr) {
       uint64_t next = seqValue + 1;
       if ((uint32_t)next == 0) next++;
@@ -630,12 +638,8 @@
       __syncthreads();
       const bool complete = allReported[0], deferred = allReported[1], redo = allReported[2];
       if (!deferred && (SERVER ? wave == 0 : tid == 0)) {
-        a.fs.out->priority = 0.0;
-        a.fs.out->index = !complete ? -3 : redo ? -4 : 0;
-        if (a.fs.seq != nullptr) {
-          __builtin_amdgcn_fence(__ATOMIC_RELEASE, "");
-          __hip_atomic_store(a.fs.seq, a.fs.flagValue, __ATOMIC_RELAXED, __HIP_MEMORY_SCOPE_SYSTEM);
-        }
+        if (a.fs.packed) host_publish_packed(a.fs.out, 0.0, a.fs.flagValue, !complete ? -3 : redo ? -4 : 0);
+        else host_publish(a.fs.out, 0.0, !complete ? -3 : redo ? -4 : 0, a.fs.seq, a.fs.flagValue);
       }
     }
     return;
@@ -648,12 +652,8 @@
       const SampledPick r = select_sampled_wg_lds<true>(a.priority, a.qgap, a.asked, a.qFirst, a.qLimit - a.qFirst,
                                                         a.fs.sampleSubtasks, a.fs.sampleRnd, tbl);
       if (tid == 0) {
-        a.fs.out->priority = r.priority;
-        a.fs.out->index = complete ? r.index + a.fs.outBase : -3;
-        if (a.fs.seq != nullptr) {
-          __builtin_amdgcn_fence(__ATOMIC_RELEASE, "");
-          __hip_atomic_store(a.fs.seq, a.fs.flagValue, __ATOMIC_RELAXED, __HIP_MEMORY_SCOPE_SYSTEM);
-        }
+        if (a.fs.packed) host_publish_packed(a.fs.out, r.priority, a.fs.flagValue, complete ? r.index : -3);
+        else host_publish(a.fs.out, r.priority, complete ? r.index + a.fs.outBase : -3, a.fs.seq, a.fs.flagValue);
       }
     }
   }
@@ -758,7 +758,8 @@
     b.fs.seq = reinterpret_cast<uint64_t *>(uniform64(reinterpret_cast<const uint64_t *>(step)[4]));
     b.fs.flagValue = uniform64(reinterpret_cast<const uint64_t *>(step)[5]);
     const uint64_t ob = uniform64(reinterpret_cast<const uint64_t *>(step)[6]);
-    b.fs.outBase = (int64_t)(ob & ~(kServerHandOver | kServerNoWatch));
+    b.fs.outBase = (int64_t)(ob & ~(kServerHandOver | kServerNoWatch | kServerPacked));
+    b.fs.packed = (ob & kServerPacked) ? 1 : 0;
     b.serverNoWatch = (ob & kServerNoWatch) != 0;
     b.fs.sampleSubtasks = (ob & kServerHandOver) ? 1 : 0;
     b.fs.seqValue = go;
@@ -1033,12 +1034,7 @@
     if (bq < 0 || p > bp || (p == bp && q < bq)) { bp = p; bq = q; }
   }
   const QuizSlot s = slots[b];
-  s.out->priority = bq < 0 ? 0.0 : bp;
-  s.out->index = bq < 0 ? -1 : bq + outBase;
-  if (s.seq != nullptr) {
-    __builtin_amdgcn_fence(__ATOMIC_RELEASE, "");
-    __hip_atomic_store(s.seq, flagValue, __ATOMIC_RELAXED, __HIP_MEMORY_SCOPE_SYSTEM);
-  }
+  host_publish(s.out, bq < 0 ? 0.0 : bp, bq < 0 ? -1 : bq + outBase, s.seq, flagValue);
 }
 
 size_t BatchRerankScratchBytes() { return (size_t)256 * kRerank * (sizeof(int64_t) + sizeof(double)); }
diff --git a/probqa_amd/csrc/hip_engine.h b/probqa_amd/csrc/hip_engine.h
--- a/probqa_amd/csrc/hip_engine.h
+++ b/probqa_amd/csrc/hip_engine.h
@@ -375,8 +375,10 @@
   std::unordered_map<Quiz *, GraphEntry> _graphs;
   SelectResult *_dGraphScratch = nullptr;
   uint64_t *_dTagCell = nullptr;
-  static constexpr uint64_t kGraphFlagBase = 1ull << 40, kServerFlagBase = 2ull << 40;
+  static constexpr uint64_t kGraphFlagBase = 1ull << 40;
   uint64_t _graphTag = kGraphFlagBase + 1;
+  uint64_t _serverTag = 0;
+  enum OwnCell { kOwnLaunched = 0, kOwnGraph = 1, kOwnResident = 2 };
   void DropQuizBufferPool();
   SelectResult *_dSel = nullptr;
   struct Pinned {
@@ -387,7 +389,9 @@
     int64_t nOutQ;
     uint64_t topQFlag;
     RatedTargetDev topQ[256];
-  };
+    PackedSelection own[3];
+  };
+  SelectResult *OwnRecord(OwnCell c) { return reinterpret_cast<SelectResult *>(&_hPinned->own[c]); }
   uint64_t _opSeq = 0;
   std::vector<QuizPinned *> _pinSlabs, _pinFree;
   static constexpr int kPinSlab = 256;
@@ -474,6 +478,7 @@
   std::atomic<uint64_t> _combNs[7] = {{0}, {0}, {0}, {0}, {0}, {0}, {0}};
   volatile uint64_t *_pendingRecordFlag = nullptr;
   Error WaitFlag(volatile uint64_t *flag, uint64_t value, const char *what);
+  Error WaitPacked(SelectResult *record, uint64_t tag, int64_t outBase, const char *what, bool resident = false);
   Error WaitFlagNapping(volatile uint64_t *flag, uint64_t value, const char *what);
   SelectResult *_dSelScratch = nullptr;
   double *_dPriorScratch = nullptr;
@@ -623,7 +628,6 @@
   uint64_t _pendingRecordOp = 0;
   bool ServerUsable() const;
   Error ServerPost(Quiz *q, SelectResult *out, uint64_t *flag, uint64_t flagValue, int64_t outBase);
-  Error ServerWait(volatile uint64_t *flag, uint64_t value, const char *what);
   void StopServer();
   void ServerQuiesce();
   SelectorRng _rng;
diff --git a/probqa_amd/csrc/hip_engine_select.cpp b/probqa_amd/csrc/hip_engine_select.cpp
--- a/probqa_amd/csrc/hip_engine_select.cpp
+++ b/probqa_amd/csrc/hip_engine_select.cpp
@@ -143,7 +143,7 @@
     }
     HIP_TRY(LaunchEvalCluster(View(), q->dPrior, q->dAsked, _dPriority, _dClusterScratch, _stream));
     if (fused != nullptr)
-      HIP_TRY(LaunchSelectArgmax(_dPriority, _dQGap, q->dAsked, 0, _Q, fused->outBase, fused->out, fused->seq, fused->flagValue, _stream));
+      HIP_TRY(LaunchSelectArgmax(_dPriority, _dQGap, q->dAsked, 0, _Q, fused->outBase, fused->out, fused->seq, fused->flagValue, _stream, fused->packed != 0));
     return Error();
   }
   if (_elem == 8) {
@@ -160,7 +160,7 @@
   else
     HIP_TRY(LaunchEvalQuestionsF32(View(), q->dPrior, q->dAsked, _dPriority, _stream));
   if (fused != nullptr)
-    HIP_TRY(LaunchSelectArgmax(_dPriority, _dQGap, q->dAsked, 0, _Q, fused->outBase, fused->out, fused->seq, fused->flagValue, _stream));
+    HIP_TRY(LaunchSelectArgmax(_dPriority, _dQGap, q->dAsked, 0, _Q, fused->outBase, fused->out, fused->seq, fused->flagValue, _stream, fused->packed != 0));
   return Error();
 }
 
@@ -255,6 +255,28 @@
   return Error();
 }
 
+Error HipEngine::WaitPacked(SelectResult *record, uint64_t tag, int64_t outBase, const char *what, bool resident) {
+  volatile PackedSelection *cell = reinterpret_cast<volatile PackedSelection *>(record);
+  volatile ServerMailbox *mb = _hMailbox;
+  SpinWait w;
+  while (!PackedCarries(cell->tagAnswer, tag)) {
+    if (!w.Tick(std::chrono::seconds(30))) return HipErr(hipErrorNotReady, what);
+    if (!w.Due()) continue;
+    if (resident) {
+      if (mb->state == kServerExited && mb->taken != _serverPosted && !PackedCarries(cell->tagAnswer, tag)) return HipErr(hipErrorUnknown, what);
+    } else if (hipStreamQuery(_stream) == hipSuccess && !PackedCarries(cell->tagAnswer, tag)) {
+      const hipError_t he = hipStreamSynchronize(_stream);
+      if (he != hipSuccess || !PackedCarries(cell->tagAnswer, tag)) return HipErr(he == hipSuccess ? hipErrorUnknown : he, what);
+    }
+  }
+  std::atomic_thread_fence(std::memory_order_acquire);
+  const uint64_t tagAnswer = cell->tagAnswer, bits = cell->priorityBits;
+  cell->tagAnswer = 0;
+  std::memcpy(&_hPinned->sel.priority, &bits, sizeof(bits));
+  _hPinned->sel.index = UnpackSelection(tagAnswer, outBase);
+  return Error();
+}
+
 int64_t HipEngine::NextQuestionArgmax(Error &err, int64_t iQuiz) { return Combine(err, iQuiz, 0, 0); }
 
 bool HipEngine::LazyFix() const {
@@ -273,7 +295,7 @@
   fs.lazyFix = 0;
   fs.flagValue = NextLaunchTag();
   HIP_TRY(LaunchEvalPoleFixup(View(), q->dPrior, q->dAsked, _dPriority, fs, _stream));
-  Error err = WaitFlag(fs.seq, fs.flagValue, what);
+  Error err = fs.packed ? WaitPacked(fs.out, fs.flagValue, fs.outBase, what) : WaitFlag(fs.seq, fs.flagValue, what);
   std::atomic_thread_fence(std::memory_order_acquire);
   if (err.ok()) _poleListPending = false;
   return err;
@@ -289,9 +311,9 @@
   if (!err.ok()) return -1;
   if (_opt.useGraph && _elem == 8) return NextQuestionArgmaxGraph(err, q);
   if (_opt.server && !q->noServer && ServerUsable()) {
-    const uint64_t value = kServerFlagBase | ++_opSeq;
-    err = ServerPost(q, &_hPinned->sel, &_hPinned->seq, value, 0);
-    if (err.ok()) err = ServerWait(&_hPinned->seq, value, "NextQuestionArgmax");
+    const uint64_t value = _serverTag = NextSelectionTag(_serverTag);
+    err = ServerPost(q, OwnRecord(kOwnResident), &_hPinned->seq, value, (int64_t)kServerPacked);
+    if (err.ok()) err = WaitPacked(OwnRecord(kOwnResident), value, 0, "NextQuestionArgmax", true);
     if (!err.ok()) return -1;
     if (_hPinned->sel.index == -3) {
       err = HipErr(hipErrorLaunchFailure, "NextQuestionArgmax (incomplete sweep)");
@@ -308,15 +330,14 @@
   if (TakeSpeculation(q, 1 << 1, &seq) != 0) fs = _spec.fs;
   else {
     seq = NextLaunchTag();
-    fs = FusedSelect{_dSelScratch, &_hPinned->sel, &_hPinned->seq, seq, 0, 0, seq, nullptr, 0, 0, nullptr, nullptr, LazyFix() && q->lateStreak < _opt.lateEager ? 1 : 0};
+    fs = FusedSelect{_dSelScratch, OwnRecord(kOwnLaunched), &_hPinned->seq, seq, 0, 0, seq, nullptr, 0, 0, nullptr, nullptr, LazyFix() && q->lateStreak < _opt.lateEager ? 1 : 0, 1};
     StopServer();
     err = LaunchSingleSweep(q, &fs);
     if (!err.ok()) return -1;
     if (fs.lazyFix) _poleListPending = true;
   }
-  err = WaitFlag(&_hPinned->seq, seq, "NextQuestionArgmax");
+  err = WaitPacked(fs.out, seq, 0, "NextQuestionArgmax");
   if (!err.ok()) return -1;
-  std::atomic_thread_fence(std::memory_order_acquire);
   if (fs.lazyFix) {
     if (_hPinned->sel.index == -4) {
       err = RunLazyFix(q, fs, "NextQuestionArgmax");
@@ -754,7 +775,7 @@
   if (it == _graphs.end() || it->second.variant != _opt.evalVariant || it->second.stream != _stream ||
       it->second.kbVersion != _kbVersion) {
     if (it != _graphs.end()) { hipGraphExecDestroy(it->second.exec); _graphs.erase(it); }
-    const FusedSelect fs{_dGraphScratch, &_hPinned->sel, &_hPinned->seq, 0, 0, 0, 0, _dTagCell, 0, 0, nullptr, nullptr};
+    const FusedSelect fs{_dGraphScratch, OwnRecord(kOwnGraph), &_hPinned->seq, 0, 0, 0, 0, _dTagCell, 0, 0, nullptr, nullptr, 0, 1};
     hipGraph_t graph = nullptr;
     hipGraphExec_t exec = nullptr;
     hipError_t he = hipStreamBeginCapture(_stream, hipStreamCaptureModeThreadLocal);
@@ -774,10 +795,8 @@
   if (!err.ok()) return -1;
   const hipError_t he = hipGraphLaunch(it->second.exec, _stream);
   if (he != hipSuccess) { err = HipErr(he, "hipGraphLaunch"); return -1; }
-  uint64_t next = _graphTag + 1;
-  if ((uint32_t)next == 0) next++;
-  _graphTag = next;
-  err = WaitFlag(&_hPinned->seq, expect, "NextQuestionArgmax (graph)");
+  _graphTag = NextSelectionTag(_graphTag);
+  err = WaitPacked(OwnRecord(kOwnGraph), expect, 0, "NextQuestionArgmax (graph)");
   if (!err.ok()) return -1;
   if (_hPinned->sel.index == -3) { err = HipErr(hipErrorLaunchFailure, "NextQuestionArgmax (incomplete sweep)"); return -1; }
   CheckPriority(_hPinned->sel.priority, _hPinned->sel.index);
@@ -797,9 +816,9 @@
   const KbView kb = View();
   const int64_t nSub = _opt.evalSubtasks ? _opt.evalSubtasks : 8 * _opt.workers;
   if (_opt.server && !q->noServer && _opt.hostSampled && !_opt.fusedSampled && ServerUsable()) {
-    const uint64_t value = kServerFlagBase | ++_opSeq;
-    err = ServerPost(q, &_hPinned->sel, &_hPinned->seq, value, (int64_t)kServerHandOver);
-    if (err.ok()) err = ServerWait(&_hPinned->seq, value, "NextQuestionSampled");
+    const uint64_t value = _serverTag = NextSelectionTag(_serverTag);
+    err = ServerPost(q, OwnRecord(kOwnResident), &_hPinned->seq, value, (int64_t)(kServerHandOver | kServerPacked));
+    if (err.ok()) err = WaitPacked(OwnRecord(kOwnResident), value, 0, "NextQuestionSampled", true);
     if (!err.ok()) return -1;
     if (_hPinned->sel.index == -3) { err = HipErr(hipErrorLaunchFailure, "NextQuestionSampled (incomplete sweep)"); return -1; }
     if (_hPinned->sel.index != -4) {
@@ -823,12 +842,12 @@
     else {
       { Error se = SettlePoleList(); if (!se.ok()) { err = se; return -1; } }
       seq = NextLaunchTag();
-      fs = FusedSelect{_dSelScratch, &_hPinned->sel, &_hPinned->seq, seq, 0, 0, seq, nullptr, 1, 0, nullptr, _hHostPriority, LazyFix() && q->lateStreak < _opt.lateEager ? 1 : 0};
+      fs = FusedSelect{_dSelScratch, OwnRecord(kOwnLaunched), &_hPinned->seq, seq, 0, 0, seq, nullptr, 1, 0, nullptr, _hHostPriority, LazyFix() && q->lateStreak < _opt.lateEager ? 1 : 0, 1};
       const hipError_t he = LaunchEvalQuestions(kb, q->dPrior, q->dAsked, 0, _Q, _dPriority, (int)_opt.evalVariant, &fs, _stream);
       if (he != hipSuccess) { err = HipErr(he, "NextQuestionSampled"); return -1; }
       if (fs.lazyFix) _poleListPending = true;
     }
-    err = WaitFlag(&_hPinned->seq, seq, "NextQuestionSampled");
+    err = WaitPacked(fs.out, seq, 0, "NextQuestionSampled");
     if (!err.ok()) return -1;
     if (fs.lazyFix) {
       if (_hPinned->sel.index == -4) {
@@ -849,10 +868,10 @@
   if (took != 3 && _opt.fusedSampled && _elem == 8 && EvalVariantFusesSampled(kb, (int)_opt.evalVariant, nSub)) {
     { Error se = SettlePoleList(); if (!se.ok()) { err = se; return -1; } }
     const uint64_t seq = NextLaunchTag();
-    const FusedSelect fs{_dSelScratch, &_hPinned->sel, &_hPinned->seq, seq, 0, 0, seq, nullptr, nSub, rnd, _dRunLength, nullptr};
+    const FusedSelect fs{_dSelScratch, OwnRecord(kOwnLaunched), &_hPinned->seq, seq, 0, 0, seq, nullptr, nSub, rnd, _dRunLength, nullptr, 0, 1};
     const hipError_t he = LaunchEvalQuestions(kb, q->dPrior, q->dAsked, 0, _Q, _dPriority, (int)_opt.evalVariant, &fs, _stream);
     if (he != hipSuccess) { err = HipErr(he, "NextQuestionSampled"); return -1; }
-    err = WaitFlag(&_hPinned->seq, seq, "NextQuestionSampled");
+    err = WaitPacked(fs.out, seq, 0, "NextQuestionSampled");
     if (!err.ok()) return -1;
     if (_hPinned->sel.index == -3) { err = HipErr(hipErrorLaunchFailure, "NextQuestionSampled (incomplete sweep)"); return -1; }
     CheckPriority(_hPinned->sel.priority, _hPinned->sel.index);
diff --git a/probqa_amd/csrc/hip_engine_server.cpp b/probqa_amd/csrc/hip_engine_server.cpp
--- a/probqa_amd/csrc/hip_engine_server.cpp
+++ b/probqa_amd/csrc/hip_engine_server.cpp
@@ -22,17 +22,6 @@
   SpinWait w;
   while (mb->done != _serverPosted && mb->state != kServerExited)
     if (!w.Tick(std::chrono::seconds(30))) return;
-}
-
-Error HipEngine::ServerWait(volatile uint64_t *flag, uint64_t value, const char *what) {
-  SpinWait w;
-  volatile ServerMailbox *mb = _hMailbox;
-  while (*flag != value) {
-    if (!w.Tick(std::chrono::seconds(30))) return HipErr(hipErrorNotReady, what);
-    if (w.Due() && mb->state == kServerExited && mb->taken != _serverPosted && *flag != value) return HipErr(hipErrorUnknown, what);
-  }
-  std::atomic_thread_fence(std::memory_order_acquire);
-  return Error();
 }
 
 Error HipEngine::ServerPost(Quiz *q, SelectResult *out, uint64_t *flag, uint64_t flagValue, int64_t outBase) {
diff --git a/probqa_amd/csrc/hip_engine_update.cpp b/probqa_amd/csrc/hip_engine_update.cpp
--- a/probqa_amd/csrc/hip_engine_update.cpp
+++ b/probqa_amd/csrc/hip_engine_update.cpp
@@ -195,8 +195,8 @@
   if (withUpdate) DropSpeculation();
   const uint64_t seq = NextLaunchTag();
   if (!SettlePoleList().ok()) return false;
-  const FusedSelect fs{_dSelScratch, &_hPinned->sel, &_hPinned->seq, seq, 0, 0, seq, nullptr, kind == 2 ? 1 : 0, 0, nullptr,
-                       kind == 2 ? _hHostPriority : nullptr, (kind == 1 || kind == 2) && LazyFix() && q->lateStreak < _opt.lateEager ? 1 : 0};
+  const FusedSelect fs{_dSelScratch, OwnRecord(kOwnLaunched), &_hPinned->seq, seq, 0, 0, seq, nullptr, kind == 2 ? 1 : 0, 0, nullptr,
+                       kind == 2 ? _hHostPriority : nullptr, (kind == 1 || kind == 2) && LazyFix() && q->lateStreak < _opt.lateEager ? 1 : 0, 1};
   if (withUpdate) {
     const int64_t topCount = std::min<int64_t>(std::min<int64_t>(std::min<int64_t>(_opt.topCache, _topWantRecent), kQuizTop), _T);
     const uint64_t op = _opSeq + 1;
diff --git a/probqa_amd/csrc/pole_kernels.hip b/probqa_amd/csrc/pole_kernels.hip
--- a/probqa_amd/csrc/pole_kernels.hip
+++ b/probqa_amd/csrc/pole_kernels.hip
@@ -345,11 +345,15 @@
       outI = r.index + a.fs.outBase;
     }
     if (tid == 0) {
-      a.fs.out->priority = outP;
-      a.fs.out->index = outI;
-      if (a.fs.seq != nullptr) {
-        __builtin_amdgcn_fence(__ATOMIC_RELEASE, "");
-        __hip_atomic_store(a.fs.seq, flagValue, __ATOMIC_RELAXED, __HIP_MEMORY_SCOPE_SYSTEM);
+      if (a.fs.packed) {
+        host_publish_packed(a.fs.out, outP, flagValue, outI);
+      } else {
+        a.fs.out->priority = outP;
+        a.fs.out->index = outI;
+        if (a.fs.seq != nullptr) {
+          __builtin_amdgcn_fence(__ATOMIC_RELEASE, "");
+          __hip_atomic_store(a.fs.seq, flagValue, __ATOMIC_RELAXED, __HIP_MEMORY_SCOPE_SYSTEM);
+        }
       }
       if (a.fs.tagCell != nullptr) {
         uint64_t next = seqValue + 1;
@@ -378,12 +382,7 @@
         }
       }
       if (lane == 0) {
-        qs.out->priority = handOver || best.i < 0 ? 0.0 : best.p;
-        qs.out->index = handOver ? 0 : best.i < 0 ? -1 : best.i + a.fs.outBase;
-        if (qs.seq != nullptr) {
-          __builtin_amdgcn_fence(__ATOMIC_RELEASE, "");
-          __hip_atomic_store(qs.seq, a.fs.flagValue, __ATOMIC_RELAXED, __HIP_MEMORY_SCOPE_SYSTEM);
-        }
+        host_publish(qs.out, handOver || best.i < 0 ? 0.0 : best.p, handOver ? 0 : best.i < 0 ? -1 : best.i + a.fs.outBase, qs.seq, a.fs.flagValue);
       }
     }
   }
diff --git a/probqa_amd/csrc/pqa_device.h b/probqa_amd/csrc/pqa_device.h
--- a/probqa_amd/csrc/pqa_device.h
+++ b/probqa_amd/csrc/pqa_device.h
@@ -5,6 +5,8 @@
 
 #include <type_traits>
 #include <utility>
+
+#include "select_record.h"
 
 namespace pqa {
 
@@ -192,6 +194,48 @@
 }
 
 template <int CTRL>
+__device__ __forceinline__ int64_t mov_dpp_i64(int64_t v) {
+  int lo = (int)(uint32_t)(uint64_t)v, hi = (int)(uint32_t)((uint64_t)v >> 32);
+  lo = __builtin_amdgcn_update_dpp(0, lo, CTRL, 0xF, 0xF, true);
+  hi = __builtin_amdgcn_update_dpp(0, hi, CTRL, 0xF, 0xF, true);
+  return (int64_t)(((uint64_t)(uint32_t)hi << 32) | (uint32_t)lo);
+}
+struct PairI64 { int64_t a, b; };
+__device__ __forceinline__ PairI64 swap16_i64(int64_t v) {
+  const uint64_t b = (uint64_t)v;
+  const auto r0 = __builtin_amdgcn_permlane16_swap((uint32_t)b, (uint32_t)b, false, false);
+  const auto r1 = __builtin_amdgcn_permlane16_swap((uint32_t)(b >> 32), (uint32_t)(b >> 32), false, false);
+  return PairI64{(int64_t)(((uint64_t)r1[0] << 32) | r0[0]), (int64_t)(((uint64_t)r1[1] << 32) | r0[1])};
+}
+__device__ __forceinline__ PairI64 swap32_i64(int64_t v) {
+  const uint64_t b = (uint64_t)v;
+  const auto r0 = __builtin_amdgcn_permlane32_swap((uint32_t)b, (uint32_t)b, false, false);
+  const auto r1 = __builtin_amdgcn_permlane32_swap((uint32_t)(b >> 32), (uint32_t)(b >> 32), false, false);
+  return PairI64{(int64_t)(((uint64_t)r1[0] << 32) | r0[0]), (int64_t)(((uint64_t)r1[1] << 32) | r0[1])};
+}
+
+__device__ __forceinline__ void host_store(double *p, double v) { __hip_atomic_store(p, v, __ATOMIC_RELAXED, __HIP_MEMORY_SCOPE_SYSTEM); }
+__device__ __forceinline__ void host_store(int64_t *p, int64_t v) { __hip_atomic_store(p, v, __ATOMIC_RELAXED, __HIP_MEMORY_SCOPE_SYSTEM); }
+__device__ __forceinline__ void host_stores_done() { asm volatile("s_waitcnt vmcnt(0)" ::: "memory"); }
+__device__ __forceinline__ void host_flag(uint64_t *flag, uint64_t value) {
+  host_stores_done();
+  __hip_atomic_store(flag, value, __ATOMIC_RELAXED, __HIP_MEMORY_SCOPE_SYSTEM);
+}
+template <class Rec>
+__device__ __forceinline__ void host_publish(Rec *out, double priority, int64_t index, uint64_t *flag, uint64_t flagValue) {
+  host_store(&out->priority, priority);
+  host_store(&out->index, index);
+  if (flag != nullptr) host_flag(flag, flagValue);
+}
+
+__device__ __forceinline__ void host_publish_packed(void *rec, double priority, uint64_t tag, int64_t localIndex) {
+  typedef unsigned int u4 __attribute__((ext_vector_type(4)));
+  const uint64_t w0 = d2u(priority), w1 = PackSelection(tag, localIndex);
+  const u4 v = {(unsigned)w0, (unsigned)(w0 >> 32), (unsigned)w1, (unsigned)(w1 >> 32)};
+  asm volatile("global_store_dwordx4 %0, %1, off sc0 sc1" ::"v"(rec), "v"(v) : "memory");
+}
+
+template <int CTRL>
 __device__ __forceinline__ float mov_dpp_f32(float v) {
   return __builtin_bit_cast(float, __builtin_amdgcn_update_dpp(0, __builtin_bit_cast(int, v), CTRL, 0xF, 0xF, true));
 }
diff --git a/probqa_amd/csrc/pqa_kernels.h b/probqa_amd/csrc/pqa_kernels.h
--- a/probqa_amd/csrc/pqa_kernels.h
+++ b/probqa_amd/csrc/pqa_kernels.h
@@ -4,6 +4,8 @@
 #include <stdint.h>
 
 #include <atomic>
+
+#include "select_record.h"
 
 namespace pqa {
 
@@ -125,6 +127,7 @@
   double *runLength;
   TaggedPriority *hostPriority;
   int64_t lazyFix;
+  int64_t packed;
 };
 struct QuizSlot {
   const double *prior;
@@ -249,6 +252,7 @@
 };
 constexpr uint64_t kServerHandOver = 1ull << 62;
 constexpr uint64_t kServerNoWatch = 1ull << 61;
+constexpr uint64_t kServerPacked = 1ull << 60;
 hipError_t LaunchEvalServer(const KbView &kb, int64_t qFirst, int64_t qLimit, double *priority, int variant,
                             SelectResult *scratch, ServerMailbox *mailbox, void *requestLine, bool everyonePolls,
                             ServerCtl *ctl, uint64_t lastSeq, uint64_t idleTicks, TaggedPriority *hostPriority, hipStream_t stream,
@@ -264,7 +268,7 @@
 
 hipError_t LaunchSelectArgmax(const double *priority, const uint32_t *qgap, const uint32_t *asked, int64_t qFirst,
                               int64_t n, int64_t outBase, SelectResult *out, uint64_t *flag, uint64_t flagValue,
-                              hipStream_t stream);
+                              hipStream_t stream, bool packed = false);
 hipError_t LaunchSelectSampled(const double *priority, const uint32_t *qgap, const uint32_t *asked, int64_t qFirst,
                                int64_t n, int64_t nSubtasks, uint64_t rnd, double *runLength, SelectResult *out,
                                uint64_t *flag, uint64_t flagValue, hipStream_t stream);
diff --git a/probqa_amd/csrc/select_kernels.hip b/probqa_amd/csrc/select_kernels.hip
--- a/probqa_amd/csrc/select_kernels.hip
+++ b/probqa_amd/csrc/select_kernels.hip
@@ -21,7 +21,7 @@
                                                              const uint32_t *__restrict__ qgap,
                                                              const uint32_t *__restrict__ asked, int64_t qFirst,
                                                              int64_t n, int64_t outBase, SelectResult *out, uint64_t *flag,
-                                                             uint64_t flagValue) {
+                                                             uint64_t flagValue, int packed) {
   __shared__ double sp[16];
   __shared__ int64_t si[16];
   Best b = {0.0, -1};
@@ -53,12 +53,8 @@
       const Best c = {sp[w], si[w]};
       if (better(c, r)) r = c;
     }
-    out->priority = r.p;
-    out->index = r.i < 0 ? -1 : r.i - qFirst + outBase;
-    if (flag != nullptr) {
-      __builtin_amdgcn_fence(__ATOMIC_RELEASE, "");
-      __hip_atomic_store(flag, flagValue, __ATOMIC_RELAXED, __HIP_MEMORY_SCOPE_SYSTEM);
-    }
+    if (packed) host_publish_packed(out, r.p, flagValue, r.i < 0 ? -1 : r.i - qFirst);
+    else host_publish(out, r.p, r.i < 0 ? -1 : r.i - qFirst + outBase, flag, flagValue);
   }
 }
 
@@ -70,12 +66,7 @@
   extern __shared__ double grand[];
   const SampledPick r = select_sampled_wg_impl<false>(priority, qgap, asked, qFirst, n, nWorkers, rnd, runLength, grand);
   if (threadIdx.x == 0) {
-    out->priority = r.priority;
-    out->index = r.index;
-    if (flag != nullptr) {
-      __builtin_amdgcn_fence(__ATOMIC_RELEASE, "");
-      __hip_atomic_store(flag, flagValue, __ATOMIC_RELAXED, __HIP_MEMORY_SCOPE_SYSTEM);
-    }
+    host_publish(out, r.priority, r.index, flag, flagValue);
   }
 }
 
@@ -87,12 +78,7 @@
   extern __shared__ double lds[];
   const SampledPick r = select_sampled_wg_lds<false>(priority, qgap, asked, qFirst, n, nWorkers, rnd, lds);
   if (threadIdx.x == 0) {
-    out->priority = r.priority;
-    out->index = r.index;
-    if (flag != nullptr) {
-      __builtin_amdgcn_fence(__ATOMIC_RELEASE, "");
-      __hip_atomic_store(flag, flagValue, __ATOMIC_RELAXED, __HIP_MEMORY_SCOPE_SYSTEM);
-    }
+    host_publish(out, r.priority, r.index, flag, flagValue);
   }
 }
 
@@ -106,10 +92,7 @@
   if constexpr (LDS) r = select_sampled_wg_lds<false>(s.priority, a.qgap, s.asked, 0, a.n, a.nWorkers, rnd, lds);
   else r = select_sampled_wg_impl<false>(s.priority, a.qgap, s.asked, 0, a.n, a.nWorkers, rnd, a.run + (size_t)b * (size_t)a.n, lds);
   if (threadIdx.x == 0) {
-    a.out[b].priority = r.priority;
-    a.out[b].index = r.index + a.outBase;
-    __builtin_amdgcn_fence(__ATOMIC_RELEASE, "");
-    __hip_atomic_store(a.seq + b, a.flagValue, __ATOMIC_RELAXED, __HIP_MEMORY_SCOPE_SYSTEM);
+    host_publish(a.out + b, r.priority, r.index + a.outBase, a.seq + b, a.flagValue);
   }
 }
 
@@ -187,10 +170,7 @@
     sel = first + upper_bound_strided(run, limit - first, Bp, inWorkerRunLen);
     if (sel >= limit) sel = limit - 1;
   }
-  a.out[b].priority = totG;
-  a.out[b].index = sel + a.outBase;
-  __builtin_amdgcn_fence(__ATOMIC_RELEASE, "");
-  __hip_atomic_store(a.seq + b, a.flagValue, __ATOMIC_RELAXED, __HIP_MEMORY_SCOPE_SYSTEM);
+  host_publish(a.out + b, totG, sel + a.outBase, a.seq + b, a.flagValue);
 }
 
 __global__ __launch_bounds__(256) void sampled_pack_parts_kernel(SampledPartsPack a) {
@@ -318,10 +298,7 @@
   __syncthreads();
   if (bad != 0) {
     if (t == 0) {
-      a.out[b].priority = 0.0;
-      a.out[b].index = (bad & 1) ? -2 : -3;
-      __builtin_amdgcn_fence(__ATOMIC_RELEASE, "");
-      __hip_atomic_store(a.flags + b, a.flagValue, __ATOMIC_RELAXED, __HIP_MEMORY_SCOPE_SYSTEM);
+      host_publish(a.out + b, 0.0, (bad & 1) ? -2 : -3, a.flags + b, a.flagValue);
     }
     return;
   }
@@ -379,20 +356,17 @@
       sel = -1;
     }
   }
-  a.out[b].priority = totG;
-  a.out[b].index = sel;
-  __builtin_amdgcn_fence(__ATOMIC_RELEASE, "");
-  __hip_atomic_store(a.flags + b, a.flagValue, __ATOMIC_RELAXED, __HIP_MEMORY_SCOPE_SYSTEM);
+  host_publish(a.out + b, totG, sel, a.flags + b, a.flagValue);
 }
 
 }
 
 hipError_t LaunchSelectArgmax(const double *priority, const uint32_t *qgap, const uint32_t *asked, int64_t qFirst,
                               int64_t n, int64_t outBase, SelectResult *out, uint64_t *flag, uint64_t flagValue,
-                              hipStream_t stream) {
+                              hipStream_t stream, bool packed) {
   const unsigned threads = n >= 1024 ? 1024 : (unsigned)(((n + 63) / 64) * 64 ? ((n + 63) / 64) * 64 : 64);
   hipLaunchKernelGGL(select_argmax_kernel, dim3(1), dim3(threads), 0, stream, priority, qgap, asked, qFirst, n,
-                     outBase, out, flag, flagValue);
+                     outBase, out, flag, flagValue, packed ? 1 : 0);
   return hipGetLastError();
 }
 
diff --git a/probqa_amd/csrc/select_record.h b/probqa_amd/csrc/select_record.h
--- /dev/null
+++ b/probqa_amd/csrc/select_record.h
@@ -0,0 +1,32 @@
+#pragma once
+#include <stdint.h>
+
+#if defined(__HIPCC__) || defined(__CUDACC__)
+#define PQA_HD __host__ __device__
+#else
+#define PQA_HD
+#endif
+
+namespace pqa {
+
+struct alignas(16) PackedSelection { uint64_t priorityBits, tagAnswer; };
+
+constexpr uint32_t kPackedNone = 0x7FFFFFFFu, kPackedIncomplete = 0x7FFFFFFEu, kPackedRedo = 0x7FFFFFFDu;
+constexpr int64_t kPackedMaxIndex = 0x7FFFFFFC;
+
+PQA_HD inline uint64_t PackSelection(uint64_t tag, int64_t index) {
+  const uint32_t answer = index == -1 ? kPackedNone : index == -3 ? kPackedIncomplete : index == -4 ? kPackedRedo : (uint32_t)index;
+  return ((uint64_t)(uint32_t)tag << 32) | answer;
+}
+PQA_HD inline uint32_t PackedTag(uint64_t tagAnswer) { return (uint32_t)(tagAnswer >> 32); }
+PQA_HD inline bool PackedCarries(uint64_t tagAnswer, uint64_t tag) { return PackedTag(tagAnswer) == (uint32_t)tag; }
+PQA_HD inline int64_t UnpackSelection(uint64_t tagAnswer, int64_t outBase) {
+  const uint32_t answer = (uint32_t)tagAnswer;
+  return answer == kPackedNone ? -1 : answer == kPackedIncomplete ? -3 : answer == kPackedRedo ? -4 : (int64_t)answer + outBase;
+}
+PQA_HD inline uint64_t NextSelectionTag(uint64_t tag) {
+  if ((uint32_t)++tag == 0) ++tag;
+  return tag;
+}
+
+}
```

Result: faster. 43830 selections/s (median of 6 runs) (+4.2%).
